# Cranial-XIX/cs231-capsule-yolo-traffic-sign-detection

Measured on AMD Instinct MI355X. Metric: train images/sec darkcapsule GTSDB 416x416 @1/2/4/8 GPU; loss-curve parity, higher is better.
Workload: dtype f32; 1 GPU; experiments/darkcapsule GTSDB-shaped 416x416, n_grid 13, 3 routing iters, batch 32 per GPU, recon off, fp32 (BASELINE configs[2]); global_batch=32, parallelism=dp1

## Files before the change

### cs231-capsule-yolo-traffic-sign-detection_amd/_lib.py

```python
import ctypes as C
import os

_HERE = os.path.dirname(os.path.abspath(__file__))
LIB_PATH = os.environ.get('CAPSYOLO_LIB') or os.path.join(_HERE, 'libcapsyolo_hip.so')

_c_float_p = C.c_void_p
_ll = C.c_longlong


class ConvGemm(C.Structure):
    _fields_ = [('X', C.c_void_p), ('Wp', C.c_void_p), ('Y', C.c_void_p), ('bias', C.c_void_p), ('stats', C.c_void_p),
                ('xs_b', _ll), ('xs_y', _ll), ('xs_x', _ll), ('xs_c', _ll),
                ('B', C.c_int), ('Hi', C.c_int), ('Wi', C.c_int), ('Cin', C.c_int),
                ('Ho', C.c_int), ('Wo', C.c_int), ('N', C.c_int),
                ('TH', C.c_int), ('TW', C.c_int), ('in_stride', C.c_int), ('dy0', C.c_int), ('dx0', C.c_int),
                ('dstep', C.c_int),
                ('Hy', C.c_int), ('Wy', C.c_int), ('out_stride', C.c_int), ('out_oy', C.c_int), ('out_ox', C.c_int),
                ('act', C.c_int),
                ('bn_z', C.c_void_p), ('bn_scale', C.c_void_p), ('bn_shift', C.c_void_p), ('bn_mean', C.c_void_p),
                ('bn_invstd', C.c_void_p), ('bn_red', C.c_void_p), ('bn_slope', C.c_float), ('act_slope', C.c_float),
                ('ws', C.c_void_p), ('ws_floats', _ll)]


class ConvWgrad(C.Structure):
    _fields_ = [('X', C.c_void_p), ('dZ', C.c_void_p), ('dW', C.c_void_p), ('slabs', C.c_void_p),
                ('xs_b', _ll), ('xs_y', _ll), ('xs_x', _ll), ('xs_c', _ll),
                ('B', C.c_int), ('Hi', C.c_int), ('Wi', C.c_int), ('Cin', C.c_int),
                ('Ho', C.c_int), ('Wo', C.c_int), ('N', C.c_int),
                ('KH', C.c_int), ('KW', C.c_int), ('stride', C.c_int), ('pad', C.c_int)]


class RoutingFwd(C.Structure):
    _fields_ = [('u', C.c_void_p), ('W', C.c_void_p), ('v_out', C.c_void_p), ('s_hist', C.c_void_p),
                ('R', C.c_int), ('N', C.c_int), ('C', C.c_int), ('Din', C.c_int), ('Dout', C.c_int),
                ('n_iter', C.c_int), ('gather_g', C.c_int), ('gather_B', C.c_int), ('ws', C.c_void_p)]


class RoutingBwd(C.Structure):
    _fields_ = [('u', C.c_void_p), ('W', C.c_void_p), ('s_hist', C.c_void_p), ('dv', C.c_void_p),
                ('du', C.c_void_p), ('dW', C.c_void_p), ('ws', C.c_void_p),
                ('R', C.c_int), ('N', C.c_int), ('C', C.c_int), ('Din', C.c_int), ('Dout', C.c_int),
                ('n_iter', C.c_int), ('gather_g', C.c_int), ('gather_B', C.c_int)]


class Decoder(C.Structure):
    _fields_ = [(k, C.c_void_p) for k in ('caps', 'labels', 'deltas', 'x', 'lin_w', 'lin_b', 'w4', 'b4', 'w7', 'b7', 'w10', 'b10',
                                          'w12', 'b12', 'out_f32', 'out_u8', 'sqerr', 'err')] + \
               [(k, C.c_int) for k in ('n', 'C', 'D', 'n_delta')]


_P, _I, _F, _L = C.c_void_p, C.c_int, C.c_float, C.c_longlong

_SIGS = {
    'cy_conv_pack_weights': [_P, _P, _I, _I, _I, _I, _I, _I, _I, _I, _I, _I, _P],
    'cy_conv_gemm': [C.POINTER(ConvGemm), _P],
    'cy_conv_wgrad': [C.POINTER(ConvWgrad), _P],
    'cy_channel_sum': [_P, _P, _L, _I, _P],
    'cy_wino_pack_weights': [_P, _P, _I, _I, _I, _P],
    'cy_conv1_3x3_fwd': [_P, _P, _P, _P, _P, _P, _P, _F, _I, _I, _I, _I, _P],
    'cy_conv1_3x3_stats': [_P, _P, _P, _P, _P, _I, _I, _I, _I, _P],
    'cy_conv1_bn_bwd_onepass': [_P, _P, _P, _P, _P, _P, _P, _P, _F, _P, _P, _P, _P, _P, _P, _P, _I, _I, _I, _I, _P],
    'cy_conv1_bn_bwd_onepass_bf16': [_P, _P, _P, _P, _P, _P, _P, _P, _F, _P, _P, _P, _P, _P, _P, _P, _I, _I, _I, _I, _P],
    'cy_conv1_3x3_wgrad': [_P, _P, _P, _P, _I, _I, _I, _I, _P],
    'cy_conv1_bn_bwd_reduce': [_P, _P, _P, _P, _P, _P, _P, _P, _F, _P, _I, _I, _I, _I, _P],
    'cy_conv1_bn_bwd_reduce_bf16': [_P, _P, _P, _P, _P, _P, _P, _P, _F, _P, _I, _I, _I, _I, _P],
    'cy_conv1_bn_bwd_wgrad': [_P, _P, _P, _P, _P, _P, _P, _P, _F, _P, _L, _P, _P, _I, _I, _I, _I, _P],
    'cy_conv1_bn_bwd_wgrad_bf16': [_P, _P, _P, _P, _P, _P, _P, _P, _F, _P, _L, _P, _P, _I, _I, _I, _I, _P],
    'cy_conv1_3x3_fwd_act_bf16': [_P, _P, _P, _P, _P, _P, _F, _I, _I, _I, _I, _P],
    'cy_conv3x3_winograd': [_P, _P, _P, _P, _P, _F, _I, _I, _I, _I, _I, _P],
    'cy_conv3x3_winograd_ws': [_P, _P, _P, _P, _P, _F, _I, _I, _I, _I, _I, _P, _L, _P],
    'cy_wino4_pack_weights': [_P, _P, _I, _I, _I, _P],
    'cy_conv3x3_winograd4': [_P, _P, _P, _P, _P, _F, _I, _I, _I, _I, _I, _P],
    'cy_conv3x3_winograd4_wgrad': [_P, _P, _P, _P, _I, _I, _I, _I, _I, _P],
    'cy_conv3x3_winograd4_wgrad_bn': [_P, _P, _P, _P, _P, _P, _P, _P, _L, _P, _P, _I, _I, _I, _I, _I, _P],
    'cy_conv3x3_winograd_wgrad': [_P, _P, _P, _P, _I, _I, _I, _I, _I, _P],
    'cy_conv3x3_winograd_wgrad_bn': [_P, _P, _P, _P, _P, _P, _P, _P, _F, _I, _P, _L, _P, _P, _I, _I, _I, _I, _I, _P],
    'cy_bn_param_grad': [_P, _P, _P, _I, _P],
    'cy_wino2_pack_weights': [_P, _P, _I, _I, _P],
    'cy_conv4x4s2_winograd': [_P, _P, _P, _P, _P, _P, _P, _F, _F, _I, _I, _I, _I, _I, _P],
    'cy_conv4x4s2_winograd4': [_P, _P, _P, _P, _P, _P, _P, _F, _F, _I, _I, _I, _I, _I, _P],
    'cy_wino4s2_pack_weights': [_P, _P, _I, _I, _P],
    'cy_wino4s2_pack_dgrad_weights': [_P, _P, _I, _I, _P],
    'cy_conv4x4s2_winograd4_dgrad': [_P, _P, _P, _P, _P, _P, _P, _P, _F, _P, _I, _I, _I, _I, _I, _P],
    'cy_conv4x4s2_winograd_wgrad': [_P, _P, _P, _P, _P, _P, _F, _I, _I, _I, _I, _I, _P],
    'cy_wino2_pack_dgrad_weights': [_P, _P, _I, _I, _P],
    'cy_conv4x4s2_winograd_dgrad': [_P, _P, _P, _P, _P, _P, _P, _P, _F, _P, _I, _I, _I, _I, _I, _P],
    'cy_bn_finalize': [_P, _L, _P, _P, _P, _P, _F, _F, _P, _P, _P, _P, _I, _P, _P],
    'cy_bn_red_fold': [_P, _I, C.c_double, _P, _P, _P, _I, _P],
    'cy_bn_eval_scale_shift': [_P, _P, _P, _P, _F, _P, _P, _I, _P],
    'cy_bn_fold_eval': [_P, _P, _P, _P, _P, _P, _F, _P, _P, _I, _I, _P],
    'cy_affine_act': [_P, _P, _P, _P, _F, _L, _I, _P],
    'cy_bn_bwd_reduce': [_P, _P, _P, _P, _P, _P, _F, _P, _L, _I, _P],
    'cy_bn_bwd_apply': [_P, _P, _P, _P, _P, _P, _P, _P, _F, _P, _P, _P, _L, _I, _P],
    'cy_act_bwd': [_P, _P, _P, _F, _L, _P],
    'cy_routing_fwd': [C.POINTER(RoutingFwd), _P],
    'cy_routing_bwd': [C.POINTER(RoutingBwd), _P],
    'cy_routing_general_fwd': [C.POINTER(RoutingFwd), _P],
    'cy_routing_general_bwd': [C.POINTER(RoutingBwd), _P],
    'cy_squash_fwd': [_P, _P, _L, _I, _P],
    'cy_squash_bwd': [_P, _P, _P, _L, _I, _P],
    'cy_length_fwd': [_P, _P, _L, _I, _P],
    'cy_length_bwd': [_P, _P, _P, _P, _L, _I, _P],
    'cy_darkcapsule_loss': [_P, _P, _I, _P, _P, _I, _I, _P],
    'cy_darkcapsule2_loss': [_P, _P, _P, _P, _I, _I, _I, _P],
    'cy_darkcapsule3_loss': [_P, _P, _P, _P, _I, _I, _I, _I, _P],
    'cy_margin_loss': [_P, _P, _P, _P, _I, _I, _P],
    'cy_recon_loss_add': [_P, _P, _F, _P, _P, _L, _P],
    'cy_dark_loss': [_P, _P, _P, _P, _P, _I, _I, _I, _I, _F, _F, _F, _P],
    'cy_scale_by_device_scalar': [_P, _P, _P, _L, _P],
    'cy_center_u8': [_P, _P, _I, _I, _I, _I, _I, _P],
    'cy_permute4': [_P, _P, _L, _I, _I, _I, _L, _L, _L, _L, _I, _P],
    'cy_maxpool2_fwd': [_P, _P, _P, _I, _I, _I, _I, _P],
    'cy_affine_act_maxpool2': [_P, _P, _P, _F, _P, _P, _I, _I, _I, _I, _P],
    'cy_maxpool2_bwd_bn': [_P, _P, _P, _P, _P, _P, _P, _F, _P, _P, _I, _I, _I, _I, _P],
    'cy_maxpool2_bwd': [_P, _P, _P, _I, _I, _I, _I, _P],
    'cy_upsample_fwd': [_P, _P, _I, _I, _I, _I, _I, _P],
    'cy_upsample_bwd': [_P, _P, _I, _I, _I, _I, _I, _P],
    'cy_tanh_fwd': [_P, _P, _L, _P],
    'cy_tanh_bwd': [_P, _P, _P, _L, _P],
    'cy_yolo_head_fwd': [_P, _P, _L, _I, _I, _P],
    'cy_yolo_head_bwd': [_P, _P, _P, _L, _I, _I, _P],
    'cy_yolo_decode_boxes': [_P, _P, C.c_double, C.c_double, _I, _I, _I, _I, _F, _P, _P, _P, _P, _I, _P],
    'cy_detect_confusion': [_P, _P, _I, _P, _P, _I, _I, C.c_double, _I, _P, _P],
    'cy_crop_resize_u8': [_P, _P, _P, _I, _L, _P, _P, _I, _I, _I, _F, _F, _I, _P, _P, _P],
    'cy_combine_scores': [_P, _P, _P, _P, _I, _P, C.c_double, _I, _I, _I, _I, _P, _P, _P, _P],
    'cy_yolo_decode_boxes_conf': [_P, _P, C.c_double, C.c_double, _I, _I, _I, _I, _F, _P, _P, _P, _P, _P, _I, _P],
    'cy_confusion_sweep': [_P, _P, _P, _I, _P, _P, _P, _I, _I, _I, _P, _I, _P, _I, _I, _P, _P, _P],
    'cy_draw_boxes_u8': [_P, _P, _P, _I, _L, _P, _P, _P, _P, _I, _I, _P, _P, _P],
    'cy_paste_resize_u8': [_P, _P, _P, _I, _L, _P, _P, _P, _I, _L, _P, _P, _P, _I, _P, _I, _I, _I, _I, _P, _P, _P],
    'cy_gather_jitter_u8': [_P, _P, _I, _I, _I, _P, _P, _P, _I, _P, _P, _P, _P],
    'cy_rank_counts': [_P, _P, _P, _I, _I, _P, _P, _P, _P, _P],
    'cy_pick_capsule': [_P, _P, _P, _I, _I, _I, _I, _P],
    'cy_decoder_fwd': [C.POINTER(Decoder), _P],
    'cy_zero_bytes': [_P, _L, _P],
    'cy_conv_bf16_pack_weights': [_P, _P, _I, _I, _I, _I, _I, _I, _I, _I, _I, _I, _P],
    'cy_conv_gemm_bf16': [C.POINTER(ConvGemm), _I, _P],
    'cy_conv_gemm_bf16_classes': [C.POINTER(ConvGemm), _I, _I, _P],
    'cy_conv_wgrad_bf16': [_P, _P, _P, _P, _I, _I, _I, _I, _I, _I, _I, _I, _I, _P],
    'cy_conv_wgrad_bf16_bn': [_P, _P, _P, _P, _P, _P, _P, _P, _P, _P, _P, _P, _I, _I, _I, _I, _I, _I, _I, _I, _I, _P],
    'cy_affine_act_bf16': [_P, _P, _P, _P, _F, _L, _I, _I, _P],
    'cy_bn_bwd_reduce_bf16': [_P, _P, _I, _P, _P, _P, _P, _F, _P, _L, _I, _P],
    'cy_bn_bwd_apply_bf16': [_P, _P, _I, _P, _P, _P, _P, _P, _F, _P, _P, _P, _L, _I, _P],
    'cy_cast_f32_bf16': [_P, _P, _L, _P],
    'cy_cast_bf16_f32': [_P, _P, _L, _P],
    'cy_multi_copy': [_P, _P, _I, _I, _P, _I, _F, _P],
    'cy_adam_multi': [_P, _P, _I, _I, _F, _F, _F, _F, _F, _F, _P],
    'cy_adam_multi_dev': [_P, _P, _I, _I, _P, _P],
}
_RET = {
    'capsyolo_last_error': (C.c_char_p, []),
    'capsyolo_abi_version': (C.c_int, []),
    'cy_conv_packed_floats': (_L, [_I, _I]),
    'cy_conv_bf16_packed_elems': (_L, [_I, _I]),
    'cy_conv_wgrad_bf16_ws_floats': (_L, [_I, _I, _I, _I, _I, _I, _I]),
    'cy_conv_wgrad_bf16_bn_ws_floats': (_L, [_I, _I, _I, _I, _I, _I, _I]),
    'cy_wino_packed_floats': (_L, [_I, _I]),
    'cy_wino_split_ws_floats': (_L, [_I, _I, _I, _I, _I, _I]),
    'cy_wino4_packed_floats': (_L, [_I, _I]),
    'cy_wino4_wgrad_ws_floats': (_L, [_I, _I, _I, _I, _I]),
    'cy_wino4_wgrad_ok': (_I, [_I, _I, _I, _I, _I]),
    'cy_conv1_3x3_wgrad_ws_floats': (_L, [_I, _I, _I, _I]),
    'cy_conv1_3x3_stats_ws_floats': (_L, [_I, _I]),
    'cy_conv1_3x3_stats_m2_offset': (_L, [_I, _I]),
    'cy_conv1_bn_bwd_wgrad_ws_floats': (_L, [_I, _I, _I, _I]),
    'cy_wino2_packed_floats': (_L, [_I, _I]),
    'cy_wino4s2_packed_floats': (_L, [_I, _I]),
    'cy_wino4s2_ok': (_I, [_I, _I, _I, _I, _I]),
    'cy_wino4s2_dgrad_ok': (_I, [_I, _I, _I, _I, _I]),
    'cy_wino4s2_dgrad_packed_floats': (_L, [_I, _I]),
    'cy_wino2_dgrad_packed_floats': (_L, [_I, _I]),
    'cy_wino2_wgrad_ws_floats': (_L, [_I, _I, _I]),
    'cy_wino_wgrad_ws_floats': (_L, [_I, _I, _I]),
    'cy_conv_wgrad_ws_floats': (_L, [C.POINTER(ConvWgrad)]),
    'cy_conv_gemm_ws_floats': (_L, [C.POINTER(ConvGemm)]),
    'cy_routing_bwd_ws_floats': (_L, [C.POINTER(RoutingBwd)]),
    'cy_routing_fwd_ws_floats': (_L, [C.POINTER(RoutingFwd)]),
    'cy_routing_general_bwd_ws_floats': (_L, [C.POINTER(RoutingBwd)]),
    'cy_routing_general_fwd_ws_floats': (_L, [C.POINTER(RoutingFwd)]),
    'cy_routing_specialised': (_I, [C.POINTER(RoutingFwd)]),
    'cy_rank_ws_ints': (_L, [_I, _I]),
    'cy_paste_resize_max_pastes': (_I, []),
    'cy_conv_gemm_bf16_plan': (_I, [C.POINTER(ConvGemm), _I, _I, C.POINTER(C.c_int)]),
    'cy_routing_plan': (_I, [C.POINTER(RoutingFwd), _I, _I, C.POINTER(_L), _I]),
}
EXPORTS = sorted(list(_SIGS) + list(_RET))
ABI_VERSION = 5

_lib = None


class HipExtensionError(RuntimeError):
    pass


def load():
    global _lib
    if _lib is not None:
        return _lib
    if not os.path.exists(LIB_PATH):
        raise HipExtensionError(
            'libcapsyolo_hip.so is not built (%s). Run `python -c "import __graft_entry__ as g; g.build()"` '
            'or `make -C cs231-capsule-yolo-traffic-sign-detection_amd/csrc`. There is no CPU fallback.' % LIB_PATH)
    lib = C.CDLL(LIB_PATH)
    lib.capsyolo_abi_version.restype = C.c_int
    have = lib.capsyolo_abi_version()
    if have != ABI_VERSION:
        raise HipExtensionError('%s has ABI version %d, these bindings were written for %d: rebuild it '
                                '(make -C cs231-capsule-yolo-traffic-sign-detection_amd/csrc)' % (LIB_PATH, have, ABI_VERSION))
    for name, argtypes in _SIGS.items():
        fn = getattr(lib, name)
        fn.argtypes, fn.restype = argtypes, C.c_int
    for name, (restype, argtypes) in _RET.items():
        fn = getattr(lib, name)
        fn.argtypes, fn.restype = argtypes, restype
    _lib = lib
    return lib


TRACE = None


def call(name, *args):
    lib = load()
    if TRACE is not None:
        TRACE.append(name)
    rc = getattr(lib, name)(*args)
    if rc != 0:
        msg = lib.capsyolo_last_error()
        raise HipExtensionError('%s failed (code %d): %s' % (name, rc, msg.decode() if msg else '?'))


def query(name, *args):
    return getattr(load(), name)(*args)
```

### cs231-capsule-yolo-traffic-sign-detection_amd/csrc/conv1.hip

```cpp
#include "common.h"
#ifndef CY_C1_NT
#define CY_C1_NT 1
#endif
#if CY_C1_NT
#define CY_C1_ST(v, p) __builtin_nontemporal_store((v), (p))
#define CY_C1_LD(p) __builtin_nontemporal_load((p))
#else
#define CY_C1_ST(v, p) (*(p) = (v))
#define CY_C1_LD(p) (*(p))
#endif


namespace {

struct Conv1Args {
  const float* X; const float* W; const float* bias; float* Y; double* stats;
  const float* scale; const float* shift; float slope;
  int B, H, Wd, Cout;
  long long ntiles;
};

template <int NT, bool AFF, bool STORE, bool OBF = false>
__global__ __launch_bounds__(256, 1) void conv1_fwd_kernel(Conv1Args a) {
  const int t = threadIdx.x, lane = t & 63, wave = t >> 6;
  const int li = lane & 31, lh = lane >> 5;
  const long long gw = (long long)blockIdx.x * 4 + wave, nw = (long long)gridDim.x * 4;
  const int segs = a.Wd / 32;
  const size_t plane = (size_t)a.H * a.Wd;

  int toff[14];
  int tky[14], tkx[14];
  float wreg[NT][14];
#pragma unroll
  for (int s = 0; s < 14; ++s) {
    const int k = 2 * s + lh;
    const int kk = k < 27 ? k : 0;
    const int c = kk / 9, kh = (kk % 9) / 3, kw = kk % 3;
    tky[s] = k < 27 ? kh - 1 : (1 << 20);
    tkx[s] = kw - 1;
    toff[s] = (int)(c * plane) + (kh - 1) * a.Wd + (kw - 1);
#pragma unroll
    for (int nt = 0; nt < NT; ++nt)
      wreg[nt][s] = k < 27 ? a.W[((size_t)(NT * li + nt) * 3 + c) * 9 + kh * 3 + kw] : 0.f;
  }
  float bv[NT];
#pragma unroll
  for (int nt = 0; nt < NT; ++nt) bv[nt] = a.bias != nullptr ? a.bias[NT * li + nt] : 0.f;
  float ssum[NT], ssq[NT];
#pragma unroll
  for (int nt = 0; nt < NT; ++nt) { ssum[nt] = 0.f; ssq[nt] = 0.f; }
  constexpr bool aff = AFF;
  float asc[NT];
#pragma unroll
  for (int nt = 0; nt < NT; ++nt) {
    asc[nt] = aff ? a.scale[NT * li + nt] : 1.f;
    if (aff) bv[nt] = bv[nt] * asc[nt] + a.shift[NT * li + nt];
  }

  auto load_a = [&](long long tile, float (&av)[14]) {
    const int seg = (int)(tile % segs);
    const long long row = tile / segs;
    const int y = (int)(row % a.H), b = (int)(row / a.H);
    const int x = seg * 32 + li;
    const float* px = a.X + (size_t)b * 3 * plane + (size_t)y * a.Wd + x;
    const bool inner = y >= 1 && y + 1 < a.H && seg >= 1 && seg + 1 < segs;
    if (inner) {
#pragma unroll
      for (int s = 0; s < 14; ++s) av[s] = (s < 13 || lh == 0) ? px[toff[s]] : 0.f;
    } else {
#pragma unroll
      for (int s = 0; s < 14; ++s) {
        const bool ok = (unsigned)(y + tky[s]) < (unsigned)a.H && (unsigned)(x + tkx[s]) < (unsigned)a.Wd;
        const float v = px[ok ? toff[s] : 0];
        av[s] = ok ? v : 0.f;
      }
    }
  };

  float acur[14], anext[14];
  long long tile = gw;
  if (tile < a.ntiles) load_a(tile, acur);
  for (; tile < a.ntiles; tile += nw) {
    const long long tn = tile + nw;
    if (tn < a.ntiles) load_a(tn, anext);
    f32x16 acc[NT];
#pragma unroll
    for (int nt = 0; nt < NT; ++nt)
#pragma unroll
      for (int r = 0; r < 16; ++r) acc[nt][r] = 0.f;
#pragma unroll
    for (int s = 0; s < 14; ++s)
#pragma unroll
      for (int nt = 0; nt < NT; ++nt) acc[nt] = __builtin_amdgcn_mfma_f32_32x32x2f32(acur[s], wreg[nt][s], acc[nt], 0, 0, 0);
    float* yp = a.Y + (size_t)tile * 32 * a.Cout + NT * li;
#pragma unroll
    for (int r = 0; r < 16; ++r) {
      typedef float vecn __attribute__((ext_vector_type(NT)));
      const int p = (r & 3) + 8 * (r >> 2) + 4 * lh;
      float v[NT];
#pragma unroll
      for (int nt = 0; nt < NT; ++nt) {
        if (aff) {
          const float y = __builtin_fmaf(acc[nt][r], asc[nt], bv[nt]);
          const float ys = y * a.slope;
          asm("v_max_f32 %0, %1, %2" : "=v"(v[nt]) : "v"(y), "v"(ys));
        } else {
          v[nt] = acc[nt][r] + bv[nt];
          ssum[nt] += v[nt];
          ssq[nt] = __builtin_fmaf(v[nt], v[nt], ssq[nt]);
        }
      }
      if constexpr (!STORE) {
        (void)p;
      } else if constexpr (OBF) {
        unsigned short* yb = (unsigned short*)a.Y + (size_t)tile * 32 * a.Cout + NT * li + (size_t)p * a.Cout;
        unsigned short h[NT];
#pragma unroll
        for (int nt = 0; nt < NT; ++nt) { const __bf16 b = (__bf16)v[nt]; h[nt] = *(const unsigned short*)&b; }
        if constexpr (NT == 4) {
          typedef unsigned u32x2_t __attribute__((ext_vector_type(2)));
          CY_C1_ST((u32x2_t{(unsigned)h[0] | ((unsigned)h[1] << 16), (unsigned)h[2] | ((unsigned)h[3] << 16)}), (u32x2_t*)yb);
        } else if constexpr (NT == 2) {
          *(unsigned*)yb = (unsigned)h[0] | ((unsigned)h[1] << 16);
        } else {
          yb[0] = h[0];
        }
      } else if constexpr (NT == 1) {
        yp[(size_t)p * a.Cout] = v[0];
      } else {
        vecn o;
#pragma unroll
        for (int nt = 0; nt < NT; ++nt) o[nt] = v[nt];
        CY_C1_ST(o, (vecn*)(yp + (size_t)p * a.Cout));
      }
    }
#pragma unroll
    for (int s = 0; s < 14; ++s) acur[s] = anext[s];
  }
  if (a.stats != nullptr) {
    double* st = a.stats + (size_t)((blockIdx.x * 4 + wave) % CY_STATS_COPIES) * a.Cout * 2;
#pragma unroll
    for (int nt = 0; nt < NT; ++nt) {
      const float s1 = ssum[nt] + __shfl_xor(ssum[nt], 32, 64), s2 = ssq[nt] + __shfl_xor(ssq[nt], 32, 64);
      if (lh == 0) {
        atomicAdd(st + 2 * (NT * li + nt), (double)s1);
        atomicAdd(st + 2 * (NT * li + nt) + 1, (double)s2);
      }
    }
  }
}

typedef __bf16 c1_bf16x8 __attribute__((ext_vector_type(8)));
template <int NT>
__global__ __launch_bounds__(256, 1) void conv1_fwd_bf16_kernel(Conv1Args a) {
  const int t = threadIdx.x, lane = t & 63, wave = t >> 6;
  const int li = lane & 31, lh = lane >> 5;
  const long long gw = (long long)blockIdx.x * 4 + wave, nw = (long long)gridDim.x * 4;
  const int segs = a.Wd / 32;
  const size_t plane = (size_t)a.H * a.Wd;
  int toff[16], tky[16], tkx[16];
  c1_bf16x8 wreg[NT][2];
#pragma unroll
  for (int i = 0; i < 16; ++i) {
    const int k = 16 * (i >> 3) + 8 * lh + (i & 7);
    const int kk = k < 27 ? k : 0;
    const int c = kk / 9, kh = (kk % 9) / 3, kw = kk % 3;
    tky[i] = k < 27 ? kh - 1 : (1 << 20);
    tkx[i] = kw - 1;
    toff[i] = (int)(c * plane) + (kh - 1) * a.Wd + (kw - 1);
#pragma unroll
    for (int nt = 0; nt < NT; ++nt)
      wreg[nt][i >> 3][i & 7] = (__bf16)(k < 27 ? a.W[((size_t)(NT * li + nt) * 3 + c) * 9 + kh * 3 + kw] : 0.f);
  }
  float bv[NT], asc[NT];
#pragma unroll
  for (int nt = 0; nt < NT; ++nt) {
    asc[nt] = a.scale[NT * li + nt];
    bv[nt] = (a.bias != nullptr ? a.bias[NT * li + nt] : 0.f) * asc[nt] + a.shift[NT * li + nt];
  }
  auto load_a = [&](long long tile, float (&av)[16]) {
    const int seg = (int)(tile % segs);
    const long long row = tile / segs;
    const int y = (int)(row % a.H), b = (int)(row / a.H);
    const int x = seg * 32 + li;
    const float* px = a.X + (size_t)b * 3 * plane + (size_t)y * a.Wd + x;
    const bool inner = y >= 1 && y + 1 < a.H && seg >= 1 && seg + 1 < segs;
    if (inner) {
#pragma unroll
      for (int i = 0; i < 16; ++i) av[i] = (i < 8 || lh == 0 || (i & 7) < 3) ? px[toff[i]] : 0.f;
    } else {
#pragma unroll
      for (int i = 0; i < 16; ++i) {
        const bool ok = (unsigned)(y + tky[i]) < (unsigned)a.H && (unsigned)(x + tkx[i]) < (unsigned)a.Wd;
        const float v = px[ok ? toff[i] : 0];
        av[i] = ok ? v : 0.f;
      }
    }
  };
  float acur[16], anext[16];
  long long tile = gw;
  if (tile < a.ntiles) load_a(tile, acur);
  for (; tile < a.ntiles; tile += nw) {
    const long long tn = tile + nw;
    if (tn < a.ntiles) load_a(tn, anext);
    c1_bf16x8 a8[2];
#pragma unroll
    for (int i = 0; i < 16; ++i) a8[i >> 3][i & 7] = (__bf16)acur[i];
    f32x16 acc[NT];
#pragma unroll
    for (int nt = 0; nt < NT; ++nt)
#pragma unroll
      for (int r = 0; r < 16; ++r) acc[nt][r] = 0.f;
#pragma unroll
    for (int s = 0; s < 2; ++s)
#pragma unroll
      for (int nt = 0; nt < NT; ++nt) acc[nt] = __builtin_amdgcn_mfma_f32_32x32x16_bf16(a8[s], wreg[nt][s], acc[nt], 0, 0, 0);
#pragma unroll
    for (int r = 0; r < 16; ++r) {
      const int p = (r & 3) + 8 * (r >> 2) + 4 * lh;
      unsigned short h[NT];
#pragma unroll
      for (int nt = 0; nt < NT; ++nt) {
        const float y = __builtin_fmaf(acc[nt][r], asc[nt], bv[nt]);
        const float ys = y * a.slope;
        float v;
        asm("v_max_f32 %0, %1, %2" : "=v"(v) : "v"(y), "v"(ys));
        const __bf16 b = (__bf16)v;
        h[nt] = *(const unsigned short*)&b;
      }
      unsigned short* yb = (unsigned short*)a.Y + (size_t)tile * 32 * a.Cout + NT * li + (size_t)p * a.Cout;
      if constexpr (NT == 4) {
        typedef unsigned u32x2_t __attribute__((ext_vector_type(2)));
        CY_C1_ST((u32x2_t{(unsigned)h[0] | ((unsigned)h[1] << 16), (unsigned)h[2] | ((unsigned)h[3] << 16)}), (u32x2_t*)yb);
      } else if constexpr (NT == 2) {
        *(unsigned*)yb = (unsigned)h[0] | ((unsigned)h[1] << 16);
      } else {
        yb[0] = h[0];
      }
    }
#pragma unroll
    for (int i = 0; i < 16; ++i) acur[i] = anext[i];
  }
}

template <int NT>
__global__ __launch_bounds__(256, 1) void conv1_wgrad_kernel(Conv1Args a, float* __restrict__ slabs) {
  const int t = threadIdx.x, lane = t & 63, wave = t >> 6;
  const int li = lane & 31, lh = lane >> 5;
  const long long gw = (long long)blockIdx.x * 4 + wave, nw = (long long)gridDim.x * 4;
  const int segs = a.Wd / 32;
  const size_t plane = (size_t)a.H * a.Wd;
  const int kk = li < 27 ? li : 0;
  const int tc = kk / 9, tkh = (kk % 9) / 3, tkw = kk % 3;
  const int toff = (int)(tc * plane) + (tkh - 1) * a.Wd + (tkw - 1) + lh;

  auto load_tile = [&](long long tile, float (&av)[NT][16], float (&bv)[16]) {
    const int seg = (int)(tile % segs);
    const long long row = tile / segs;
    const int y = (int)(row % a.H), b = (int)(row / a.H);
    const float* pz = a.Y + (size_t)tile * 32 * a.Cout + (size_t)lh * a.Cout + NT * li;
#pragma unroll
    for (int s = 0; s < 16; ++s) {
      typedef float vecn __attribute__((ext_vector_type(NT)));
      if constexpr (NT == 1) {
        av[0][s] = pz[(size_t)(2 * s) * a.Cout];
      } else {
        const vecn v = *(const vecn*)(pz + (size_t)(2 * s) * a.Cout);
#pragma unroll
        for (int nt = 0; nt < NT; ++nt) av[nt][s] = v[nt];
      }
    }
    const float* px = a.X + (size_t)b * 3 * plane + (size_t)y * a.Wd + seg * 32;
    const bool inner = y >= 1 && y + 1 < a.H && seg >= 1 && seg + 1 < segs;
    if (inner) {
#pragma unroll
      for (int s = 0; s < 16; ++s) bv[s] = px[toff + 2 * s];
    } else {
      const bool rowok = (unsigned)(y + tkh - 1) < (unsigned)a.H;
#pragma unroll
      for (int s = 0; s < 16; ++s) {
        const bool ok = rowok && (unsigned)(seg * 32 + 2 * s + lh + tkw - 1) < (unsigned)a.Wd;
        const float v = px[ok ? toff + 2 * s : 0];
        bv[s] = ok ? v : 0.f;
      }
    }
  };

  f32x16 acc[NT];
#pragma unroll
  for (int nt = 0; nt < NT; ++nt)
#pragma unroll
    for (int r = 0; r < 16; ++r) acc[nt][r] = 0.f;
  float acur[NT][16], bcur[16], anext[NT][16], bnext[16];
  long long tile = gw;
  if (tile < a.ntiles) load_tile(tile, acur, bcur);
  for (; tile < a.ntiles; tile += nw) {
    const long long tn = tile + nw;
    if (tn < a.ntiles) load_tile(tn, anext, bnext);
#pragma unroll
    for (int s = 0; s < 16; ++s)
#pragma unroll
      for (int nt = 0; nt < NT; ++nt) acc[nt] = __builtin_amdgcn_mfma_f32_32x32x2f32(acur[nt][s], bcur[s], acc[nt], 0, 0, 0);
#pragma unroll
    for (int s = 0; s < 16; ++s) {
      bcur[s] = bnext[s];
#pragma unroll
      for (int nt = 0; nt < NT; ++nt) acur[nt][s] = anext[nt][s];
    }
  }
  float* out = slabs + (size_t)gw * a.Cout * 32;
#pragma unroll
  for (int nt = 0; nt < NT; ++nt)
#pragma unroll
    for (int r = 0; r < 16; ++r) {
      const int co = NT * ((r & 3) + 8 * (r >> 2) + 4 * lh) + nt;
      out[(size_t)co * 32 + li] = acc[nt][r];
    }
}

struct Conv1BnArgs {
  const float* X; const float* W; const float* bias; const float* dA;
  const float* scale; const float* shift; const float* mean; const float* invstd; float slope;
  double* red_out;
  const double* red_in; double inv_count;
  float* slabs;
  int B, H, Wd, Cout;
  long long ntiles;
};

template <int NT, int PASS, bool GBF = false>
__global__ __launch_bounds__(256, 1) void conv1_bn_bwd_kernel(Conv1BnArgs a) {
  typedef float vecn __attribute__((ext_vector_type(NT)));
  const int t = threadIdx.x, lane = t & 63, wave = t >> 6;
  const int li = lane & 31, lh = lane >> 5;
  const long long gw = (long long)blockIdx.x * 4 + wave, nw = (long long)gridDim.x * 4;
  const int segs = a.Wd / 32;
  const size_t plane = (size_t)a.H * a.Wd;
  int toff[14], tky[14], tkx[14];
  float wreg[NT][14];
#pragma unroll
  for (int s = 0; s < 14; ++s) {
    const int k = 2 * s + lh;
    const int kk = k < 27 ? k : 0;
    const int c = kk / 9, kh = (kk % 9) / 3, kw = kk % 3;
    tky[s] = k < 27 ? kh - 1 : (1 << 20);
    tkx[s] = kw - 1;
    toff[s] = (int)(c * plane) + (kh - 1) * a.Wd + (kw - 1);
#pragma unroll
    for (int nt = 0; nt < NT; ++nt)
      wreg[nt][s] = k < 27 ? a.W[((size_t)(NT * li + nt) * 3 + c) * 9 + kh * 3 + kw] : 0.f;
  }
  const int kt = li < 27 ? li : 0;
  const int wc = kt / 9, wkh = (kt % 9) / 3, wkw = kt % 3;
  const int woff = (int)(wc * plane) + (wkh - 1) * a.Wd + (wkw - 1) + 4 * lh;
  float bv[NT], sc[NT], sh[NT], is[NT], nm[NT], m1[NT], m2[NT];
#pragma unroll
  for (int nt = 0; nt < NT; ++nt) {
    const int c = NT * li + nt;
    bv[nt] = a.bias != nullptr ? a.bias[c] : 0.f;
    sc[nt] = a.scale[c]; sh[nt] = a.shift[c]; is[nt] = a.invstd[c]; nm[nt] = -a.mean[c] * is[nt];
    m1[nt] = PASS == 1 ? (float)(a.red_in[2 * c] * a.inv_count) : 0.f;
    m2[nt] = PASS == 1 ? (float)(a.red_in[2 * c + 1] * a.inv_count) : 0.f;
  }
  float b1[NT], b2[NT];
#pragma unroll
  for (int nt = 0; nt < NT; ++nt) { b1[nt] = 0.f; b2[nt] = 0.f; }

  auto load_img = [&](long long tile, float (&av)[14], float (&bw)[16]) {
    const int seg = (int)(tile % segs);
    const long long row = tile / segs;
    const int y = (int)(row % a.H), b = (int)(row / a.H);
    const float* p0 = a.X + (size_t)b * 3 * plane + (size_t)y * a.Wd + seg * 32;
    const float* px = p0 + li;
    const bool inner = y >= 1 && y + 1 < a.H && seg >= 1 && seg + 1 < segs;
    if (inner) {
#pragma unroll
      for (int s = 0; s < 14; ++s) av[s] = (s < 13 || lh == 0) ? px[toff[s]] : 0.f;
      if (PASS >= 1) {
#pragma unroll
        for (int s = 0; s < 16; ++s) bw[s] = p0[woff + (s & 3) + 8 * (s >> 2)];
      }
    } else {
#pragma unroll
      for (int s = 0; s < 14; ++s) {
        const bool ok = (unsigned)(y + tky[s]) < (unsigned)a.H && (unsigned)(seg * 32 + li + tkx[s]) < (unsigned)a.Wd;
        const float v = px[ok ? toff[s] : 0];
        av[s] = ok ? v : 0.f;
      }
      if (PASS >= 1) {
        const bool rowok = (unsigned)(y + wkh - 1) < (unsigned)a.H;
#pragma unroll
        for (int s = 0; s < 16; ++s) {
          const int pcol = (s & 3) + 8 * (s >> 2) + 4 * lh;
          const bool ok = rowok && (unsigned)(seg * 32 + pcol + wkw - 1) < (unsigned)a.Wd;
          const float v = p0[ok ? woff + (s & 3) + 8 * (s >> 2) : 0];
          bw[s] = ok ? v : 0.f;
        }
      }
    }
  };

  f32x16 accw[NT];
#pragma unroll
  for (int nt = 0; nt < NT; ++nt)
#pragma unroll
    for (int r = 0; r < 16; ++r) accw[nt][r] = 0.f;
  float acur[14], anext[14], bwcur[16], bwnext[16];
  long long tile = gw;
  if (tile < a.ntiles) load_img(tile, acur, bwcur);
  for (; tile < a.ntiles; tile += nw) {
    vecn g[16];
    if constexpr (GBF) {
      const unsigned short* pg = (const unsigned short*)a.dA + (size_t)tile * 32 * a.Cout + NT * li;
#pragma unroll
      for (int r = 0; r < 16; ++r) {
        const unsigned short* q = pg + (size_t)((r & 3) + 8 * (r >> 2) + 4 * lh) * a.Cout;
        if constexpr (NT == 4) {
          typedef unsigned u32x2_t __attribute__((ext_vector_type(2)));
          const u32x2_t w = CY_C1_LD((const u32x2_t*)q);
          g[r][0] = __uint_as_float(w[0] << 16); g[r][1] = __uint_as_float(w[0] & 0xffff0000u);
          g[r][2] = __uint_as_float(w[1] << 16); g[r][3] = __uint_as_float(w[1] & 0xffff0000u);
        } else if constexpr (NT == 2) {
          const unsigned w = *(const unsigned*)q;
          g[r][0] = __uint_as_float(w << 16); g[r][1] = __uint_as_float(w & 0xffff0000u);
        } else {
          g[r] = vecn(__uint_as_float((unsigned)q[0] << 16));
        }
      }
    } else {
      const float* pg = a.dA + (size_t)tile * 32 * a.Cout + NT * li;
#pragma unroll
      for (int r = 0; r < 16; ++r) g[r] = CY_C1_LD((const vecn*)(pg + (size_t)((r & 3) + 8 * (r >> 2) + 4 * lh) * a.Cout));
    }
    const long long tn = tile + nw;
    if (tn < a.ntiles) load_img(tn, anext, bwnext);
    f32x16 acc[NT];
#pragma unroll
    for (int nt = 0; nt < NT; ++nt)
#pragma unroll
      for (int r = 0; r < 16; ++r) acc[nt][r] = 0.f;
#pragma unroll
    for (int s = 0; s < 14; ++s)
#pragma unroll
      for (int nt = 0; nt < NT; ++nt) acc[nt] = __builtin_amdgcn_mfma_f32_32x32x2f32(acur[s], wreg[nt][s], acc[nt], 0, 0, 0);
#pragma unroll
    for (int r = 0; r < 16; ++r) {
      float dzr[NT];
#pragma unroll
      for (int nt = 0; nt < NT; ++nt) {
        const float z = acc[nt][r] + bv[nt];
        const float y = __builtin_fmaf(z, sc[nt], sh[nt]);
        const float gv = ((const float*)&g[r])[nt];
        const float d = y > 0.f ? gv : gv * a.slope;
        const float xh = __builtin_fmaf(z, is[nt], nm[nt]);
        if (PASS == 0) {
          b1[nt] += d;
          b2[nt] = __builtin_fmaf(d, xh, b2[nt]);
        } else if (PASS == 1) {
          dzr[nt] = sc[nt] * (d - m1[nt] - xh * m2[nt]);
        } else {
          b1[nt] += d;
          dzr[nt] = d;
        }
      }
      if (PASS >= 1) {
#pragma unroll
        for (int nt = 0; nt < NT; ++nt) accw[nt] = __builtin_amdgcn_mfma_f32_32x32x2f32(dzr[nt], bwcur[r], accw[nt], 0, 0, 0);
      }
    }
#pragma unroll
    for (int s = 0; s < 14; ++s) acur[s] = anext[s];
    if (PASS >= 1) {
#pragma unroll
      for (int s = 0; s < 16; ++s) bwcur[s] = bwnext[s];
    }
  }
  if (PASS == 0 || PASS == 2) {
    double* rd = a.red_out + (size_t)((blockIdx.x * 4 + wave) % CY_STATS_COPIES) * a.Cout * 2;
#pragma unroll
    for (int nt = 0; nt < NT; ++nt) {
      const float s1 = b1[nt] + __shfl_xor(b1[nt], 32, 64), s2 = b2[nt] + __shfl_xor(b2[nt], 32, 64);
      if (lh == 0) {
        atomicAdd(rd + 2 * (NT * li + nt), (double)s1);
        if (PASS == 0) atomicAdd(rd + 2 * (NT * li + nt) + 1, (double)s2);
      }
    }
  }
  if (PASS >= 1) {
    float* out = a.slabs + (size_t)gw * a.Cout * 32;
#pragma unroll
    for (int nt = 0; nt < NT; ++nt)
#pragma unroll
      for (int r = 0; r < 16; ++r) {
        const int co = NT * ((r & 3) + 8 * (r >> 2) + 4 * lh) + nt;
        out[(size_t)co * 32 + li] = accw[nt][r];
      }
  }
}

template <int NT, int PASS>
__global__ __launch_bounds__(256, 1) void conv1_bn_bwd_bf16mm_kernel(Conv1BnArgs a) {
  const int t = threadIdx.x, lane = t & 63, wave = t >> 6;
  const int li = lane & 31, lh = lane >> 5;
  const long long gw = (long long)blockIdx.x * 4 + wave, nw = (long long)gridDim.x * 4;
  const int segs = a.Wd / 32;
  const size_t plane = (size_t)a.H * a.Wd;
  int toff[16], tky[16], tkx[16];
  c1_bf16x8 wreg[NT][2];
#pragma unroll
  for (int i = 0; i < 16; ++i) {
    const int k = 16 * (i >> 3) + 8 * lh + (i & 7);
    const int kk = k < 27 ? k : 0;
    const int c = kk / 9, kh = (kk % 9) / 3, kw = kk % 3;
    tky[i] = k < 27 ? kh - 1 : (1 << 20);
    tkx[i] = kw - 1;
    toff[i] = (int)(c * plane) + (kh - 1) * a.Wd + (kw - 1);
#pragma unroll
    for (int nt = 0; nt < NT; ++nt)
      wreg[nt][i >> 3][i & 7] = (__bf16)(k < 27 ? a.W[((size_t)(NT * li + nt) * 3 + c) * 9 + kh * 3 + kw] : 0.f);
  }
  const int kt = li < 27 ? li : 0;
  const int wc = kt / 9, wkh = (kt % 9) / 3, wkw = kt % 3;
  const int woff = (int)(wc * plane) + (wkh - 1) * a.Wd + (wkw - 1) + 4 * lh;
  float bv[NT], sc[NT], sh[NT], is[NT], nm[NT], m1[NT], m2[NT], b1[NT], b2[NT];
#pragma unroll
  for (int nt = 0; nt < NT; ++nt) {
    const int c = NT * li + nt;
    bv[nt] = a.bias != nullptr ? a.bias[c] : 0.f;
    sc[nt] = a.scale[c]; sh[nt] = a.shift[c];
    sh[nt] = __builtin_fmaf(bv[nt], sc[nt], sh[nt]);
    is[nt] = PASS < 2 ? a.invstd[c] : 0.f;
    nm[nt] = PASS < 2 ? (bv[nt] - a.mean[c]) * is[nt] : 0.f;
    m1[nt] = PASS == 1 ? (float)(a.red_in[2 * c] * a.inv_count) : 0.f;
    m2[nt] = PASS == 1 ? (float)(a.red_in[2 * c + 1] * a.inv_count) : 0.f;
    b1[nt] = 0.f; b2[nt] = 0.f;
  }
  auto load_img = [&](long long tile, float (&av)[16], float (&bw)[16]) {
    const int seg = (int)(tile % segs);
    const long long row = tile / segs;
    const int y = (int)(row % a.H), b = (int)(row / a.H);
    const float* p0 = a.X + (size_t)b * 3 * plane + (size_t)y * a.Wd + seg * 32;
    const float* px = p0 + li;
    const bool inner = y >= 1 && y + 1 < a.H && seg >= 1 && seg + 1 < segs;
    if (inner) {
#pragma unroll
      for (int i = 0; i < 16; ++i) av[i] = (i < 8 || lh == 0 || (i & 7) < 3) ? px[toff[i]] : 0.f;
      if (PASS >= 1) {
#pragma unroll
        for (int r = 0; r < 16; ++r) bw[r] = p0[woff + (r & 3) + 8 * (r >> 2)];
      }
    } else {
#pragma unroll
      for (int i = 0; i < 16; ++i) {
        const bool ok = (unsigned)(y + tky[i]) < (unsigned)a.H && (unsigned)(seg * 32 + li + tkx[i]) < (unsigned)a.Wd;
        const float v = px[ok ? toff[i] : 0];
        av[i] = ok ? v : 0.f;
      }
      if (PASS >= 1) {
        const bool rowok = (unsigned)(y + wkh - 1) < (unsigned)a.H;
#pragma unroll
        for (int r = 0; r < 16; ++r) {
          const int pcol = (r & 3) + 8 * (r >> 2) + 4 * lh;
          const bool ok = rowok && (unsigned)(seg * 32 + pcol + wkw - 1) < (unsigned)a.Wd;
          const float v = p0[ok ? woff + (r & 3) + 8 * (r >> 2) : 0];
          bw[r] = ok ? v : 0.f;
        }
      }
    }
  };
  f32x16 accw[NT];
#pragma unroll
  for (int nt = 0; nt < NT; ++nt)
#pragma unroll
    for (int r = 0; r < 16; ++r) accw[nt][r] = 0.f;
  float acur[16], anext[16], bwcur[16], bwnext[16];
  long long tile = gw;
  if (tile < a.ntiles) load_img(tile, acur, bwcur);
  for (; tile < a.ntiles; tile += nw) {
    float g[16][NT];
    {
      const unsigned short* pg = (const unsigned short*)a.dA + (size_t)tile * 32 * a.Cout + NT * li;
#pragma unroll
      for (int r = 0; r < 16; ++r) {
        const unsigned short* q = pg + (size_t)((r & 3) + 8 * (r >> 2) + 4 * lh) * a.Cout;
        if constexpr (NT == 4) {
          typedef unsigned u32x2_t __attribute__((ext_vector_type(2)));
          const u32x2_t w = CY_C1_LD((const u32x2_t*)q);
          g[r][0] = __uint_as_float(w[0] << 16); g[r][1] = __uint_as_float(w[0] & 0xffff0000u);
          g[r][2] = __uint_as_float(w[1] << 16); g[r][3] = __uint_as_float(w[1] & 0xffff0000u);
        } else if constexpr (NT == 2) {
          const unsigned w = *(const unsigned*)q;
          g[r][0] = __uint_as_float(w << 16); g[r][1] = __uint_as_float(w & 0xffff0000u);
        } else {
          g[r][0] = __uint_as_float((unsigned)q[0] << 16);
        }
      }
    }
    const long long tn = tile + nw;
    if (tn < a.ntiles) load_img(tn, anext, bwnext);
    c1_bf16x8 a8[2], b8[2];
#pragma unroll
    for (int i = 0; i < 16; ++i) { a8[i >> 3][i & 7] = (__bf16)acur[i]; if (PASS >= 1) b8[i >> 3][i & 7] = (__bf16)bwcur[i]; }
    f32x16 acc[NT];
#pragma unroll
    for (int nt = 0; nt < NT; ++nt)
#pragma unroll
      for (int r = 0; r < 16; ++r) acc[nt][r] = 0.f;
#pragma unroll
    for (int s = 0; s < 2; ++s)
#pragma unroll
      for (int nt = 0; nt < NT; ++nt) acc[nt] = __builtin_amdgcn_mfma_f32_32x32x16_bf16(a8[s], wreg[nt][s], acc[nt], 0, 0, 0);
#pragma unroll
    for (int nt = 0; nt < NT; ++nt) {
      c1_bf16x8 d8[2];
#pragma unroll
      for (int r = 0; r < 16; ++r) {
        const float y = __builtin_fmaf(acc[nt][r], sc[nt], sh[nt]);
        const float gv = g[r][nt];
        const float d = y > 0.f ? gv : gv * a.slope;
        if (PASS == 0) {
          const float xh = __builtin_fmaf(acc[nt][r], is[nt], nm[nt]);
          b1[nt] += d;
          b2[nt] = __builtin_fmaf(d, xh, b2[nt]);
        } else if (PASS == 1) {
          const float xh = __builtin_fmaf(acc[nt][r], is[nt], nm[nt]);
          d8[r >> 3][r & 7] = (__bf16)(sc[nt] * (d - m1[nt] - xh * m2[nt]));
        } else {
          b1[nt] += d;
          d8[r >> 3][r & 7] = (__bf16)d;
        }
      }
      if (PASS >= 1) {
#pragma unroll
        for (int s = 0; s < 2; ++s) accw[nt] = __builtin_amdgcn_mfma_f32_32x32x16_bf16(d8[s], b8[s], accw[nt], 0, 0, 0);
      }
    }
#pragma unroll
    for (int i = 0; i < 16; ++i) { acur[i] = anext[i]; if (PASS >= 1) bwcur[i] = bwnext[i]; }
  }
  if (PASS == 0 || PASS == 2) {
    double* rd = a.red_out + (size_t)((blockIdx.x * 4 + wave) % CY_STATS_COPIES) * a.Cout * 2;
#pragma unroll
    for (int nt = 0; nt < NT; ++nt) {
      const float s1 = b1[nt] + __shfl_xor(b1[nt], 32, 64), s2 = b2[nt] + __shfl_xor(b2[nt], 32, 64);
      if (lh == 0) {
        atomicAdd(rd + 2 * (NT * li + nt), (double)s1);
        if (PASS == 0) atomicAdd(rd + 2 * (NT * li + nt) + 1, (double)s2);
      }
    }
  }
  if (PASS >= 1) {
    float* out = a.slabs + (size_t)gw * a.Cout * 32;
#pragma unroll
    for (int nt = 0; nt < NT; ++nt)
#pragma unroll
      for (int r = 0; r < 16; ++r) {
        const int co = NT * ((r & 3) + 8 * (r >> 2) + 4 * lh) + nt;
        out[(size_t)co * 32 + li] = accw[nt][r];
      }
  }
}

__global__ __launch_bounds__(256) void conv1_wgrad_finish_kernel(const float* __restrict__ slabs, float* __restrict__ dW,
                                                                 int nslab, int Cout) {
  __shared__ float part[8][32];
  const int co = blockIdx.x, tap = threadIdx.x & 31, grp = threadIdx.x >> 5;
  float s = 0.f;
  for (int w = grp; w < nslab; w += 8) s += slabs[((size_t)w * Cout + co) * 32 + tap];
  part[grp][tap] = s;
  __syncthreads();
  if (threadIdx.x < 27) {
    float v = 0.f;
#pragma unroll
    for (int g = 0; g < 8; ++g) v += part[g][threadIdx.x];
    dW[co * 27 + threadIdx.x] = v;
  }
}

__global__ __launch_bounds__(256) void conv1_bn_bwd_finish_kernel(const float* __restrict__ slabs, int nslab, const double* __restrict__ redc,
                                                                  const double* __restrict__ M2, const float* __restrict__ W,
                                                                  const float* __restrict__ bias, const float* __restrict__ scale,
                                                                  const float* __restrict__ mean, const float* __restrict__ invstd,
                                                                  float* __restrict__ dW, float* __restrict__ dgamma,
                                                                  float* __restrict__ dbeta, double* __restrict__ red_out, int Cout) {
  __shared__ float part[8][32];
  __shared__ double G[27], wv[27], sdz;
  const int co = blockIdx.x, tap = threadIdx.x & 31, grp = threadIdx.x >> 5;
  float s = 0.f;
  for (int w = grp; w < nslab; w += 8) s += slabs[((size_t)w * Cout + co) * 32 + tap];
  part[grp][tap] = s;
  __syncthreads();
  if (threadIdx.x < 27) {
    float v = 0.f;
#pragma unroll
    for (int g = 0; g < 8; ++g) v += part[g][threadIdx.x];
    G[threadIdx.x] = (double)v;
    wv[threadIdx.x] = (double)W[co * 27 + threadIdx.x];
  }
  __syncthreads();
  double Sd = 0.0;
  for (int c = 0; c < CY_STATS_COPIES; ++c) Sd += redc[((size_t)c * Cout + co) * 2];
  const double b = bias != nullptr ? (double)bias[co] : 0.0, mu = (double)mean[co], is = (double)invstd[co];
  if (threadIdx.x == 0) {
    double wg = 0.0;
    for (int t = 0; t < 27; ++t) wg += wv[t] * G[t];
    sdz = wg + b * Sd;
  }
  __syncthreads();
  const double P = M2[27 * 32 + 27];
  const double sdx = is * (sdz - mu * Sd);
  if (threadIdx.x == 0) {
    dbeta[co] = (float)Sd;
    dgamma[co] = (float)sdx;
    if (red_out != nullptr) { red_out[2 * co] = Sd; red_out[2 * co + 1] = sdx; }
  }
  if (threadIdx.x < 27) {
    const int t = threadIdx.x;
    double m2w = 0.0;
    for (int u = 0; u < 27; ++u) m2w += M2[t * 32 + u] * wv[u];
    const double mvt = M2[27 * 32 + t];
    const double sxp = is * (m2w + (b - mu) * mvt);
    dW[co * 27 + t] = (float)((double)scale[co] * (G[t] - (Sd / P) * mvt - (sdx / P) * sxp));
  }
}

static int conv1_blocks(long long ntiles, long long* blocks, const char* who) {
  return cyi_persistent_blocks(who, (ntiles + 3) / 4, blocks);
}

}

extern "C" long long cy_conv1_3x3_wgrad_ws_floats(int B, int H, int Wd, int Cout) {
  long long blocks = 0;
  if (B <= 0 || H <= 0 || Wd <= 0 || Wd % 32 || conv1_blocks((long long)B * H * (Wd / 32), &blocks, "cy_conv1_3x3_wgrad_ws_floats")) return -1;
  return blocks * 4 * Cout * 32;
}

extern "C" int cy_conv1_3x3_wgrad(const float* X, const float* dZ, float* dW, float* ws, int B, int H, int Wd, int Cout,
                                  void* stream) {
  CY_REQUIRE(X && dZ && dW && ws && B > 0 && H > 0 && Wd > 0, "cy_conv1_3x3_wgrad: bad arguments");
  CY_REQUIRE(Wd % 32 == 0, "cy_conv1_3x3_wgrad: W=%d must be a multiple of 32", Wd);
  CY_REQUIRE(Cout == 32 || Cout == 64 || Cout == 128, "cy_conv1_3x3_wgrad: Cout=%d must be 32, 64 or 128", Cout);
  CY_REQUIRE((long long)3 * H * Wd < (1ll << 30), "cy_conv1_3x3_wgrad: image too large for 32-bit offsets");
  Conv1Args a;
  a.X = X; a.W = nullptr; a.bias = nullptr; a.Y = const_cast<float*>(dZ); a.stats = nullptr;
  a.scale = a.shift = nullptr; a.slope = 1.f;
  a.B = B; a.H = H; a.Wd = Wd; a.Cout = Cout;
  a.ntiles = (long long)B * H * (Wd / 32);
  long long blocks = 0;
  int rc = conv1_blocks(a.ntiles, &blocks, "cy_conv1_3x3_wgrad");
  if (rc) return rc;
  hipStream_t s = (hipStream_t)stream;
  if (Cout == 128) conv1_wgrad_kernel<4><<<(unsigned)blocks, 256, 0, s>>>(a, ws);
  else if (Cout == 64) conv1_wgrad_kernel<2><<<(unsigned)blocks, 256, 0, s>>>(a, ws);
  else conv1_wgrad_kernel<1><<<(unsigned)blocks, 256, 0, s>>>(a, ws);
  CY_LAUNCH_CHECK("cy_conv1_3x3_wgrad");
  conv1_wgrad_finish_kernel<<<Cout, 256, 0, s>>>(ws, dW, (int)(blocks * 4), Cout);
  CY_LAUNCH_CHECK("cy_conv1_3x3_wgrad (finish)");
  return 0;
}

static int conv1_bn_check(const char* who, const float* X, const float* W, const float* dA, const float* scale,
                          const float* shift, const float* mean, const float* invstd, float slope, int B, int H, int Wd,
                          int Cout) {
  CY_REQUIRE(X && W && dA && scale && shift && mean && invstd && B > 0 && H > 0 && Wd > 0, "%s: bad arguments", who);
  CY_REQUIRE(Wd % 32 == 0, "%s: W=%d must be a multiple of 32", who, Wd);
  CY_REQUIRE(Cout == 32 || Cout == 64 || Cout == 128, "%s: Cout=%d must be 32, 64 or 128", who, Cout);
  CY_REQUIRE((long long)3 * H * Wd < (1ll << 30), "%s: image too large for 32-bit offsets", who);
  CY_REQUIRE(slope >= 0.f && slope <= 1.f, "%s: slope must be in [0, 1]", who);
  return 0;
}

static int conv1_bn_bwd_reduce_impl(const char* who, const float* X, const float* W, const float* bias, const void* dA,
                                    bool da_bf16, const float* scale, const float* shift, const float* mean, const float* invstd,
                                    float slope, double* red, int B, int H, int Wd, int Cout, void* stream) {
  int rc = conv1_bn_check(who, X, W, (const float*)dA, scale, shift, mean, invstd, slope, B, H, Wd, Cout);
  if (rc) return rc;
  CY_REQUIRE(red != nullptr, "%s: red is NULL", who);
  Conv1BnArgs a;
  a.X = X; a.W = W; a.bias = bias; a.dA = (const float*)dA; a.scale = scale; a.shift = shift; a.mean = mean; a.invstd = invstd;
  a.slope = slope; a.red_out = red; a.red_in = nullptr; a.inv_count = 0.0; a.slabs = nullptr;
  a.B = B; a.H = H; a.Wd = Wd; a.Cout = Cout; a.ntiles = (long long)B * H * (Wd / 32);
  long long blocks = 0;
  rc = conv1_blocks(a.ntiles, &blocks, who);
  if (rc) return rc;
  hipStream_t s = (hipStream_t)stream;
  if (da_bf16) {
#ifdef CY_C1_F32MM
    if (Cout == 128) conv1_bn_bwd_kernel<4, 0, true><<<(unsigned)blocks, 256, 0, s>>>(a);
    else if (Cout == 64) conv1_bn_bwd_kernel<2, 0, true><<<(unsigned)blocks, 256, 0, s>>>(a);
    else conv1_bn_bwd_kernel<1, 0, true><<<(unsigned)blocks, 256, 0, s>>>(a);
#else
    if (Cout == 128) conv1_bn_bwd_bf16mm_kernel<4, 0><<<(unsigned)blocks, 256, 0, s>>>(a);
    else if (Cout == 64) conv1_bn_bwd_bf16mm_kernel<2, 0><<<(unsigned)blocks, 256, 0, s>>>(a);
    else conv1_bn_bwd_bf16mm_kernel<1, 0><<<(unsigned)blocks, 256, 0, s>>>(a);
#endif
  } else {
    if (Cout == 128) conv1_bn_bwd_kernel<4, 0><<<(unsigned)blocks, 256, 0, s>>>(a);
    else if (Cout == 64) conv1_bn_bwd_kernel<2, 0><<<(unsigned)blocks, 256, 0, s>>>(a);
    else conv1_bn_bwd_kernel<1, 0><<<(unsigned)blocks, 256, 0, s>>>(a);
  }
  CY_LAUNCH_CHECK(who);
  return 0;
}
extern "C" int cy_conv1_bn_bwd_reduce(const float* X, const float* W, const float* bias, const float* dA, const float* scale,
                                      const float* shift, const float* mean, const float* invstd, float slope, double* red,
                                      int B, int H, int Wd, int Cout, void* stream) {
  return conv1_bn_bwd_reduce_impl("cy_conv1_bn_bwd_reduce", X, W, bias, dA, false, scale, shift, mean, invstd, slope, red, B, H, Wd,
                                  Cout, stream);
}
extern "C" int cy_conv1_bn_bwd_reduce_bf16(const float* X, const float* W, const float* bias, const void* dA, const float* scale,
                                           const float* shift, const float* mean, const float* invstd, float slope, double* red,
                                           int B, int H, int Wd, int Cout, void* stream) {
  return conv1_bn_bwd_reduce_impl("cy_conv1_bn_bwd_reduce_bf16", X, W, bias, dA, true, scale, shift, mean, invstd, slope, red, B, H,
                                  Wd, Cout, stream);
}

static int conv1_bn_bwd_onepass_impl(const char* who, const float* X, const float* W, const float* bias, const void* dA, bool da_bf16,
                                     const float* scale, const float* shift, const float* mean, const float* invstd, float slope,
                                     const double* M2, double* redc, float* dW, float* dgamma, float* dbeta, double* red_out,
                                     float* ws, int B, int H, int Wd, int Cout, void* stream) {
  int rc = conv1_bn_check(who, X, W, (const float*)dA, scale, shift, mean, invstd, slope, B, H, Wd, Cout);
  if (rc) return rc;
  CY_REQUIRE(M2 && redc && dW && dgamma && dbeta && ws, "%s: NULL argument", who);
  Conv1BnArgs a;
  a.X = X; a.W = W; a.bias = bias; a.dA = (const float*)dA; a.scale = scale; a.shift = shift; a.mean = mean; a.invstd = invstd;
  a.slope = slope; a.red_out = redc; a.red_in = nullptr; a.inv_count = 0.0; a.slabs = ws;
  a.B = B; a.H = H; a.Wd = Wd; a.Cout = Cout; a.ntiles = (long long)B * H * (Wd / 32);
  long long blocks = 0;
  rc = conv1_blocks(a.ntiles, &blocks, who);
  if (rc) return rc;
  hipStream_t s = (hipStream_t)stream;
  if (da_bf16) {
#ifdef CY_C1_F32MM
    if (Cout == 128) conv1_bn_bwd_kernel<4, 2, true><<<(unsigned)blocks, 256, 0, s>>>(a);
    else if (Cout == 64) conv1_bn_bwd_kernel<2, 2, true><<<(unsigned)blocks, 256, 0, s>>>(a);
    else conv1_bn_bwd_kernel<1, 2, true><<<(unsigned)blocks, 256, 0, s>>>(a);
#else
    if (Cout == 128) conv1_bn_bwd_bf16mm_kernel<4, 2><<<(unsigned)blocks, 256, 0, s>>>(a);
    else if (Cout == 64) conv1_bn_bwd_bf16mm_kernel<2, 2><<<(unsigned)blocks, 256, 0, s>>>(a);
    else conv1_bn_bwd_bf16mm_kernel<1, 2><<<(unsigned)blocks, 256, 0, s>>>(a);
#endif
  } else {
    if (Cout == 128) conv1_bn_bwd_kernel<4, 2><<<(unsigned)blocks, 256, 0, s>>>(a);
    else if (Cout == 64) conv1_bn_bwd_kernel<2, 2><<<(unsigned)blocks, 256, 0, s>>>(a);
    else conv1_bn_bwd_kernel<1, 2><<<(unsigned)blocks, 256, 0, s>>>(a);
  }
  CY_LAUNCH_CHECK(who);
  conv1_bn_bwd_finish_kernel<<<Cout, 256, 0, s>>>(ws, (int)(blocks * 4), redc, M2, W, bias, scale, mean, invstd, dW, dgamma, dbeta,
                                                  red_out, Cout);
  CY_LAUNCH_CHECK(who);
  return 0;
}
extern "C" int cy_conv1_bn_bwd_onepass(const float* X, const float* W, const float* bias, const float* dA, const float* scale,
                                       const float* shift, const float* mean, const float* invstd, float slope, const double* M2,
                                       double* redc, float* dW, float* dgamma, float* dbeta, double* red_out, float* ws, int B,
                                       int H, int Wd, int Cout, void* stream) {
  return conv1_bn_bwd_onepass_impl("cy_conv1_bn_bwd_onepass", X, W, bias, dA, false, scale, shift, mean, invstd, slope, M2, redc, dW,
                                   dgamma, dbeta, red_out, ws, B, H, Wd, Cout, stream);
}
extern "C" int cy_conv1_bn_bwd_onepass_bf16(const float* X, const float* W, const float* bias, const void* dA, const float* scale,
                                            const float* shift, const float* mean, const float* invstd, float slope,
                                            const double* M2, double* redc, float* dW, float* dgamma, float* dbeta, double* red_out,
                                            float* ws, int B, int H, int Wd, int Cout, void* stream) {
  return conv1_bn_bwd_onepass_impl("cy_conv1_bn_bwd_onepass_bf16", X, W, bias, dA, true, scale, shift, mean, invstd, slope, M2, redc,
                                   dW, dgamma, dbeta, red_out, ws, B, H, Wd, Cout, stream);
}

extern "C" long long cy_conv1_bn_bwd_wgrad_ws_floats(int B, int H, int Wd, int Cout) {
  return cy_conv1_3x3_wgrad_ws_floats(B, H, Wd, Cout);
}

static int conv1_bn_bwd_wgrad_impl(const char* who, bool da_bf16, const float* X, const float* W, const float* bias, const void* dA, const float* scale,
                                     const float* shift, const float* mean, const float* invstd, float slope,
                                     const double* red, long long count, float* dW, float* ws, int B, int H, int Wd,
                                     int Cout, void* stream) {
  int rc = conv1_bn_check(who, X, W, (const float*)dA, scale, shift, mean, invstd, slope, B, H, Wd, Cout);
  if (rc) return rc;
  CY_REQUIRE(red && dW && ws && count > 0, "cy_conv1_bn_bwd_wgrad: bad arguments");
  Conv1BnArgs a;
  a.X = X; a.W = W; a.bias = bias; a.dA = (const float*)dA; a.scale = scale; a.shift = shift; a.mean = mean; a.invstd = invstd;
  a.slope = slope; a.red_out = nullptr; a.red_in = red; a.inv_count = 1.0 / (double)count; a.slabs = ws;
  a.B = B; a.H = H; a.Wd = Wd; a.Cout = Cout; a.ntiles = (long long)B * H * (Wd / 32);
  long long blocks = 0;
  rc = conv1_blocks(a.ntiles, &blocks, who);
  if (rc) return rc;
  hipStream_t s = (hipStream_t)stream;
  if (da_bf16) {
#ifdef CY_C1_F32MM
    if (Cout == 128) conv1_bn_bwd_kernel<4, 1, true><<<(unsigned)blocks, 256, 0, s>>>(a);
    else if (Cout == 64) conv1_bn_bwd_kernel<2, 1, true><<<(unsigned)blocks, 256, 0, s>>>(a);
    else conv1_bn_bwd_kernel<1, 1, true><<<(unsigned)blocks, 256, 0, s>>>(a);
#else
    if (Cout == 128) conv1_bn_bwd_bf16mm_kernel<4, 1><<<(unsigned)blocks, 256, 0, s>>>(a);
    else if (Cout == 64) conv1_bn_bwd_bf16mm_kernel<2, 1><<<(unsigned)blocks, 256, 0, s>>>(a);
    else conv1_bn_bwd_bf16mm_kernel<1, 1><<<(unsigned)blocks, 256, 0, s>>>(a);
#endif
  } else {
    if (Cout == 128) conv1_bn_bwd_kernel<4, 1><<<(unsigned)blocks, 256, 0, s>>>(a);
    else if (Cout == 64) conv1_bn_bwd_kernel<2, 1><<<(unsigned)blocks, 256, 0, s>>>(a);
    else conv1_bn_bwd_kernel<1, 1><<<(unsigned)blocks, 256, 0, s>>>(a);
  }
  CY_LAUNCH_CHECK(who);
  conv1_wgrad_finish_kernel<<<Cout, 256, 0, s>>>(ws, dW, (int)(blocks * 4), Cout);
  CY_LAUNCH_CHECK(who);
  return 0;
}

extern "C" int cy_conv1_bn_bwd_wgrad(const float* X, const float* W, const float* bias, const float* dA, const float* scale,
                                     const float* shift, const float* mean, const float* invstd, float slope,
                                     const double* red, long long count, float* dW, float* ws, int B, int H, int Wd,
                                     int Cout, void* stream) {
  return conv1_bn_bwd_wgrad_impl("cy_conv1_bn_bwd_wgrad", false, X, W, bias, dA, scale, shift, mean, invstd, slope, red, count, dW, ws, B,
                                 H, Wd, Cout, stream);
}
extern "C" int cy_conv1_bn_bwd_wgrad_bf16(const float* X, const float* W, const float* bias, const void* dA, const float* scale,
                                          const float* shift, const float* mean, const float* invstd, float slope,
                                          const double* red, long long count, float* dW, float* ws, int B, int H, int Wd,
                                          int Cout, void* stream) {
  return conv1_bn_bwd_wgrad_impl("cy_conv1_bn_bwd_wgrad_bf16", true, X, W, bias, dA, scale, shift, mean, invstd, slope, red, count, dW,
                                 ws, B, H, Wd, Cout, stream);
}

extern "C" int cy_conv1_3x3_fwd(const float* X, const float* W, const float* bias, float* Y, double* stats,
                                const float* scale, const float* shift, float slope, int B, int H, int Wd, int Cout,
                                void* stream) {
  CY_REQUIRE(X && W && (Y || (stats && !scale)) && B > 0 && H > 0 && Wd > 0, "cy_conv1_3x3_fwd: bad arguments");
  CY_REQUIRE((scale == nullptr) == (shift == nullptr), "cy_conv1_3x3_fwd: scale and shift go together");
  CY_REQUIRE(scale == nullptr || (stats == nullptr && slope >= 0.f && slope <= 1.f),
             "cy_conv1_3x3_fwd: the affine pass takes no statistics and a slope in [0, 1]");
  CY_REQUIRE(Wd % 32 == 0, "cy_conv1_3x3_fwd: W=%d must be a multiple of 32", Wd);
  CY_REQUIRE(Cout == 32 || Cout == 64 || Cout == 128, "cy_conv1_3x3_fwd: Cout=%d must be 32, 64 or 128", Cout);
  CY_REQUIRE((long long)3 * H * Wd < (1ll << 30), "cy_conv1_3x3_fwd: image too large for 32-bit offsets");
  Conv1Args a;
  a.X = X; a.W = W; a.bias = bias; a.Y = Y; a.stats = stats;
  a.scale = scale; a.shift = shift; a.slope = slope;
  a.B = B; a.H = H; a.Wd = Wd; a.Cout = Cout;
  a.ntiles = (long long)B * H * (Wd / 32);
  long long blocks = 0;
  int rc = conv1_blocks(a.ntiles, &blocks, "cy_conv1_3x3_fwd");
  if (rc) return rc;
  hipStream_t s = (hipStream_t)stream;
#define CY_CONV1_LAUNCH(NT_)                                                                  \
  do {                                                                                         \
    if (scale) conv1_fwd_kernel<NT_, true, true><<<(unsigned)blocks, 256, 0, s>>>(a);          \
    else if (Y) conv1_fwd_kernel<NT_, false, true><<<(unsigned)blocks, 256, 0, s>>>(a);        \
    else conv1_fwd_kernel<NT_, false, false><<<(unsigned)blocks, 256, 0, s>>>(a);              \
  } while (0)
  if (Cout == 128) CY_CONV1_LAUNCH(4);
  else if (Cout == 64) CY_CONV1_LAUNCH(2);
  else CY_CONV1_LAUNCH(1);
#undef CY_CONV1_LAUNCH
  CY_LAUNCH_CHECK("cy_conv1_3x3_fwd");
  return 0;
}

extern "C" int cy_conv1_3x3_fwd_act_bf16(const float* X, const float* W, const float* bias, void* Y, const float* scale,
                                         const float* shift, float slope, int B, int H, int Wd, int Cout, void* stream) {
  CY_REQUIRE(X && W && Y && scale && shift && B > 0 && H > 0 && Wd > 0, "cy_conv1_3x3_fwd_act_bf16: bad arguments");
  CY_REQUIRE(slope >= 0.f && slope <= 1.f, "cy_conv1_3x3_fwd_act_bf16: slope must be in [0, 1]");
  CY_REQUIRE(Wd % 32 == 0, "cy_conv1_3x3_fwd_act_bf16: W=%d must be a multiple of 32", Wd);
  CY_REQUIRE(Cout == 32 || Cout == 64 || Cout == 128, "cy_conv1_3x3_fwd_act_bf16: Cout=%d must be 32, 64 or 128", Cout);
  CY_REQUIRE((long long)3 * H * Wd < (1ll << 30), "cy_conv1_3x3_fwd_act_bf16: image too large for 32-bit offsets");
  Conv1Args a;
  a.X = X; a.W = W; a.bias = bias; a.Y = (float*)Y; a.stats = nullptr;
  a.scale = scale; a.shift = shift; a.slope = slope;
  a.B = B; a.H = H; a.Wd = Wd; a.Cout = Cout;
  a.ntiles = (long long)B * H * (Wd / 32);
  long long blocks = 0;
  int rc = conv1_blocks(a.ntiles, &blocks, "cy_conv1_3x3_fwd_act_bf16");
  if (rc) return rc;
  hipStream_t s = (hipStream_t)stream;
#ifdef CY_C1_F32MM
  if (Cout == 128) conv1_fwd_kernel<4, true, true, true><<<(unsigned)blocks, 256, 0, s>>>(a);
  else if (Cout == 64) conv1_fwd_kernel<2, true, true, true><<<(unsigned)blocks, 256, 0, s>>>(a);
  else conv1_fwd_kernel<1, true, true, true><<<(unsigned)blocks, 256, 0, s>>>(a);
#else
  if (Cout == 128) conv1_fwd_bf16_kernel<4><<<(unsigned)blocks, 256, 0, s>>>(a);
  else if (Cout == 64) conv1_fwd_bf16_kernel<2><<<(unsigned)blocks, 256, 0, s>>>(a);
  else conv1_fwd_bf16_kernel<1><<<(unsigned)blocks, 256, 0, s>>>(a);
#endif
  CY_LAUNCH_CHECK("cy_conv1_3x3_fwd_act_bf16");
  return 0;
}
```

### cs231-capsule-yolo-traffic-sign-detection_amd/ops.py

```python
import collections
import ctypes as C
import functools

import torch

from . import _lib
from ._lib import ConvGemm, ConvWgrad, RoutingBwd, RoutingFwd, call, query


def _stream():
    return C.c_void_p(torch.cuda.current_stream().cuda_stream)


class KernelTimer(object):

    def __init__(self):
        self.enabled = False
        self.events = {}

    class _Range(object):
        def __init__(self, timer, name):
            self.timer, self.name = timer, name

        def __enter__(self):
            if self.timer.enabled:
                self.start = torch.cuda.Event(enable_timing=True)
                self.start.record(torch.cuda.current_stream())

        def __exit__(self, *exc):
            if self.timer.enabled:
                end = torch.cuda.Event(enable_timing=True)
                end.record(torch.cuda.current_stream())
                self.timer.events.setdefault(self.name, []).append((self.start, end))
            return False

    def range(self, name):
        return KernelTimer._Range(self, name)

    def reset(self):
        self.events = {}

    def summary(self):
        return dict((k, (len(v), sum(a.elapsed_time(b) for a, b in v) / len(v))) for k, v in self.events.items())


timer = KernelTimer()


def _ptr(t):
    return None if t is None else C.c_void_p(t.data_ptr())


def _f32(t, name='tensor'):
    if not (t.is_cuda and t.dtype == torch.float32):
        raise _lib.HipExtensionError('%s must be a float32 tensor on the GPU (got %s on %s); there is no CPU fallback'
                                     % (name, t.dtype, t.device))
    return t if t.is_contiguous() else t.contiguous()


def _empty(shape, like, dtype=torch.float32):
    return torch.empty(shape, dtype=dtype, device=like.device)


class _ZeroPool(object):

    def __init__(self):
        self.pools = {}

    def reset(self, device):
        st = self.pools.get(device)
        if st is None:
            return
        if st['need'] > st['buf'].numel():
            st['buf'] = torch.zeros(2 * st['need'], dtype=torch.uint8, device=device)
        elif st['off']:
            call('cy_zero_bytes', C.c_void_p(st['buf'].data_ptr()), st['off'], _stream())
        st['off'], st['need'] = 0, 0

    def take(self, shape, dtype, device):
        n = 1
        for d in shape:
            n *= int(d)
        nbytes = (n * torch.empty((), dtype=dtype).element_size() + 255) & ~255
        st = self.pools.get(device)
        if st is None:
            st = self.pools[device] = {'buf': torch.zeros(1 << 20, dtype=torch.uint8, device=device), 'off': 0, 'need': 0}
        st['need'] += nbytes
        if st['off'] + nbytes > st['buf'].numel():
            return torch.zeros(shape, dtype=dtype, device=device)
        out = st['buf'][st['off']:st['off'] + nbytes].view(dtype)[:n].view(shape)
        st['off'] += nbytes
        return out


zero_pool = _ZeroPool()
_zero_consts = {}


def _const_zeros(n, like):
    key = (int(n), like.device)
    t = _zero_consts.get(key)
    if t is None:
        t = _zero_consts[key] = torch.zeros(n, dtype=torch.float32, device=like.device)
    return t


def _x_geometry(x, nchw):
    if nchw:
        B, Cin, Hi, Wi = x.shape
        return B, Hi, Wi, Cin, (Cin * Hi * Wi, Wi, 1, Hi * Wi)
    B, Hi, Wi, Cin = x.shape
    return B, Hi, Wi, Cin, (Hi * Wi * Cin, Wi * Cin, Cin, 1)


STATS_COPIES = 16
USE_CONV1_MOMENTS = True
FUSE_BN_BWD_APPLY_BF16 = True
USE_CONV1_ONEPASS = True
CONV1_MOMENTS_MIN_PIXELS = 1 << 18
USE_CONV1_BWD = True
USE_CONV1 = True
USE_WINOGRAD_S2_DGRAD = True
USE_WINOGRAD_S2 = True
USE_WINOGRAD = True
USE_WINOGRAD4_S2 = True
USE_WINOGRAD4_S2_DGRAD = True
WINOGRAD4_S2_MIN_PIXELS = 1 << 16
USE_WINOGRAD4 = True
WINOGRAD4_MIN_PIXELS = 1 << 17


FUSE_BN_BWD_REDUCE = True
FUSE_BN_BWD_APPLY = True
FUSE_INPUT_AFFINE = True
USE_WINOGRAD4_WGRAD = True

ConvPlan = collections.namedtuple('ConvPlan', [
    'fwd', 'dgrad', 'wgrad',
    'in_affine',
    'dgrad_bn_fuse',
    'dgrad_premasks',
    'wgrad_bn',
    'wgrad_bn4',
    'conv1',
    'conv1_bwd',
    'conv1_moments',
    'conv1_onepass'])
_WINO3_DGRAD = ('conv_wino_dgrad', 'conv_wino4_dgrad')


@functools.lru_cache(maxsize=None)
def _shape_ok(name, *shape):
    return bool(query(name, *shape))


def conv_plan(in_shape, cout, k, stride, pad, nchw=False, relu=False, lrelu=False):
    if nchw:
        B, Cin, Hi, Wi = in_shape
    else:
        B, Hi, Wi, Cin = in_shape
    fwd, dgrad, wgrad = 'conv_gemm_fwd', None if nchw else 'conv_gemm_dgrad', 'conv_wgrad'
    in_affine = wgrad_bn = wgrad_bn4 = conv1 = False
    if k == 3 and stride == 1 and pad == 1:
        px = B * Hi * Wi
        if nchw:
            conv1 = bool(USE_CONV1 and Cin == 3 and cout in (32, 64, 128) and Wi % 32 == 0)
            if conv1:
                fwd, wgrad = fwd if relu or lrelu else 'conv1_fwd', 'conv1_wgrad'
        elif USE_WINOGRAD:
            f4 = USE_WINOGRAD4 and px >= WINOGRAD4_MIN_PIXELS
            if not relu and Cin % 8 == 0 and Cin >= 8:
                fwd = 'conv_wino4_fwd' if f4 else 'conv_wino_fwd'
            if cout % 8 == 0 and cout >= 8:
                dgrad = 'conv_wino4_dgrad' if f4 else 'conv_wino_dgrad'
            w3 = Cin % 64 == 0 and cout % 64 == 0
            w4 = bool(USE_WINOGRAD4_WGRAD and px >= WINOGRAD4_MIN_PIXELS and _shape_ok('cy_wino4_wgrad_ok', B, Hi, Wi, Cin, cout))
            wgrad = 'conv_wino4_wgrad' if w4 else 'conv_wino_wgrad' if w3 else wgrad
            wgrad_bn = bool(FUSE_BN_BWD_APPLY and w3)
            wgrad_bn4 = wgrad_bn and w4
    elif (k == 4 and stride == 2 and pad == 1 and not nchw and USE_WINOGRAD and USE_WINOGRAD_S2 and Hi % 2 == 0 and Wi % 2 == 0):
        f4 = USE_WINOGRAD4_S2 and B * (Hi // 2) * (Wi // 2) >= WINOGRAD4_S2_MIN_PIXELS
        if not relu and Cin % 8 == 0:
            fwd = 'conv_wino42_fwd' if f4 and _shape_ok('cy_wino4s2_ok', B, Hi, Wi, Cin, cout) else 'conv_wino2_fwd'
        if USE_WINOGRAD_S2_DGRAD and Cin % 64 == 0 and cout % 8 == 0:
            dgrad = ('conv_wino42_dgrad' if f4 and USE_WINOGRAD4_S2_DGRAD and _shape_ok('cy_wino4s2_dgrad_ok', B, Hi, Wi, Cin, cout)
                     else 'conv_wino2_dgrad')
        if Cin % 32 == 0 and cout % 64 == 0:
            wgrad, in_affine = 'conv_wino2_wgrad', not relu
    dgrad_bn_fuse = bool(FUSE_BN_BWD_REDUCE and dgrad is not None and dgrad not in _WINO3_DGRAD and Cin % 4 == 0)
    conv1_bwd = bool(conv1 and USE_CONV1_BWD)
    return ConvPlan(fwd, dgrad, wgrad, in_affine, dgrad_bn_fuse, dgrad_bn_fuse and dgrad in ('conv_wino2_dgrad', 'conv_wino42_dgrad'),
                    wgrad_bn, wgrad_bn4, conv1, conv1_bwd,
                    bool(conv1_bwd and USE_CONV1_MOMENTS and B * Hi * Wi >= CONV1_MOMENTS_MIN_PIXELS), bool(conv1 and USE_CONV1_ONEPASS))


def _winograd(x, weight, bias, stats, transpose, f4, tag, out_slope=1.0):
    B, H, W_, Cg = x.shape
    Cout_l, Cin_l = weight.shape[0], weight.shape[1]
    n = Cin_l if transpose else Cout_l
    st = _stream()
    u = _empty((query('cy_wino4_packed_floats' if f4 else 'cy_wino_packed_floats', Cg, n),), x)
    call('cy_wino4_pack_weights' if f4 else 'cy_wino_pack_weights', _ptr(weight), _ptr(u), Cout_l, Cin_l, 1 if transpose else 0, st)
    y = _empty((B, H, W_, n), x)
    nws = 0 if f4 else query('cy_wino_split_ws_floats', B, H, W_, Cg, n, int(bias is None and stats is None and out_slope == 1.0))
    ws = _empty((nws,), x) if nws > 0 else None
    with timer.range(('conv_wino4_' if f4 else 'conv_wino_') + ('dgrad/' if transpose else 'fwd/') + tag):
        if f4:
            call('cy_conv3x3_winograd4', _ptr(x), _ptr(u), _ptr(y), _ptr(bias), _ptr(stats), float(out_slope), B, H, W_, Cg, n, st)
        else:
            call('cy_conv3x3_winograd_ws', _ptr(x), _ptr(u), _ptr(y), _ptr(bias), _ptr(stats), float(out_slope), B, H, W_, Cg, n,
                 _ptr(ws), nws, st)
    return y


def conv1_affine_act(x, weight, bias, scale, shift, slope, tag='conv', out_bf16=False):
    B, _, Hi, Wi = x.shape
    Cout = weight.shape[0]
    with timer.range('conv1_fwd_act/' + tag):
        if out_bf16:
            out = torch.empty((B, Hi, Wi, Cout), dtype=torch.bfloat16, device=x.device)
            call('cy_conv1_3x3_fwd_act_bf16', _ptr(x), _ptr(weight.contiguous()), _ptr(bias), _ptr(out), _ptr(scale), _ptr(shift),
                 float(slope), B, Hi, Wi, Cout, _stream())
        else:
            out = _empty((B, Hi, Wi, Cout), x)
            call('cy_conv1_3x3_fwd', _ptr(x), _ptr(weight.contiguous()), _ptr(bias), _ptr(out), None, _ptr(scale), _ptr(shift),
                 float(slope), B, Hi, Wi, Cout, _stream())
    return out


def conv_forward(x, weight, bias, k, stride, pad, nchw=False, stats=None, relu=False, tag='conv', in_affine=None, lrelu=None):
    if lrelu is not None and (relu or stats is not None or in_affine is not None or not 0.0 <= lrelu <= 1.0):
        raise _lib.HipExtensionError('conv_forward: the LeakyReLU epilogue (slope %r) is the eval-mode forward: no statistics, no '
                                     'fused input affine, slope in [0, 1]' % (lrelu,))
    osl = 1.0 if lrelu is None else float(lrelu)
    x, weight = _f32(x, 'conv input'), _f32(weight, 'conv weight')
    B, Hi, Wi, Cin, xs = _x_geometry(x, nchw)
    Cout = weight.shape[0]
    Ho, Wo = (Hi + 2 * pad - k) // stride + 1, (Wi + 2 * pad - k) // stride + 1
    plan = conv_plan(x.shape, Cout, k, stride, pad, nchw, relu, lrelu is not None)
    if in_affine is not None and not plan.in_affine:
        raise _lib.HipExtensionError('a fused input affine needs the 4x4/stride-2 Winograd kernels (got k=%d s=%d Cin=%d Cout=%d)' % (k, stride, Cin, Cout))
    if plan.fwd in ('conv_wino_fwd', 'conv_wino4_fwd'):
        return _winograd(x, weight, bias, stats, False, plan.fwd == 'conv_wino4_fwd', tag, osl)
    st = _stream()
    if plan.fwd in ('conv_wino2_fwd', 'conv_wino42_fwd'):
        pk, f4 = ('cy_wino4s2', '4') if plan.fwd == 'conv_wino42_fwd' else ('cy_wino2', '')
        y = _empty((B, Ho, Wo, Cout), x)
        isc, ish, isl = in_affine if in_affine is not None else (None, None, 1.0)
        u = _empty((query(pk + '_packed_floats', Cin, Cout),), x)
        call(pk + '_pack_weights', _ptr(weight), _ptr(u), Cout, Cin, st)
        with timer.range(plan.fwd + '/' + tag):
            call('cy_conv4x4s2_winograd' + f4, _ptr(x), _ptr(u), _ptr(y), _ptr(bias), _ptr(stats), _ptr(isc), _ptr(ish),
                 float(isl), osl, B, Hi, Wi, Cin, Cout, st)
        return y
    if plan.fwd == 'conv1_fwd':
        z = _empty((B, Ho, Wo, Cout), x)
        with timer.range('conv1_fwd/' + tag):
            call('cy_conv1_3x3_fwd', _ptr(x), _ptr(weight.contiguous()), _ptr(bias), _ptr(z), _ptr(stats), None, None, 1.0,
                 B, Hi, Wi, Cout, st)
        return z
    wp = _empty((query('cy_conv_packed_floats', k * k * Cin, Cout),), x)
    call('cy_conv_pack_weights', _ptr(weight), _ptr(wp), Cout, Cin, k, k, k, k, 0, 0, 1, 0, st)
    z = _empty((B, Ho, Wo, Cout), x)
    a = ConvGemm(X=x.data_ptr(), Wp=wp.data_ptr(), Y=z.data_ptr(),
                 bias=bias.data_ptr() if bias is not None else None,
                 stats=stats.data_ptr() if stats is not None else None,
                 xs_b=xs[0], xs_y=xs[1], xs_x=xs[2], xs_c=xs[3], B=B, Hi=Hi, Wi=Wi, Cin=Cin, Ho=Ho, Wo=Wo, N=Cout,
                 TH=k, TW=k, in_stride=stride, dy0=-pad, dx0=-pad, dstep=1,
                 Hy=Ho, Wy=Wo, out_stride=1, out_oy=0, out_ox=0, act=1 if relu else 2 if lrelu is not None else 0, act_slope=osl)
    ws = _gemm_workspace(a, x)
    with timer.range('conv_gemm_fwd/' + tag):
        call('cy_conv_gemm', C.byref(a), st)
    del ws
    return z


def _gemm_workspace(a, like):
    n = query('cy_conv_gemm_ws_floats', C.byref(a))
    if n <= 0:
        return None
    ws = _empty((n,), like)
    a.ws, a.ws_floats = ws.data_ptr(), n
    return ws


def dgrad_classes(Hi, Wi, k, stride, pad):
    out = []
    for py in range(stride):
        kh0 = (py + pad) % stride
        TH = len(range(kh0, k, stride))
        for px in range(stride):
            kw0 = (px + pad) % stride
            TW = len(range(kw0, k, stride))
            Hv, Wv = (Hi - py + stride - 1) // stride, (Wi - px + stride - 1) // stride
            if Hv <= 0 or Wv <= 0:
                continue
            if TH == 0 or TW == 0:
                raise _lib.HipExtensionError('conv_dgrad: kernel %d / stride %d leaves input pixels without taps'
                                             % (k, stride))
            out.append(dict(TH=TH, TW=TW, kh0=kh0, kw0=kw0, kstep=stride, Ho=Hv, Wo=Wv,
                            dy0=(py + pad - kh0) // stride, dx0=(px + pad - kw0) // stride, dstep=-1,
                            out_stride=stride, out_oy=py, out_ox=px))
    return out


def conv_dgrad(dz, weight, in_shape, k, stride, pad, tag='conv', bn_fuse=None, plan=None):
    dz, weight = _f32(dz, 'grad'), _f32(weight, 'conv weight')
    B, Hi, Wi, Cin = in_shape
    _, Ho, Wo, Cout = dz.shape
    plan = plan or conv_plan(in_shape, Cout, k, stride, pad)
    if plan.dgrad in _WINO3_DGRAD:
        if bn_fuse is not None:
            raise _lib.HipExtensionError('bn_fuse is implemented in the direct input-gradient kernel only')
        return _winograd(dz, weight, None, None, True, plan.dgrad == 'conv_wino4_dgrad', tag)
    st = _stream()
    dx = _empty((B, Hi, Wi, Cin), dz)
    if plan.dgrad in ('conv_wino2_dgrad', 'conv_wino42_dgrad'):
        pk, f4 = ('cy_wino4s2', '4') if plan.dgrad == 'conv_wino42_dgrad' else ('cy_wino2', '')
        bz, bsc, bsh, bmu, bis, bsl, bred = bn_fuse if bn_fuse is not None else (None,) * 5 + (0.0, None)
        u = _empty((query(pk + '_dgrad_packed_floats', Cin, Cout),), dz)
        call(pk + '_pack_dgrad_weights', _ptr(weight), _ptr(u), Cout, Cin, st)
        with timer.range(plan.dgrad + '/' + tag):
            call('cy_conv4x4s2_winograd%s_dgrad' % f4, _ptr(dz), _ptr(u), _ptr(dx), _ptr(bz), _ptr(bsc), _ptr(bsh), _ptr(bmu),
                 _ptr(bis), float(bsl), _ptr(bred), B, Hi, Wi, Cin, Cout, st)
        return dx
    wp = _empty((query('cy_conv_packed_floats', ((k + stride - 1) // stride) ** 2 * Cout, Cin),), dz)
    for c in dgrad_classes(Hi, Wi, k, stride, pad):
        call('cy_conv_pack_weights', _ptr(weight), _ptr(wp), Cout, Cin, k, k, c['TH'], c['TW'], c['kh0'], c['kw0'],
             c['kstep'], 1, st)
        a = ConvGemm(X=dz.data_ptr(), Wp=wp.data_ptr(), Y=dx.data_ptr(), bias=None, stats=None,
                     xs_b=Ho * Wo * Cout, xs_y=Wo * Cout, xs_x=Cout, xs_c=1, B=B, Hi=Ho, Wi=Wo, Cin=Cout,
                     Ho=c['Ho'], Wo=c['Wo'], N=Cin, TH=c['TH'], TW=c['TW'], in_stride=1,
                     dy0=c['dy0'], dx0=c['dx0'], dstep=c['dstep'],
                     Hy=Hi, Wy=Wi, out_stride=c['out_stride'], out_oy=c['out_oy'], out_ox=c['out_ox'], act=0)
        if bn_fuse is not None:
            bz, bsc, bsh, bmu, bis, bsl, bred = bn_fuse
            a.bn_z, a.bn_scale, a.bn_shift = bz.data_ptr(), bsc.data_ptr(), bsh.data_ptr()
            a.bn_mean, a.bn_invstd, a.bn_red, a.bn_slope = bmu.data_ptr(), bis.data_ptr(), bred.data_ptr(), float(bsl)
        ws = _gemm_workspace(a, dz)
        with timer.range('conv_gemm_dgrad/' + tag):
            call('cy_conv_gemm', C.byref(a), st)
        del ws
    return dx


def conv_wgrad(x, dz, k, stride, pad, nchw=False, tag='conv', in_affine=None, plan=None):
    x, dz = _f32(x, 'conv input'), _f32(dz, 'grad')
    B, Hi, Wi, Cin, xs = _x_geometry(x, nchw)
    _, Ho, Wo, Cout = dz.shape
    st = _stream()
    dW = _empty((Cout, Cin, k, k), dz)
    plan = plan or conv_plan(x.shape, Cout, k, stride, pad, nchw)
    if in_affine is not None and not plan.in_affine:
        raise _lib.HipExtensionError('a fused input affine needs the 4x4/stride-2 Winograd weight-gradient kernel')
    if plan.wgrad == 'conv_wino4_wgrad':
        ws = _empty((query('cy_wino4_wgrad_ws_floats', B, Hi, Wi, Cin, Cout),), dz)
        with timer.range('conv_wino4_wgrad/' + tag):
            call('cy_conv3x3_winograd4_wgrad', _ptr(x), _ptr(dz), _ptr(dW), _ptr(ws), B, Hi, Wi, Cin, Cout, st)
    elif plan.wgrad == 'conv_wino_wgrad':
        ws = _empty((query('cy_wino_wgrad_ws_floats', B, Cin, Cout),), dz)
        with timer.range('conv_wino_wgrad/' + tag):
            call('cy_conv3x3_winograd_wgrad', _ptr(x), _ptr(dz), _ptr(dW), _ptr(ws), B, Hi, Wi, Cin, Cout, st)
    elif plan.wgrad == 'conv_wino2_wgrad':
        ws = _empty((query('cy_wino2_wgrad_ws_floats', B, Cin, Cout),), dz)
        isc, ish, isl = in_affine if in_affine is not None else (None, None, 1.0)
        with timer.range('conv_wino2_wgrad/' + tag):
            call('cy_conv4x4s2_winograd_wgrad', _ptr(x), _ptr(dz), _ptr(dW), _ptr(ws), _ptr(isc), _ptr(ish), float(isl),
                 B, Hi, Wi, Cin, Cout, st)
    elif plan.wgrad == 'conv1_wgrad':
        ws = _empty((query('cy_conv1_3x3_wgrad_ws_floats', B, Hi, Wi, Cout),), dz)
        with timer.range('conv1_wgrad/' + tag):
            call('cy_conv1_3x3_wgrad', _ptr(x), _ptr(dz), _ptr(dW), _ptr(ws), B, Hi, Wi, Cout, st)
    else:
        a = ConvWgrad(X=x.data_ptr(), dZ=dz.data_ptr(), dW=dW.data_ptr(), slabs=None,
                      xs_b=xs[0], xs_y=xs[1], xs_x=xs[2], xs_c=xs[3], B=B, Hi=Hi, Wi=Wi, Cin=Cin, Ho=Ho, Wo=Wo, N=Cout,
                      KH=k, KW=k, stride=stride, pad=pad)
        ws = _empty((query('cy_conv_wgrad_ws_floats', C.byref(a)),), dz)
        a.slabs = ws.data_ptr()
        with timer.range('conv_wgrad/' + tag):
            call('cy_conv_wgrad', C.byref(a), st)
    return dW


FOLD_EVAL_BN = True
PARAM_EPOCH = 0


def _bump_param_epoch():
    global PARAM_EPOCH
    PARAM_EPOCH += 1


def fold_eval_bn(weight, bias, gamma, beta, bn):
    ts = (weight, bias, gamma, beta, bn.running_mean, bn.running_var)
    key = (PARAM_EPOCH, float(bn.eps)) + tuple((t.data_ptr(), t._version) if t is not None else None for t in ts)
    hit = getattr(bn, '_cy_fold', None)
    if hit is not None and hit[0] == key:
        return hit[1], hit[2]
    weight = _f32(weight, 'conv weight')
    Wf, bf = torch.empty_like(weight), _empty((weight.shape[0],), weight)
    call('cy_bn_fold_eval', _ptr(weight), _ptr(bias), _ptr(gamma), _ptr(beta), _ptr(bn.running_mean), _ptr(bn.running_var),
         float(bn.eps), _ptr(Wf), _ptr(bf), weight.shape[0], weight.numel() // weight.shape[0], _stream())
    bn._cy_fold = (key, Wf, bf)
    return Wf, bf


class ConvBlockCfg(object):

    def __init__(self, k, stride, pad, nchw_in=False, bn=None, slope=None, name='conv', defer_act=False, in_slope=None):
        self.k, self.stride, self.pad, self.nchw_in, self.name = k, stride, pad, nchw_in, name
        self.defer_act = defer_act
        self.in_slope = in_slope
        self.in_holder = None
        self.out_holder = None
        self.out_bf16 = False
        self.in_f32 = self.out_f32 = False
        self.bn = bn
        self.slope = slope


SYNC_BN = False


def _sync_world():
    import torch.distributed as dist
    if SYNC_BN and dist.is_available() and dist.is_initialized() and dist.get_world_size() > 1:
        return dist, dist.get_world_size()
    return None, 1


def _bn_finalize(stats, P, gamma, beta, bn, scale, shift, mean, invstd, N, st):
    dist, world = _sync_world()
    if dist is not None:
        dist.all_reduce(stats)
    call('cy_bn_finalize', _ptr(stats), P * world, _ptr(gamma), _ptr(beta), _ptr(bn.running_mean),
         _ptr(bn.running_var), float(bn.momentum), float(bn.eps), _ptr(scale), _ptr(shift), _ptr(mean),
         _ptr(invstd), N, _ptr(bn.num_batches_tracked), st)
    _bump_param_epoch()


def _leave(out, cfg, st):
    if not cfg.out_bf16:
        return out
    ob = torch.empty(out.shape, dtype=torch.bfloat16, device=out.device)
    call('cy_cast_f32_bf16', _ptr(out), _ptr(ob), out.numel(), st)
    return ob


class _ConvBlock(torch.autograd.Function):

    @staticmethod
    def forward(ctx, x, weight, bias, gamma, beta, cfg, in_scale=None, in_shift=None):
        x, weight = _f32(x, 'conv input'), _f32(weight, 'conv weight')
        st = _stream()
        N = weight.shape[0]
        bn = cfg.bn
        ctx.cfg, ctx.has_bias, ctx.bn_train = cfg, bias is not None, False
        ctx.set_materialize_grads(False)
        ctx.holder = None
        ctx.in_affine = ina = (in_scale, in_shift, float(cfg.in_slope)) if cfg.in_slope is not None else None
        if bn is None:
            if cfg.defer_act:
                raise _lib.HipExtensionError('defer_act needs a BatchNorm block')
            relu = cfg.slope is not None and cfg.slope == 0.0
            z = conv_forward(x, weight, bias, cfg.k, cfg.stride, cfg.pad, cfg.nchw_in, None, relu, cfg.name, ina)
            out = z
            if cfg.slope is not None and not relu:
                out = torch.empty_like(z)
                call('cy_affine_act', _ptr(z), _ptr(out), None, None, float(cfg.slope), z.numel() // N, N, st)
            ctx.save_for_backward(x, weight, z)
            return out
        scale, shift, mean, invstd = (_empty((N,), x) for _ in range(4))
        slope = 1.0 if cfg.slope is None else float(cfg.slope)
        plan = conv_plan(x.shape, N, cfg.k, cfg.stride, cfg.pad, cfg.nchw_in)
        ctx.conv1_m2 = None
        ctx.conv1_fused = bool(plan.conv1_bwd and bn.training and not cfg.defer_act and not x.requires_grad and 0.0 <= slope <= 1.0)
        if bn.training:
            stats = zero_pool.take((STATS_COPIES, N, 2), torch.float64, x.device)
            if ctx.conv1_fused:
                Bx, _, Hx, Wx = x.shape
                if plan.conv1_moments:
                    wsm = _empty((query('cy_conv1_3x3_stats_ws_floats', Bx, Hx),), x)
                    with timer.range('conv1_fwd_stats/' + cfg.name):
                        call('cy_conv1_3x3_stats', _ptr(x), _ptr(weight.contiguous()), _ptr(bias), _ptr(stats), _ptr(wsm),
                             Bx, Hx, Wx, N, st)
                    off = query('cy_conv1_3x3_stats_m2_offset', Bx, Hx)
                    ctx.conv1_m2 = wsm[off:off + 2048]
                else:
                    with timer.range('conv1_fwd_stats/' + cfg.name):
                        call('cy_conv1_3x3_fwd', _ptr(x), _ptr(weight.contiguous()), _ptr(bias), None, _ptr(stats), None, None,
                             1.0, Bx, Hx, Wx, N, st)
                z = x.new_empty(0)
                P = Bx * Hx * Wx
            else:
                z = conv_forward(x, weight, bias, cfg.k, cfg.stride, cfg.pad, cfg.nchw_in, stats, False, cfg.name, ina)
                P = z.numel() // N
            _bn_finalize(stats, P, gamma, beta, bn, scale, shift, mean, invstd, N, st)
            ctx.bn_train = True
        else:
            ctx.folded = bool(FOLD_EVAL_BN and not cfg.defer_act and ina is None and 0.0 <= slope <= 1.0)
            if ctx.folded:
                ctx.save_for_backward()
                if plan.conv1:
                    call('cy_bn_eval_scale_shift', _ptr(gamma), _ptr(beta), _ptr(bn.running_mean), _ptr(bn.running_var),
                         float(bn.eps), _ptr(scale), _ptr(shift), N, st)
                    return conv1_affine_act(x, weight, bias, scale, shift, slope, cfg.name, cfg.out_bf16)
                Wf, bf = fold_eval_bn(weight, bias, gamma, beta, bn)
                return _leave(conv_forward(x, Wf, bf, cfg.k, cfg.stride, cfg.pad, cfg.nchw_in, None, False, cfg.name, None, lrelu=slope), cfg, st)
            z = conv_forward(x, weight, bias, cfg.k, cfg.stride, cfg.pad, cfg.nchw_in, None, False, cfg.name, ina)
            P = z.numel() // N
            call('cy_bn_eval_scale_shift', _ptr(gamma), _ptr(beta), _ptr(bn.running_mean), _ptr(bn.running_var),
                 float(bn.eps), _ptr(scale), _ptr(shift), N, st)
        ctx.P = P
        ctx.save_for_backward(x, weight, z, scale, shift, mean, invstd, gamma, *([bias] if bias is not None else []))
        if cfg.defer_act:
            ctx.mark_non_differentiable(scale, shift)
            ctx.holder = cfg.out_holder = {'mean': mean, 'invstd': invstd, 'red': None} if ctx.bn_train else None
            return z, scale, shift
        if plan.conv1 and 0.0 <= slope <= 1.0:
            return conv1_affine_act(x, weight, bias, scale, shift, slope, cfg.name, cfg.out_bf16)
        out = torch.empty_like(z)
        call('cy_affine_act', _ptr(z), _ptr(out), _ptr(scale), _ptr(shift), slope, P, N, st)
        return _leave(out, cfg, st)

    @staticmethod
    def backward(ctx, da, *unused):
        cfg = ctx.cfg
        if da is None:
            raise _lib.HipExtensionError('conv block %s: no gradient reached its output' % cfg.name)
        if getattr(ctx, 'folded', False):
            raise _lib.HipExtensionError('backward through an eval-mode BatchNorm block is not implemented')
        da_bf16 = da.dtype == torch.bfloat16 and cfg.out_bf16
        if da_bf16 and not (cfg.bn is not None and ctx.bn_train and ctx.conv1_fused):
            daf = torch.empty(da.shape, dtype=torch.float32, device=da.device)
            call('cy_cast_bf16_f32', _ptr(da.contiguous()), _ptr(daf), da.numel(), _stream())
            da, da_bf16 = daf, False
        if not da_bf16:
            da = _f32(da, 'grad')
        st = _stream()
        saved = ctx.saved_tensors
        x, weight, z = saved[0], saved[1], saved[2]
        N = weight.shape[0]
        P = ctx.P if cfg.bn is not None else z.numel() // N
        plan = conv_plan(x.shape, N, cfg.k, cfg.stride, cfg.pad, cfg.nchw_in)
        dgamma = dbeta = dbias = dW = None
        if cfg.bn is None:
            if cfg.slope is not None:
                dz = torch.empty_like(z)
                call('cy_act_bwd', _ptr(z), _ptr(da), _ptr(dz), float(cfg.slope), z.numel(), st)
            else:
                dz = da
            if ctx.has_bias:
                dbias = _empty((N,), z)
                call('cy_channel_sum', _ptr(dz), _ptr(dbias), P, N, st)
        else:
            if not ctx.bn_train:
                raise _lib.HipExtensionError('backward through an eval-mode BatchNorm block is not implemented')
            scale, shift, mean, invstd, gamma = saved[3:8]
            slope = 1.0 if cfg.slope is None else float(cfg.slope)
            if ctx.conv1_fused:
                da = da.contiguous()
                bias_t = saved[8] if ctx.has_bias else None
                B, _, Hi, Wi = x.shape
                redc = zero_pool.take((STATS_COPIES, N, 2), torch.float64, z.device)
                dW, dbeta, dgamma = _empty(tuple(weight.shape), z), _empty((N,), z), _empty((N,), z)
                ws = _empty((query('cy_conv1_bn_bwd_wgrad_ws_floats', B, Hi, Wi, N),), z)
                dbias = _const_zeros(N, z) if ctx.has_bias else None
                if plan.conv1_onepass and ctx.conv1_m2 is not None and _sync_world()[0] is None:
                    with timer.range('conv1_bn_bwd_onepass/' + cfg.name):
                        call('cy_conv1_bn_bwd_onepass_bf16' if da_bf16 else 'cy_conv1_bn_bwd_onepass', _ptr(x), _ptr(weight),
                             _ptr(bias_t), _ptr(da), _ptr(scale), _ptr(shift), _ptr(mean), _ptr(invstd), slope,
                             _ptr(ctx.conv1_m2), _ptr(redc), _ptr(dW), _ptr(dgamma), _ptr(dbeta), None, _ptr(ws), B, Hi, Wi, N, st)
                    return None, dW, dbias, dgamma, dbeta, None, None, None
                with timer.range('conv1_bn_bwd_reduce/' + cfg.name):
                    call('cy_conv1_bn_bwd_reduce_bf16' if da_bf16 else 'cy_conv1_bn_bwd_reduce', _ptr(x), _ptr(weight), _ptr(bias_t), _ptr(da), _ptr(scale), _ptr(shift),
                         _ptr(mean), _ptr(invstd), slope, _ptr(redc), B, Hi, Wi, N, st)
                red = _empty((N, 2), z, torch.float64)
                dist, world = _sync_world()
                call('cy_bn_red_fold', _ptr(redc), STATS_COPIES, 1.0 / world, _ptr(red), _ptr(dgamma), _ptr(dbeta), N, st)
                if dist is not None:
                    dist.all_reduce(red)
                    call('cy_bn_red_fold', _ptr(red), 1, 1.0, None, _ptr(dgamma), _ptr(dbeta), N, st)
                with timer.range('conv1_bn_bwd_wgrad/' + cfg.name):
                    call('cy_conv1_bn_bwd_wgrad_bf16' if da_bf16 else 'cy_conv1_bn_bwd_wgrad', _ptr(x), _ptr(weight), _ptr(bias_t), _ptr(da), _ptr(scale), _ptr(shift),
                         _ptr(mean), _ptr(invstd), slope, _ptr(red), P, _ptr(dW), _ptr(ws), B, Hi, Wi, N, st)
                return None, dW, dbias, dgamma, dbeta, None, None, None
            premasked = False
            if ctx.holder is not None and ctx.holder.get('red') is not None:
                red = ctx.holder['red']
                ctx.holder['red'] = None
                premasked = bool(ctx.holder.pop('premasked', False))
                if premasked:
                    slope = 1.0
            else:
                red = _empty((N, 2), z, torch.float64)
                call('cy_bn_bwd_reduce', _ptr(z), _ptr(da), _ptr(scale), _ptr(shift), _ptr(mean), _ptr(invstd), slope,
                     _ptr(red), P, N, st)
            dist, world = _sync_world()
            if dist is not None:
                red = red.contiguous()
                call('cy_bn_red_fold', _ptr(red), 1, 1.0 / world, _ptr(red), None, None, N, st)
                dist.all_reduce(red)
            dz = torch.empty_like(z)
            dgamma, dbeta = _empty((N,), z), _empty((N,), z)
            if ctx.has_bias:
                dbias = _const_zeros(N, z)
            if plan.wgrad_bn and ctx.in_affine is None:
                red = red.contiguous()
                call('cy_bn_param_grad', _ptr(red), _ptr(dgamma), _ptr(dbeta), N, st)
                B_, Hi, Wi, Cin = x.shape
                dW = _empty(tuple(weight.shape), z)
                if premasked and plan.wgrad_bn4:
                    ws = _empty((query('cy_wino4_wgrad_ws_floats', B_, Hi, Wi, Cin, N),), z)
                    with timer.range('conv_wino4_wgrad_bn/' + cfg.name):
                        call('cy_conv3x3_winograd4_wgrad_bn', _ptr(_f32(x, 'conv input')), _ptr(z), _ptr(da), _ptr(dz), _ptr(scale),
                             _ptr(mean), _ptr(invstd), _ptr(red), P, _ptr(dW), _ptr(ws), B_, Hi, Wi, Cin, N, st)
                else:
                    ws = _empty((query('cy_wino_wgrad_ws_floats', B_, Cin, N),), z)
                    with timer.range('conv_wino_wgrad_bn/' + cfg.name):
                        call('cy_conv3x3_winograd_wgrad_bn', _ptr(_f32(x, 'conv input')), _ptr(z), _ptr(da), _ptr(dz), _ptr(scale),
                             _ptr(shift), _ptr(mean), _ptr(invstd), slope, 1 if premasked else 0, _ptr(red), P, _ptr(dW), _ptr(ws),
                             B_, Hi, Wi, Cin, N, st)
            else:
                call('cy_bn_bwd_apply', _ptr(z), _ptr(da), _ptr(dz), _ptr(scale), _ptr(shift), _ptr(mean), _ptr(invstd),
                     _ptr(gamma), slope, _ptr(red), _ptr(dgamma), _ptr(dbeta), P, N, st)
        if dW is None:
            dW = conv_wgrad(x, dz, cfg.k, cfg.stride, cfg.pad, cfg.nchw_in, cfg.name, ctx.in_affine, plan)
        dx = None
        if ctx.needs_input_grad[0]:
            if plan.dgrad is None:
                raise _lib.HipExtensionError('input gradient of an NCHW-input convolution is not implemented')
            fuse, h = None, cfg.in_holder
            if plan.dgrad_bn_fuse and ctx.in_affine is not None and h is not None:
                bred = zero_pool.take((STATS_COPIES, x.shape[3], 2), torch.float64, x.device)
                fuse = (x, ctx.in_affine[0], ctx.in_affine[1], h['mean'], h['invstd'], ctx.in_affine[2], bred)
            dx = conv_dgrad(dz, weight, tuple(x.shape), cfg.k, cfg.stride, cfg.pad, cfg.name, fuse, plan)
            if fuse is not None:
                h['premasked'] = plan.dgrad_premasks
                h['red'] = _empty((x.shape[3], 2), x, torch.float64)
                call('cy_bn_red_fold', _ptr(bred), STATS_COPIES, 1.0, _ptr(h['red']), None, None, x.shape[3], st)
        return dx, dW, dbias, dgamma, dbeta, None, None, None


def _bf(t, name='tensor'):
    if not (t.is_cuda and t.dtype == torch.bfloat16):
        raise _lib.HipExtensionError('%s must be a bfloat16 tensor on the GPU (got %s on %s)' % (name, t.dtype, t.device))
    return t if t.is_contiguous() else t.contiguous()


def bf16_layer_ok(k, stride, pad, cin, cout):
    return pad == 1 and ((k == 3 and stride == 1 and cout % 128 == 0) or (k == 4 and stride == 2)) and cin % 64 == 0 and cout % 64 == 0


def cast_bf16(x):
    return _CastBF16.apply(x)


class _CastBF16(torch.autograd.Function):
    @staticmethod
    def forward(ctx, x):
        x = _f32(x)
        y = torch.empty(x.shape, dtype=torch.bfloat16, device=x.device)
        call('cy_cast_f32_bf16', _ptr(x), _ptr(y), x.numel(), _stream())
        return y

    @staticmethod
    def backward(ctx, dy):
        if dy.dtype == torch.bfloat16:
            out = torch.empty(dy.shape, dtype=torch.float32, device=dy.device)
            call('cy_cast_bf16_f32', _ptr(_bf(dy)), _ptr(out), dy.numel(), _stream())
            return out
        return dy


def conv_forward_bf16(x, weight, bias, k, stride, pad, stats=None, tag='conv', lrelu=None, out_f32=False):
    x, weight = _bf(x, 'conv input'), _f32(weight, 'conv weight')
    B, Hi, Wi, Cin = x.shape
    Cout = weight.shape[0]
    Ho, Wo = (Hi + 2 * pad - k) // stride + 1, (Wi + 2 * pad - k) // stride + 1
    st = _stream()
    wp = torch.empty((query('cy_conv_bf16_packed_elems', k * k * Cin, Cout),), dtype=torch.bfloat16, device=x.device)
    call('cy_conv_bf16_pack_weights', _ptr(weight), _ptr(wp), Cout, Cin, k, k, k, k, 0, 0, 1, 0, st)
    z = torch.empty((B, Ho, Wo, Cout), dtype=torch.float32 if out_f32 else torch.bfloat16, device=x.device)
    a = _fwd_desc_bf16(x.shape, Cout, k, stride, pad, lrelu)
    a.X, a.Wp, a.Y = x.data_ptr(), wp.data_ptr(), z.data_ptr()
    a.bias, a.stats = bias.data_ptr() if bias is not None else None, stats.data_ptr() if stats is not None else None
    with timer.range('conv_bf16_fwd/' + tag):
        call('cy_conv_gemm_bf16', C.byref(a), 1 if out_f32 else 0, st)
    return z


BF16_DGRAD_ONE_LAUNCH = True
FUSE_BN_BWD_REDUCE_BF16 = True


def conv_dgrad_bf16(dz, weight, in_shape, k, stride, pad, out_f32=False, tag='conv', bn_fuse=None):
    dz, weight = _bf(dz, 'grad'), _f32(weight, 'conv weight')
    if bn_fuse is not None and out_f32:
        raise _lib.HipExtensionError('conv_dgrad_bf16: the fused BatchNorm-backward sums are built for the bf16 output')
    B, Hi, Wi, Cin = in_shape
    _, Ho, Wo, Cout = dz.shape
    st = _stream()
    dx = torch.empty((B, Hi, Wi, Cin), dtype=torch.float32 if out_f32 else torch.bfloat16, device=dz.device)
    classes, descs, one_launch = _dgrad_descs_bf16(in_shape, dz.shape, k, stride, pad)
    nel = query('cy_conv_bf16_packed_elems', ((k + stride - 1) // stride) ** 2 * Cout, Cin)
    wp = torch.empty((len(classes), nel), dtype=torch.bfloat16, device=dz.device)
    for i, c in enumerate(classes):
        call('cy_conv_bf16_pack_weights', _ptr(weight), _ptr(wp[i]), Cout, Cin, k, k, c['TH'], c['TW'], c['kh0'], c['kw0'],
             c['kstep'], 1, st)
        a = descs[i]
        a.X, a.Wp, a.Y = dz.data_ptr(), wp[i].data_ptr(), dx.data_ptr()
        if bn_fuse is not None:
            bz, bsc, bsh, bmu, bis, bsl, bred = bn_fuse
            a.bn_z, a.bn_scale, a.bn_shift = _bf(bz, 'producer z').data_ptr(), bsc.data_ptr(), bsh.data_ptr()
            a.bn_mean, a.bn_invstd, a.bn_red, a.bn_slope = bmu.data_ptr(), bis.data_ptr(), bred.data_ptr(), float(bsl)
    if one_launch:
        with timer.range('conv_bf16_dgrad/' + tag):
            call('cy_conv_gemm_bf16_classes', descs, len(classes), 1 if out_f32 else 0, st)
    else:
        for i in range(len(classes)):
            with timer.range('conv_bf16_dgrad/' + tag):
                call('cy_conv_gemm_bf16', C.byref(descs[i]), 1 if out_f32 else 0, st)
    return dx


def _fwd_desc_bf16(x_shape, Cout, k, stride, pad, lrelu=None):
    B, Hi, Wi, Cin = x_shape
    Ho, Wo = (Hi + 2 * pad - k) // stride + 1, (Wi + 2 * pad - k) // stride + 1
    return ConvGemm(xs_b=Hi * Wi * Cin, xs_y=Wi * Cin, xs_x=Cin, xs_c=1, B=B, Hi=Hi, Wi=Wi, Cin=Cin, Ho=Ho, Wo=Wo, N=Cout,
                    TH=k, TW=k, in_stride=stride, dy0=-pad, dx0=-pad, dstep=1, Hy=Ho, Wy=Wo, out_stride=1, out_oy=0, out_ox=0,
                    act=0 if lrelu is None else 2, act_slope=1.0 if lrelu is None else float(lrelu))


def _dgrad_descs_bf16(in_shape, dz_shape, k, stride, pad):
    B, Hi, Wi, Cin = in_shape
    _, Ho, Wo, Cout = dz_shape
    classes = dgrad_classes(Hi, Wi, k, stride, pad)
    descs = (ConvGemm * len(classes))()
    for i, c in enumerate(classes):
        descs[i] = ConvGemm(xs_b=Ho * Wo * Cout, xs_y=Wo * Cout, xs_x=Cout, xs_c=1, B=B, Hi=Ho, Wi=Wo, Cin=Cout,
                            Ho=c['Ho'], Wo=c['Wo'], N=Cin, TH=c['TH'], TW=c['TW'], in_stride=1, dy0=c['dy0'], dx0=c['dx0'],
                            dstep=c['dstep'], Hy=Hi, Wy=Wi, out_stride=c['out_stride'], out_oy=c['out_oy'], out_ox=c['out_ox'], act=0)
    same = all((c['TH'], c['TW'], c['Ho'], c['Wo'], c['dstep'], c['out_stride']) ==
               (classes[0]['TH'], classes[0]['TW'], classes[0]['Ho'], classes[0]['Wo'], classes[0]['dstep'], classes[0]['out_stride'])
               for c in classes)
    return classes, descs, BF16_DGRAD_ONE_LAUNCH and 1 < len(classes) <= 4 and same


def _plan_bf16(descs, ncls, out_f32, bnf):
    plan = (C.c_int * 5)()
    if bnf:
        for i in range(ncls):
            descs[i].bn_red = 1
    rc = query('cy_conv_gemm_bf16_plan', descs, ncls, 1 if out_f32 else 0, plan)
    if rc != 0:
        raise _lib.HipExtensionError('cy_conv_gemm_bf16_plan failed (code %d): %s' % (rc, query('capsyolo_last_error').decode()))
    return dict(BM=plan[0], BN=plan[1], TAPIN=plan[2], ntiles=plan[3], blocks=plan[4])


def conv_bf16_plans(op, in_shape, Cout, k, stride, pad, out_f32=False, bnf=False):
    B, Hi, Wi, Cin = in_shape
    if op == 'fwd':
        if bnf:
            raise ValueError('the fused BatchNorm-backward sums belong to the input gradient')
        return [_plan_bf16((ConvGemm * 1)(_fwd_desc_bf16(in_shape, Cout, k, stride, pad)), 1, out_f32, False)]
    Ho, Wo = (Hi + 2 * pad - k) // stride + 1, (Wi + 2 * pad - k) // stride + 1
    classes, descs, one_launch = _dgrad_descs_bf16(in_shape, (B, Ho, Wo, Cout), k, stride, pad)
    if one_launch:
        return [_plan_bf16(descs, len(classes), out_f32, bnf)]
    return [_plan_bf16((ConvGemm * 1)(descs[i]), 1, out_f32, bnf) for i in range(len(classes))]


def conv_wgrad_bf16(x, dz, k, stride, pad, tag='conv'):
    x, dz = _bf(x, 'conv input'), _bf(dz, 'grad')
    B, Hi, Wi, Cin = x.shape
    _, Ho, Wo, Cout = dz.shape
    nws = query('cy_conv_wgrad_bf16_ws_floats', B, Ho, Wo, Cin, Cout, k, stride)
    if nws < 0 or pad != 1:
        raise _lib.HipExtensionError('bf16 weight gradient: unsupported layer k=%d s=%d p=%d Cin=%d Cout=%d' % (k, stride, pad, Cin, Cout))
    ws = _empty((nws,), dz)
    dW = _empty((Cout, Cin, k, k), dz)
    with timer.range('conv_bf16_wgrad/' + tag):
        call('cy_conv_wgrad_bf16', _ptr(x), _ptr(dz), _ptr(dW), _ptr(ws), B, Hi, Wi, Cin, Ho, Wo, Cout, k, stride, _stream())
    return dW


class _ConvBlockBF16(torch.autograd.Function):

    @staticmethod
    def forward(ctx, x, weight, bias, gamma, beta, cfg):
        st = _stream()
        if cfg.in_f32:
            xf = _f32(x, 'conv input')
            x = torch.empty(xf.shape, dtype=torch.bfloat16, device=xf.device)
            call('cy_cast_f32_bf16', _ptr(xf), _ptr(x), xf.numel(), st)
        x, weight = _bf(x, 'conv input'), _f32(weight, 'conv weight')
        N = weight.shape[0]
        bn = cfg.bn
        if bn is None or cfg.slope is None:
            raise _lib.HipExtensionError('the bf16 path is built for conv -> BatchNorm -> LeakyReLU blocks')
        ctx.cfg, ctx.has_bias = cfg, bias is not None
        scale, shift, mean, invstd = (_empty((N,), weight) for _ in range(4))
        if bn.training:
            stats = zero_pool.take((STATS_COPIES, N, 2), torch.float64, x.device)
            z = conv_forward_bf16(x, weight, bias, cfg.k, cfg.stride, cfg.pad, stats, cfg.name)
            P = z.numel() // N
            _bn_finalize(stats, P, gamma, beta, bn, scale, shift, mean, invstd, N, st)
        else:
            if FOLD_EVAL_BN and 0.0 <= float(cfg.slope) <= 1.0:
                Wf, bf = fold_eval_bn(weight, bias, gamma, beta, bn)
                ctx.bn_train = False
                ctx.save_for_backward()
                return conv_forward_bf16(x, Wf, bf, cfg.k, cfg.stride, cfg.pad, None, cfg.name, lrelu=float(cfg.slope), out_f32=cfg.out_f32)
            z = conv_forward_bf16(x, weight, bias, cfg.k, cfg.stride, cfg.pad, None, cfg.name)
            P = z.numel() // N
            call('cy_bn_eval_scale_shift', _ptr(gamma), _ptr(beta), _ptr(bn.running_mean), _ptr(bn.running_var), float(bn.eps),
                 _ptr(scale), _ptr(shift), N, st)
        ctx.bn_train, ctx.P = bool(bn.training), P
        out_f32 = cfg.out_f32
        out = torch.empty(z.shape, dtype=torch.float32 if out_f32 else torch.bfloat16, device=z.device)
        call('cy_affine_act_bf16', _ptr(z), _ptr(out), _ptr(scale), _ptr(shift), float(cfg.slope), P, N, 1 if out_f32 else 0, st)
        ctx.save_for_backward(x, weight, z, scale, shift, mean, invstd)
        h = cfg.out_holder
        if h is not None:
            h.clear()
            if bn.training and not out_f32:
                h.update(z=z, scale=scale, shift=shift, mean=mean, invstd=invstd, slope=float(cfg.slope), red=None)
        return out

    @staticmethod
    def backward(ctx, da):
        cfg = ctx.cfg
        if not ctx.bn_train:
            raise _lib.HipExtensionError('backward through an eval-mode BatchNorm block is not implemented')
        x, weight, z, scale, shift, mean, invstd = ctx.saved_tensors
        st = _stream()
        N, P = weight.shape[0], ctx.P
        da_f32 = da.dtype == torch.float32
        da = _f32(da, 'grad') if da_f32 else _bf(da, 'grad')
        slope = float(cfg.slope)
        ho = cfg.out_holder
        if ho is not None and ho.get('red') is not None and not da_f32:
            red = ho['red']
            ho['red'] = None
            slope = 1.0
        else:
            red = _empty((N, 2), weight, torch.float64)
            call('cy_bn_bwd_reduce_bf16', _ptr(z), _ptr(da), 1 if da_f32 else 0, _ptr(scale), _ptr(shift), _ptr(mean), _ptr(invstd),
                 slope, _ptr(red), P, N, st)
        dist, world = _sync_world()
        if dist is not None:
            call('cy_bn_red_fold', _ptr(red), 1, 1.0 / world, _ptr(red), None, None, N, st)
            dist.all_reduce(red)
        dz = torch.empty_like(z)
        dgamma, dbeta = _empty((N,), weight), _empty((N,), weight)
        Bx, Hx, Wx, Cx = x.shape
        nws = -1
        if FUSE_BN_BWD_APPLY_BF16 and slope == 1.0 and not da_f32 and cfg.pad == 1:
            nws = query('cy_conv_wgrad_bf16_bn_ws_floats', Bx, z.shape[1], z.shape[2], Cx, N, cfg.k, cfg.stride)
        if nws >= 0:
            ws = _empty((nws,), weight)
            dW = _empty((N, Cx, cfg.k, cfg.k), weight)
            with timer.range('conv_bf16_wgrad_bn/' + cfg.name):
                call('cy_conv_wgrad_bf16_bn', _ptr(x), _ptr(da.contiguous()), _ptr(z), _ptr(dz), _ptr(dW), _ptr(ws), _ptr(scale), _ptr(mean),
                     _ptr(invstd), _ptr(red), _ptr(dgamma), _ptr(dbeta), Bx, Hx, Wx, Cx, z.shape[1], z.shape[2], N, cfg.k, cfg.stride, st)
        else:
            call('cy_bn_bwd_apply_bf16', _ptr(z), _ptr(da), 1 if da_f32 else 0, _ptr(dz), _ptr(scale), _ptr(shift), _ptr(mean),
                 _ptr(invstd), slope, _ptr(red), _ptr(dgamma), _ptr(dbeta), P, N, st)
            dW = conv_wgrad_bf16(x, dz, cfg.k, cfg.stride, cfg.pad, cfg.name)
        dx = None
        if ctx.needs_input_grad[0]:
            in_f32, hi = cfg.in_f32, cfg.in_holder
            fuse = None
            if (FUSE_BN_BWD_REDUCE_BF16 and hi is not None and hi.get('z') is not None and not in_f32
                    and tuple(hi['z'].shape) == tuple(x.shape)):
                Cin = x.shape[3]
                bred = zero_pool.take((STATS_COPIES, Cin, 2), torch.float64, x.device)
                fuse = (hi['z'], hi['scale'], hi['shift'], hi['mean'], hi['invstd'], hi['slope'], bred)
            dx = conv_dgrad_bf16(dz, weight, tuple(x.shape), cfg.k, cfg.stride, cfg.pad, in_f32, cfg.name, fuse)
            if fuse is not None:
                hi['red'] = _empty((x.shape[3], 2), weight, torch.float64)
                call('cy_bn_red_fold', _ptr(fuse[6]), STATS_COPIES, 1.0, _ptr(hi['red']), None, None, x.shape[3], st)
        dbias = _const_zeros(N, weight) if ctx.has_bias else None
        return dx, dW, dbias, dgamma, dbeta, None


def conv_block_bf16(x, weight, bias, gamma, beta, cfg):
    return _ConvBlockBF16.apply(x, weight, bias, gamma, beta, cfg)


def conv_block(x, weight, bias, gamma, beta, cfg, in_scale=None, in_shift=None):
    return _ConvBlock.apply(x, weight, bias, gamma, beta, cfg, in_scale, in_shift)


ROUTING_FORCE_GENERAL = False


ROUTING_PATHS = ('c1', 'rows_fused', 'rows_phased', 'general', 'mfma_fused', 'mfma_phased')
ROUTING_REGIONS = ('ds_all', 'V', 'SA', 'slabs', 'tail', 'W', 'cdb', 'du_hat', 'dW_splits')


def routing_plan(R, N, Cc, Din, Dout, n_iter, gather_g=0, gather_B=0, backward=False, force_general=None):
    a = RoutingFwd(R=R, N=N, C=Cc, Din=Din, Dout=Dout, n_iter=n_iter, gather_g=gather_g, gather_B=gather_B)
    out = (C.c_longlong * (7 + 3 * len(ROUTING_REGIONS)))()
    force = ROUTING_FORCE_GENERAL if force_general is None else force_general
    rc = query('cy_routing_plan', C.byref(a), int(backward), int(force), out, len(out))
    if rc:
        msg = _lib.load().capsyolo_last_error()
        raise _lib.HipExtensionError('cy_routing_plan failed (code %d): %s' % (rc, msg.decode() if msg else '?'))
    names = [n + '_all' if backward and n == 'V' else n for n in ROUTING_REGIONS]
    return {'path': ROUTING_PATHS[out[0]], 'row_blocks': out[1], 'nch': out[2], 'ic': out[3], 'cdb': bool(out[4]), 'total': out[5],
            'regions': [(names[out[7 + 3 * k]], out[8 + 3 * k], out[9 + 3 * k]) for k in range(out[6])]}


def _routing_call(kind, a, like):
    p = routing_plan(a.R, a.N, a.C, a.Din, a.Dout, a.n_iter, a.gather_g, a.gather_B, backward=kind == 'bwd')
    ws = _empty((p['total'],), like) if p['total'] else None
    a.ws = ws.data_ptr() if p['total'] else None
    with timer.range('routing_' + kind):
        call(('cy_routing_general_' if p['path'] == 'general' else 'cy_routing_') + kind, C.byref(a), _stream())


class _Routing(torch.autograd.Function):
    @staticmethod
    def forward(ctx, u, W, n_iter, gather_g, gather_B):
        u, W = _f32(u, 'capsule input'), _f32(W, 'route_weights')
        _, N, Cc, Din, Dout = W.shape
        if gather_g:
            R = gather_g * gather_g * gather_B
            out_shape = (gather_B, gather_g, gather_g, Cc, Dout)
        else:
            R = u.shape[0]
            out_shape = (R, Cc, Dout)
        v = _empty(out_shape, u)
        s_hist = _empty((n_iter, R, Cc, Dout), u)
        _routing_call('fwd', RoutingFwd(u=u.data_ptr(), W=W.data_ptr(), v_out=v.data_ptr(), s_hist=s_hist.data_ptr(), R=R, N=N, C=Cc,
                                        Din=Din, Dout=Dout, n_iter=n_iter, gather_g=gather_g, gather_B=gather_B, ws=None), u)
        ctx.save_for_backward(u, W, s_hist)
        ctx.dims = (R, N, Cc, Din, Dout, n_iter, gather_g, gather_B)
        return v

    @staticmethod
    def backward(ctx, dv):
        u, W, s_hist = ctx.saved_tensors
        R, N, Cc, Din, Dout, n_iter, g, gB = ctx.dims
        dv = _f32(dv, 'grad')
        du, dW = torch.empty_like(u), torch.empty_like(W)
        _routing_call('bwd', RoutingBwd(u=u.data_ptr(), W=W.data_ptr(), s_hist=s_hist.data_ptr(), dv=dv.data_ptr(), du=du.data_ptr(),
                                        dW=dW.data_ptr(), ws=None, R=R, N=N, C=Cc, Din=Din, Dout=Dout, n_iter=n_iter, gather_g=g,
                                        gather_B=gB), u)
        return du, dW, None, None, None


def routing(u, W, n_iter=3, gather_g=0, gather_B=0):
    return _Routing.apply(u, W, int(n_iter), int(gather_g), int(gather_B))


class _Rows(torch.autograd.Function):

    @staticmethod
    def forward(ctx, x, kind):
        x = _f32(x)
        D = x.shape[-1]
        rows = x.numel() // D
        st = _stream()
        ctx.kind = kind
        if kind == 'squash':
            y = torch.empty_like(x)
            call('cy_squash_fwd', _ptr(x), _ptr(y), rows, D, st)
            ctx.save_for_backward(x)
        else:
            y = _empty(x.shape[:-1], x)
            call('cy_length_fwd', _ptr(x), _ptr(y), rows, D, st)
            ctx.save_for_backward(x, y)
        return y

    @staticmethod
    def backward(ctx, dy):
        dy = _f32(dy)
        st = _stream()
        x = ctx.saved_tensors[0]
        D = x.shape[-1]
        rows = x.numel() // D
        dx = torch.empty_like(x)
        if ctx.kind == 'squash':
            call('cy_squash_bwd', _ptr(x), _ptr(dy), _ptr(dx), rows, D, st)
        else:
            call('cy_length_bwd', _ptr(x), _ptr(ctx.saved_tensors[1]), _ptr(dy), _ptr(dx), rows, D, st)
        return dx, None


def squash(x):
    return _Rows.apply(x, 'squash')


def length(x):
    return _Rows.apply(x, 'length')


class _Permute4(torch.autograd.Function):

    @staticmethod
    def forward(ctx, x, nb, dims, strides):
        x = _f32(x)
        out = _empty((nb,) + tuple(dims), x)
        call('cy_permute4', _ptr(x), _ptr(out), nb, dims[0], dims[1], dims[2], strides[0], strides[1], strides[2],
             strides[3], 0, _stream())
        ctx.args = (nb, dims, strides, tuple(x.shape))
        return out

    @staticmethod
    def backward(ctx, dout):
        nb, dims, strides, xshape = ctx.args
        dout = _f32(dout)
        dx = _empty(xshape, dout)
        call('cy_permute4', _ptr(dout), _ptr(dx), nb, dims[0], dims[1], dims[2], strides[0], strides[1], strides[2],
             strides[3], 1, _stream())
        return dx, None, None, None


def nchw_to_nhwc(x):
    B, Cc, H, W = x.shape
    return _Permute4.apply(x, B, (H, W, Cc), (Cc * H * W, W, 1, H * W))


def nhwc_to_nchw(x):
    B, H, W, Cc = x.shape
    return _Permute4.apply(x, B, (Cc, H, W), (H * W * Cc, 1, W * Cc, Cc))


def primary_caps_rows(z, n_caps):
    B, H, W, Cc = z.shape
    O = Cc // n_caps
    out = _Permute4.apply(z, B, (O, H * W, n_caps), (H * W * Cc, n_caps, Cc, 1))
    return out.view(B, O * H * W, n_caps)


class _MaxPool2(torch.autograd.Function):
    @staticmethod
    def forward(ctx, x):
        x = _f32(x)
        B, H, W, Cc = x.shape
        y = _empty((B, H // 2, W // 2, Cc), x)
        idx = _empty((B, H // 2, W // 2, Cc), x, torch.uint8)
        call('cy_maxpool2_fwd', _ptr(x), _ptr(y), _ptr(idx), B, H // 2, W // 2, Cc, _stream())
        ctx.save_for_backward(idx)
        ctx.shape = (B, H, W, Cc)
        return y

    @staticmethod
    def backward(ctx, dy):
        (idx,) = ctx.saved_tensors
        B, H, W, Cc = ctx.shape
        dy = _f32(dy)
        dx = _empty((B, H, W, Cc), dy) if (H % 2 == 0 and W % 2 == 0) else torch.zeros((B, H, W, Cc), device=dy.device)
        call('cy_maxpool2_bwd', _ptr(dy), _ptr(idx), _ptr(dx), B, H // 2, W // 2, Cc, _stream())
        return dx


def maxpool2(x):
    return _MaxPool2.apply(x)


FUSE_POOL = True


def pool_fusable(C, H, W, slope):
    return (FUSE_POOL and H % 2 == 0 and W % 2 == 0 and C % 4 == 0 and (C % 64 == 0 or C in (4, 8, 16, 32)) and slope is not None
            and 0.0 < slope <= 1.0)


class _AffineActMaxPool(torch.autograd.Function):

    @staticmethod
    def forward(ctx, z, scale, shift, slope, holder):
        z = _f32(z, 'conv output')
        B, H, W, Cc = z.shape
        y = _empty((B, H // 2, W // 2, Cc), z)
        idx = torch.empty((B, H // 2, W // 2, Cc), dtype=torch.uint8, device=z.device)
        with timer.range('affine_act_maxpool'):
            call('cy_affine_act_maxpool2', _ptr(z), _ptr(scale), _ptr(shift), float(slope), _ptr(y), _ptr(idx), B, H // 2, W // 2, Cc, _stream())
        ctx.save_for_backward(z, scale, shift, idx)
        ctx.slope, ctx.holder = float(slope), holder
        return y

    @staticmethod
    def backward(ctx, dy):
        z, scale, shift, idx = ctx.saved_tensors
        B, H, W, Cc = z.shape
        dy = _f32(dy, 'pooled gradient')
        h = ctx.holder
        d = torch.empty_like(z)
        red = zero_pool.take((Cc, 2), torch.float64, z.device)
        with timer.range('maxpool_bwd_bn'):
            call('cy_maxpool2_bwd_bn', _ptr(dy), _ptr(idx), _ptr(z), _ptr(scale), _ptr(shift), _ptr(h['mean']), _ptr(h['invstd']), ctx.slope,
                 _ptr(d), _ptr(red), B, H // 2, W // 2, Cc, _stream())
        h['red'], h['premasked'] = red, True
        return d, None, None, None, None


def affine_act_maxpool(z, scale, shift, slope, holder):
    return _AffineActMaxPool.apply(z, scale, shift, slope, holder)


class _Upsample(torch.autograd.Function):
    @staticmethod
    def forward(ctx, x, f):
        x = _f32(x)
        B, H, W, Cc = x.shape
        y = _empty((B, H * f, W * f, Cc), x)
        call('cy_upsample_fwd', _ptr(x), _ptr(y), B, H, W, Cc, f, _stream())
        ctx.args = (B, H, W, Cc, f)
        return y

    @staticmethod
    def backward(ctx, dy):
        B, H, W, Cc, f = ctx.args
        dy = _f32(dy)
        dx = _empty((B, H, W, Cc), dy)
        call('cy_upsample_bwd', _ptr(dy), _ptr(dx), B, H, W, Cc, f, _stream())
        return dx, None


def upsample_nearest(x, f):
    return _Upsample.apply(x, int(f))


class _Tanh(torch.autograd.Function):
    @staticmethod
    def forward(ctx, x):
        x = _f32(x)
        y = torch.empty_like(x)
        call('cy_tanh_fwd', _ptr(x), _ptr(y), x.numel(), _stream())
        ctx.save_for_backward(y)
        return y

    @staticmethod
    def backward(ctx, dy):
        (y,) = ctx.saved_tensors
        dy = _f32(dy)
        dx = torch.empty_like(y)
        call('cy_tanh_bwd', _ptr(y), _ptr(dy), _ptr(dx), y.numel(), _stream())
        return dx


def tanh(x):
    return _Tanh.apply(x)


class _YoloHead(torch.autograd.Function):
    @staticmethod
    def forward(ctx, x, split, n_classes):
        x = _f32(x)
        y = torch.empty_like(x)
        cells = x.numel() // (split + n_classes)
        call('cy_yolo_head_fwd', _ptr(x), _ptr(y), cells, split, n_classes, _stream())
        ctx.save_for_backward(y)
        ctx.args = (cells, split, n_classes)
        return y

    @staticmethod
    def backward(ctx, dy):
        (y,) = ctx.saved_tensors
        cells, split, n_classes = ctx.args
        dy = _f32(dy)
        dx = torch.empty_like(y)
        call('cy_yolo_head_bwd', _ptr(y), _ptr(dy), _ptr(dx), cells, split, n_classes, _stream())
        return dx, None, None


def yolo_head(x, split, n_classes):
    return _YoloHead.apply(x, int(split), int(n_classes))


class _PickCapsule(torch.autograd.Function):
    @staticmethod
    def forward(ctx, caps, y):
        caps = _f32(caps)
        B, Cc, D = caps.shape
        y = y.to(torch.int64).contiguous()
        out = _empty((B, D), caps)
        call('cy_pick_capsule', _ptr(caps), _ptr(y), _ptr(out), B, Cc, D, 0, _stream())
        ctx.save_for_backward(y)
        ctx.shape = (B, Cc, D)
        return out

    @staticmethod
    def backward(ctx, dout):
        (y,) = ctx.saved_tensors
        B, Cc, D = ctx.shape
        dout = _f32(dout)
        dcaps = _empty((B, Cc, D), dout)
        call('cy_pick_capsule', _ptr(dout), _ptr(y), _ptr(dcaps), B, Cc, D, 1, _stream())
        return dcaps, None


def pick_capsule(caps, y):
    return _PickCapsule.apply(caps, y)


def _scaled(grad, gout):
    out = torch.empty_like(grad)
    gout = gout.to(torch.float32).contiguous()
    call('cy_scale_by_device_scalar', _ptr(grad), _ptr(gout), _ptr(out), grad.numel(), _stream())
    return out


class _DarkCapsuleLoss(torch.autograd.Function):
    @staticmethod
    def forward(ctx, caps, y):
        caps = _f32(caps, 'caps')
        if not (y.is_cuda and y.dtype == torch.float64):
            y = y.to(device=caps.device, dtype=torch.float64)
        y = y.contiguous()
        B = caps.shape[0]
        cells = caps.numel() // (5 * B)
        loss, dcaps = _empty((), caps), torch.empty_like(caps)
        call('cy_darkcapsule_loss', _ptr(caps), _ptr(y), y.shape[-1], _ptr(loss), _ptr(dcaps), B, cells, _stream())
        ctx.save_for_backward(dcaps)
        return loss

    @staticmethod
    def backward(ctx, gout):
        return _scaled(ctx.saved_tensors[0], gout), None


class _DarkCapsule23Loss(torch.autograd.Function):

    @staticmethod
    def forward(ctx, caps, y, variant):
        caps = _f32(caps, 'caps')
        if not (y.is_cuda and y.dtype == torch.float64):
            y = y.to(device=caps.device, dtype=torch.float64)
        y = y.contiguous()
        B = caps.shape[0]
        Cc = y.shape[-1] - 5
        cells = y.numel() // (y.shape[-1] * B)
        loss, dcaps = _empty((), caps), torch.empty_like(caps)
        if variant == 2:
            if caps.shape[-1] != 5 + Cc:
                raise _lib.HipExtensionError('darkcapsule2_loss: caps last dim %d != 5 + n_classes %d' % (caps.shape[-1], Cc))
            call('cy_darkcapsule2_loss', _ptr(caps), _ptr(y), _ptr(loss), _ptr(dcaps), B, cells, Cc, _stream())
        else:
            if caps.dim() != 5 or caps.shape[3] != Cc:
                raise _lib.HipExtensionError('darkcapsule3_loss: caps must be [B,g,g,n_classes,D]; got %s' % (tuple(caps.shape),))
            call('cy_darkcapsule3_loss', _ptr(caps), _ptr(y), _ptr(loss), _ptr(dcaps), B, cells, Cc, caps.shape[4], _stream())
        ctx.save_for_backward(dcaps)
        return loss

    @staticmethod
    def backward(ctx, gout):
        return _scaled(ctx.saved_tensors[0], gout), None, None


def darkcapsule2_loss_fn(caps, y):
    return _DarkCapsule23Loss.apply(caps, y, 2)


def darkcapsule3_loss_fn(caps, y):
    return _DarkCapsule23Loss.apply(caps, y, 3)


class _CapsuleLoss(torch.autograd.Function):

    @staticmethod
    def forward(ctx, scores, y, x, recon, coef):
        scores = _f32(scores, 'scores')
        B, Cc = scores.shape
        y = y.to(torch.int64).contiguous()
        st = _stream()
        loss, dscores = _empty((), scores), torch.empty_like(scores)
        call('cy_margin_loss', _ptr(scores), _ptr(y), _ptr(loss), _ptr(dscores), B, Cc, st)
        if recon is not None:
            x, recon = _f32(x, 'x'), _f32(recon, 'recon')
            drecon = torch.empty_like(recon)
            call('cy_recon_loss_add', _ptr(x), _ptr(recon), float(coef) / B, _ptr(loss), _ptr(drecon), recon.numel(), st)
            ctx.save_for_backward(dscores, drecon)
        else:
            ctx.save_for_backward(dscores)
        return loss

    @staticmethod
    def backward(ctx, gout):
        saved = ctx.saved_tensors
        drecon = _scaled(saved[1], gout) if len(saved) > 1 else None
        return _scaled(saved[0], gout), None, None, drecon, None


class _DarkLoss(torch.autograd.Function):
    @staticmethod
    def forward(ctx, y_pred, y_true, nb, n_classes, l_coord, l_noobj, img):
        y_pred = _f32(y_pred, 'y_pred')
        if not (y_true.is_cuda and y_true.dtype == torch.float64):
            y_true = y_true.to(device=y_pred.device, dtype=torch.float64)
        y_true = y_true.contiguous()
        B, g = y_pred.shape[0], y_pred.shape[1]
        loss, avg_iou = _empty((), y_pred), _empty((), y_pred)
        dpred = torch.empty_like(y_pred)
        call('cy_dark_loss', _ptr(y_pred), _ptr(y_true), _ptr(loss), _ptr(avg_iou), _ptr(dpred), B, g, nb, n_classes,
             float(l_coord), float(l_noobj), float(img), _stream())
        ctx.save_for_backward(dpred)
        ctx.mark_non_differentiable(avg_iou)
        return loss, avg_iou

    @staticmethod
    def backward(ctx, gout, _g_iou):
        return _scaled(ctx.saved_tensors[0], gout), None, None, None, None, None, None


def darkcapsule_loss_fn(caps, y):
    return _DarkCapsuleLoss.apply(caps, y)


def capsule_loss_fn(scores, y, x=None, recon=None, coef=0.0):
    return _CapsuleLoss.apply(scores, y, x, recon, coef)


def dark_loss_fn(y_pred, y_true, nb, n_classes, l_coord, l_noobj, img):
    return _DarkLoss.apply(y_pred, y_true, nb, n_classes, l_coord, l_noobj, img)
```

### include/capsyolo_hip.h

```cpp
#ifndef CAPSYOLO_HIP_H
#define CAPSYOLO_HIP_H
#ifdef __cplusplus
extern "C" {
#endif

#define CY_EINVAL 10001

const char* capsyolo_last_error(void);
int capsyolo_abi_version(void);

typedef struct {
  const float* X; const float* Wp; float* Y; const float* bias; double* stats;
  long long xs_b, xs_y, xs_x, xs_c;
  int B, Hi, Wi, Cin;
  int Ho, Wo, N;
  int TH, TW, in_stride, dy0, dx0, dstep;
  int Hy, Wy, out_stride, out_oy, out_ox;
  int act;
  const float* bn_z; const float* bn_scale; const float* bn_shift; const float* bn_mean; const float* bn_invstd;
  double* bn_red;
  float bn_slope;
  float act_slope;
  float* ws; long long ws_floats;
} cy_conv_gemm_t;

int cy_conv1_3x3_fwd(const float* X, const float* W, const float* bias, float* Y, double* stats, const float* scale,
                     const float* shift, float slope, int B, int H, int Wd, int Cout, void* stream);
long long cy_conv1_3x3_stats_ws_floats(int B, int H);
long long cy_conv1_3x3_stats_m2_offset(int B, int H);
int cy_conv1_3x3_stats(const float* X, const float* W, const float* bias, double* stats, float* ws, int B, int H, int Wd,
                       int Cout, void* stream);
long long cy_conv1_3x3_wgrad_ws_floats(int B, int H, int Wd, int Cout);
int cy_conv1_3x3_wgrad(const float* X, const float* dZ, float* dW, float* ws, int B, int H, int Wd, int Cout, void* stream);
int cy_conv1_bn_bwd_reduce(const float* X, const float* W, const float* bias, const float* dA, const float* scale,
                           const float* shift, const float* mean, const float* invstd, float slope, double* red, int B, int H,
                           int Wd, int Cout, void* stream);
long long cy_conv1_bn_bwd_wgrad_ws_floats(int B, int H, int Wd, int Cout);
int cy_conv1_bn_bwd_wgrad(const float* X, const float* W, const float* bias, const float* dA, const float* scale,
                          const float* shift, const float* mean, const float* invstd, float slope, const double* red,
                          long long count, float* dW, float* ws, int B, int H, int Wd, int Cout, void* stream);
int cy_conv1_3x3_fwd_act_bf16(const float* X, const float* W, const float* bias, void* Y, const float* scale,
                              const float* shift, float slope, int B, int H, int Wd, int Cout, void* stream);
int cy_conv1_bn_bwd_reduce_bf16(const float* X, const float* W, const float* bias, const void* dA, const float* scale,
                                const float* shift, const float* mean, const float* invstd, float slope, double* red, int B,
                                int H, int Wd, int Cout, void* stream);
int cy_conv1_bn_bwd_wgrad_bf16(const float* X, const float* W, const float* bias, const void* dA, const float* scale,
                               const float* shift, const float* mean, const float* invstd, float slope, const double* red,
                               long long count, float* dW, float* ws, int B, int H, int Wd, int Cout, void* stream);
int cy_conv1_bn_bwd_onepass(const float* X, const float* W, const float* bias, const float* dA, const float* scale,
                            const float* shift, const float* mean, const float* invstd, float slope, const double* M2,
                            double* redc, float* dW, float* dgamma, float* dbeta, double* red_out, float* ws, int B, int H,
                            int Wd, int Cout, void* stream);
int cy_conv1_bn_bwd_onepass_bf16(const float* X, const float* W, const float* bias, const void* dA, const float* scale,
                                 const float* shift, const float* mean, const float* invstd, float slope, const double* M2,
                                 double* redc, float* dW, float* dgamma, float* dbeta, double* red_out, float* ws, int B, int H,
                                 int Wd, int Cout, void* stream);

long long cy_conv_packed_floats(int K, int N);
int cy_conv_pack_weights(const float* W, float* Wp, int Cout, int Cin, int KH, int KW,
                         int TH, int TW, int kh0, int kw0, int kstep, int transpose, void* stream);
#define CY_STATS_COPIES 16
int cy_conv_gemm(const cy_conv_gemm_t* a, void* stream);
long long cy_conv_gemm_ws_floats(const cy_conv_gemm_t* a);

typedef struct {
  const float* X; const float* dZ; float* dW; float* slabs;
  long long xs_b, xs_y, xs_x, xs_c;
  int B, Hi, Wi, Cin;
  int Ho, Wo, N;
  int KH, KW, stride, pad;
} cy_conv_wgrad_t;
long long cy_conv_wgrad_ws_floats(const cy_conv_wgrad_t* a);
int cy_conv_wgrad(const cy_conv_wgrad_t* a, void* stream);

long long cy_wino_packed_floats(int Cin, int N);
int cy_wino_pack_weights(const float* W, float* U, int Cout, int Cin, int transpose, void* stream);
int cy_conv3x3_winograd(const float* X, const float* U, float* Y, const float* bias, double* stats, float out_slope,
                        int B, int H, int W, int Cin, int Cout, void* stream);
long long cy_wino_split_ws_floats(int B, int H, int W, int Cin, int Cout, int plain);
int cy_conv3x3_winograd_ws(const float* X, const float* U, float* Y, const float* bias, double* stats, float out_slope,
                           int B, int H, int W, int Cin, int Cout, float* ws, long long ws_floats, void* stream);
long long cy_wino4_packed_floats(int Cin, int N);
int cy_wino4_pack_weights(const float* W, float* U, int Cout, int Cin, int transpose, void* stream);
int cy_conv3x3_winograd4(const float* X, const float* U, float* Y, const float* bias, double* stats, float out_slope,
                         int B, int H, int W, int Cin, int Cout, void* stream);
int cy_wino4_wgrad_ok(int B, int H, int W, int Cin, int Cout);
long long cy_wino4_wgrad_ws_floats(int B, int H, int W, int Cin, int Cout);
int cy_conv3x3_winograd4_wgrad(const float* X, const float* dZ, float* dW, float* ws,
                               int B, int H, int W, int Cin, int Cout, void* stream);
int cy_conv3x3_winograd4_wgrad_bn(const float* X, const float* Z, const float* dA, float* dZ, const float* scale,
                                  const float* mean, const float* invstd, const double* red, long long count,
                                  float* dW, float* ws, int B, int H, int W, int Cin, int Cout, void* stream);
long long cy_wino_wgrad_ws_floats(int B, int Cin, int Cout);
int cy_conv3x3_winograd_wgrad(const float* X, const float* dZ, float* dW, float* ws,
                              int B, int H, int W, int Cin, int Cout, void* stream);
int cy_conv3x3_winograd_wgrad_bn(const float* X, const float* Z, const float* dA, float* dZ, const float* scale,
                                 const float* shift, const float* mean, const float* invstd, float slope, int premasked,
                                 const double* red, long long count, float* dW, float* ws,
                                 int B, int H, int W, int Cin, int Cout, void* stream);

long long cy_wino2_packed_floats(int Cin, int N);
int cy_wino2_pack_weights(const float* W, float* U, int Cout, int Cin, void* stream);
int cy_conv4x4s2_winograd(const float* X, const float* U, float* Y, const float* bias, double* stats,
                          const float* in_scale, const float* in_shift, float in_slope, float out_slope,
                          int B, int H, int W, int Cin, int Cout, void* stream);
int cy_wino4s2_ok(int B, int H, int W, int Cin, int Cout);
long long cy_wino4s2_packed_floats(int Cin, int N);
int cy_wino4s2_pack_weights(const float* W, float* U, int Cout, int Cin, void* stream);
int cy_conv4x4s2_winograd4(const float* X, const float* U, float* Y, const float* bias, double* stats,
                           const float* in_scale, const float* in_shift, float in_slope, float out_slope,
                           int B, int H, int W, int Cin, int Cout, void* stream);
int cy_wino4s2_dgrad_ok(int B, int H, int W, int Cin, int Cout);
long long cy_wino4s2_dgrad_packed_floats(int Cin, int Cout);
int cy_wino4s2_pack_dgrad_weights(const float* W, float* U, int Cout, int Cin, void* stream);
int cy_conv4x4s2_winograd4_dgrad(const float* dZ, const float* U, float* dX, const float* bn_z, const float* bn_scale,
                                 const float* bn_shift, const float* bn_mean, const float* bn_invstd, float bn_slope,
                                 double* bn_red, int B, int H, int W, int Cin, int Cout, void* stream);
long long cy_wino2_wgrad_ws_floats(int B, int Cin, int Cout);
int cy_conv4x4s2_winograd_wgrad(const float* X, const float* dZ, float* dW, float* ws,
                                const float* in_scale, const float* in_shift, float in_slope,
                                int B, int H, int W, int Cin, int Cout, void* stream);

long long cy_wino2_dgrad_packed_floats(int Cin, int Cout);
int cy_wino2_pack_dgrad_weights(const float* W, float* U, int Cout, int Cin, void* stream);
int cy_conv4x4s2_winograd_dgrad(const float* dZ, const float* U, float* dX, const float* bn_z, const float* bn_scale,
                                const float* bn_shift, const float* bn_mean, const float* bn_invstd, float bn_slope,
                                double* bn_red, int B, int H, int W, int Cin, int Cout, void* stream);

int cy_channel_sum(const float* dZ, float* out, long long P, int N, void* stream);

long long cy_conv_bf16_packed_elems(int K, int N);
int cy_conv_bf16_pack_weights(const float* W, void* Wp, int Cout, int Cin, int KH, int KW, int TH, int TW, int kh0, int kw0,
                              int kstep, int transpose, void* stream);
int cy_conv_gemm_bf16(const cy_conv_gemm_t* a, int out_f32, void* stream);
int cy_conv_gemm_bf16_classes(const cy_conv_gemm_t* a, int ncls, int out_f32, void* stream);
int cy_conv_gemm_bf16_plan(const cy_conv_gemm_t* a, int ncls, int out_f32, int* plan5);
long long cy_conv_wgrad_bf16_ws_floats(int B, int Ho, int Wo, int Cin, int Cout, int KH, int stride);
int cy_conv_wgrad_bf16(const void* X, const void* dZ, float* dW, float* ws, int B, int Hi, int Wi, int Cin, int Ho, int Wo,
                       int Cout, int KH, int stride, void* stream);
long long cy_conv_wgrad_bf16_bn_ws_floats(int B, int Ho, int Wo, int Cin, int Cout, int KH, int stride);
int cy_conv_wgrad_bf16_bn(const void* X, const void* D, const void* Z, void* dZ, float* dW, float* ws, const float* scale,
                          const float* mean, const float* invstd, const double* red, float* dgamma, float* dbeta, int B, int Hi,
                          int Wi, int Cin, int Ho, int Wo, int Cout, int KH, int stride, void* stream);
int cy_affine_act_bf16(const void* Z, void* A, const float* scale, const float* shift, float slope, long long P, int N,
                       int out_f32, void* stream);
int cy_bn_bwd_reduce_bf16(const void* Z, const void* dA, int da_f32, const float* scale, const float* shift, const float* mean,
                          const float* invstd, float slope, double* red, long long P, int N, void* stream);
int cy_bn_bwd_apply_bf16(const void* Z, const void* dA, int da_f32, void* dZ, const float* scale, const float* shift,
                         const float* mean, const float* invstd, float slope, const double* red, float* dgamma, float* dbeta,
                         long long P, int N, void* stream);
int cy_cast_f32_bf16(const float* in, void* out, long long n, void* stream);
int cy_cast_bf16_f32(const void* in, float* out, long long n, void* stream);

int cy_bn_finalize(const double* stats, long long count, const float* gamma, const float* beta,
                   float* running_mean, float* running_var, float momentum, float eps,
                   float* scale, float* shift, float* mean, float* invstd, int N, long long* num_batches_tracked, void* stream);
int cy_bn_red_fold(const double* red_copies, int copies, double scale, double* red_out, float* dgamma, float* dbeta,
                   int N, void* stream);
int cy_bn_eval_scale_shift(const float* gamma, const float* beta, const float* running_mean,
                           const float* running_var, float eps, float* scale, float* shift, int N, void* stream);
int cy_bn_fold_eval(const float* W, const float* bias, const float* gamma, const float* beta, const float* running_mean,
                    const float* running_var, float eps, float* Wf, float* bf, int Cout, int per_out, void* stream);
int cy_affine_act(const float* Z, float* A, const float* scale, const float* shift, float slope,
                  long long P, int N, void* stream);
int cy_bn_bwd_reduce(const float* Z, const float* dA, const float* scale, const float* shift,
                     const float* mean, const float* invstd, float slope, double* red,
                     long long P, int N, void* stream);
int cy_bn_bwd_apply(const float* Z, const float* dA, float* dZ, const float* scale, const float* shift,
                    const float* mean, const float* invstd, const float* gamma, float slope,
                    const double* red, float* dgamma, float* dbeta, long long P, int N, void* stream);
int cy_bn_param_grad(const double* red, float* dgamma, float* dbeta, int N, void* stream);
int cy_act_bwd(const float* Z, const float* dA, float* dZ, float slope, long long n, void* stream);

typedef struct {
  const float* u; const float* W; float* v_out; float* s_hist;
  int R, N, C, Din, Dout, n_iter;
  int gather_g, gather_B;
  float* ws;
} cy_routing_fwd_t;
long long cy_routing_fwd_ws_floats(const cy_routing_fwd_t* a);
int cy_routing_fwd(const cy_routing_fwd_t* a, void* stream);

typedef struct {
  const float* u; const float* W; const float* s_hist; const float* dv;
  float* du;
  float* dW;
  float* ws;
  int R, N, C, Din, Dout, n_iter;
  int gather_g, gather_B;
} cy_routing_bwd_t;
long long cy_routing_bwd_ws_floats(const cy_routing_bwd_t* a);
int cy_routing_bwd(const cy_routing_bwd_t* a, void* stream);

int cy_routing_specialised(const cy_routing_fwd_t* a);
long long cy_routing_general_fwd_ws_floats(const cy_routing_fwd_t* a);
int cy_routing_general_fwd(const cy_routing_fwd_t* a, void* stream);
long long cy_routing_general_bwd_ws_floats(const cy_routing_bwd_t* a);
int cy_routing_general_bwd(const cy_routing_bwd_t* a, void* stream);
int cy_routing_plan(const cy_routing_fwd_t* a, int backward, int force_general, long long* out, int n);

int cy_squash_fwd(const float* s, float* v, long long rows, int D, void* stream);
int cy_squash_bwd(const float* s, const float* dv, float* ds, long long rows, int D, void* stream);
int cy_length_fwd(const float* v, float* len, long long rows, int D, void* stream);
int cy_length_bwd(const float* v, const float* len, const float* dlen, float* dv, long long rows, int D, void* stream);

int cy_darkcapsule_loss(const float* caps, const double* y, int ystride, float* loss_out, float* dcaps,
                        int B, int cells, void* stream);
int cy_darkcapsule2_loss(const float* caps, const double* y, float* loss_out, float* dcaps, int B, int cells, int C,
                         void* stream);
int cy_darkcapsule3_loss(const float* caps, const double* y, float* loss_out, float* dcaps, int B, int cells, int C, int D,
                         void* stream);
int cy_margin_loss(const float* scores, const long long* y, float* loss_out, float* dscores,
                   int B, int C, void* stream);
int cy_recon_loss_add(const float* x, const float* recon, float coef_over_B, float* loss_out, float* drecon,
                      long long n, void* stream);
int cy_dark_loss(const float* y_pred, const double* y_true, float* loss_out, float* avg_iou_out, float* dpred,
                 int B, int g, int nb, int C, float l_coord, float l_noobj, float img_size, void* stream);
int cy_scale_by_device_scalar(const float* in, const float* scalar, float* out, long long n, void* stream);

int cy_center_u8(const unsigned char* src, float* dst, int B, int H, int W, int C, int to_nchw, void* stream);
int cy_permute4(const float* in, float* out, long long nb, int d1, int d2, int d3, long long sb, long long s1,
                long long s2, long long s3, int scatter, void* stream);
int cy_affine_act_maxpool2(const float* Z, const float* scale, const float* shift, float slope, float* Y, unsigned char* idx,
                           int B, int Ho, int Wo, int C, void* stream);
int cy_maxpool2_bwd_bn(const float* dP, const unsigned char* idx, const float* Z, const float* scale, const float* shift,
                       const float* mean, const float* invstd, float slope, float* D, double* red, int B, int Ho, int Wo, int C,
                       void* stream);
int cy_maxpool2_fwd(const float* x, float* y, unsigned char* idx, int B, int Ho, int Wo, int C, void* stream);
int cy_maxpool2_bwd(const float* dy, const unsigned char* idx, float* dx, int B, int Ho, int Wo, int C, void* stream);
int cy_upsample_fwd(const float* x, float* y, int B, int Hi, int Wi, int C, int f, void* stream);
int cy_upsample_bwd(const float* dy, float* dx, int B, int Hi, int Wi, int C, int f, void* stream);
int cy_tanh_fwd(const float* x, float* y, long long n, void* stream);
int cy_tanh_bwd(const float* y, const float* dy, float* dx, long long n, void* stream);
int cy_yolo_head_fwd(const float* x, float* y, long long cells, int split, int C, void* stream);
int cy_yolo_head_bwd(const float* y, const float* dy, float* dx, long long cells, int split, int C, void* stream);
int cy_yolo_decode_boxes(const float* y, const long long* image_hw, double img_h, double img_w, int B, int g, int nb, int C,
                         float conf_th, int* count, int* image_idx, double* xy, int* cls, int max_boxes, void* stream);
int cy_detect_confusion(const int* gt_idx, const double* gt_xy, int n_gt, const int* pr_idx, const double* pr_xy, int n_pr,
                        int n_images, double iou_th, int max_per_image, int* out4, void* stream);
int cy_crop_resize_u8(const unsigned char* imgs, const long long* img_off, const int* img_hw, int n_images, long long imgs_bytes,
                      const int* box_img, const int* rect, int n, int OH, int OW, float shift, float scale, int to_nchw,
                      float* out, int* err, void* stream);
int cy_combine_scores(const float* dark, const float* scores, const int* box_img, const double* box_xy, int n,
                      const long long* image_hw, double side, int B, int g, int D, int C, int* winner, float* y_hat, int* err,
                      void* stream);
int cy_yolo_decode_boxes_conf(const float* y, const long long* image_hw, double img_h, double img_w, int B, int g, int nb, int C,
                              float conf_th, int* count, int* image_idx, double* xy, int* cls, float* conf, int max_boxes,
                              void* stream);
int cy_confusion_sweep(const int* gt_key, const double* gt_xy, const float* gt_conf, int n_gt, const int* pr_key,
                       const double* pr_xy, const float* pr_conf, int n_pr, int n_groups, int C, const double* conf_ths, int K,
                       const double* iou_ths, int T, int max_per_group, int* out, int* err, void* stream);
int cy_draw_boxes_u8(unsigned char* imgs, const long long* img_off, const int* img_hw, int n_images, long long imgs_bytes,
                     const int* box_img, const int* box_xy, const unsigned char* box_color, const int* box_label, int n,
                     int max_items, const unsigned char* glyphs, int* err, void* stream);
#define CY_PASTE_OUT_U8 0
#define CY_PASTE_OUT_F32_NHWC 1
#define CY_PASTE_OUT_F32_NCHW 2
int cy_paste_resize_max_pastes(void);
int cy_paste_resize_u8(const unsigned char* imgs, const long long* img_off, const int* img_hw, int n_images, long long imgs_bytes,
                       const unsigned char* signs, const long long* sign_off, const int* sign_hw, int n_signs, long long signs_bytes,
                       const int* sample_img, const int* sample_rect, const int* begin, int n, const int* pastes, int n_pastes,
                       int OH, int OW, int mode, void* out, int* err, void* stream);
int cy_gather_jitter_u8(const unsigned char* set, const long long* labels, int n_set, int H, int W, const int* shift,
                        const float* light, const int* index, int B, float* x_out, long long* y_out, int* err, void* stream);
long long cy_rank_ws_ints(int N, int C);
int cy_rank_counts(const float* scores, const long long* labels, const int* order, int N, int C, int* ws, int* counts,
                   int* correct, int* err, void* stream);
int cy_pick_capsule(const float* caps, const long long* y, float* out, int B, int C, int D, int backward, void* stream);
typedef struct {
  const float* caps; const long long* labels; const float* deltas; const float* x;
  const float* lin_w; const float* lin_b; const float* w4; const float* b4; const float* w7; const float* b7;
  const float* w10; const float* b10; const float* w12; const float* b12;
  float* out_f32; unsigned char* out_u8; float* sqerr; int* err;
  int n, C, D, n_delta;
} cy_decoder_t;
int cy_decoder_fwd(const cy_decoder_t* a, void* stream);

int cy_zero_bytes(void* p, long long nbytes, void* stream);
int cy_multi_copy(const void* table, const void* blockmap, int n_blocks, int chunk, float* flat, int unpack, float scale,
                  void* stream);
int cy_adam_multi(const void* table, const void* blockmap, int n_blocks, int chunk,
                  float lr, float beta1, float beta2, float eps, float bias_corr1, float bias_corr2,
                  void* stream);
int cy_adam_multi_dev(const void* table, const void* blockmap, int n_blocks, int chunk, const float* hyper, void* stream);

#ifdef __cplusplus
}
#endif
#endif
```

Baseline: 707.5 images/s.

## Store leaky-ReLU sign bitmask in conv1 forward to skip recompute in backward

The first-layer fused conv+BN+activation forward kernel now writes a packed bitmask of pre-activation signs. The one-pass backward reads this mask to apply the leaky-ReLU derivative, so it no longer reloads input patches and reruns the forward convolution MFMAs. This trades a small extra write and read of the mask for removing recomputation in backward. The path is enabled only for the fp32 gradient, single-process, moments/onepass case.

New measurement: 715.1 images/s (median of 6 runs). 1.1% higher.

```diff
diff --git a/cs231-capsule-yolo-traffic-sign-detection_amd/_lib.py b/cs231-capsule-yolo-traffic-sign-detection_amd/_lib.py
--- a/cs231-capsule-yolo-traffic-sign-detection_amd/_lib.py
+++ b/cs231-capsule-yolo-traffic-sign-detection_amd/_lib.py
@@ -61,6 +61,8 @@
     'cy_conv1_3x3_stats': [_P, _P, _P, _P, _P, _I, _I, _I, _I, _P],
     'cy_conv1_bn_bwd_onepass': [_P, _P, _P, _P, _P, _P, _P, _P, _F, _P, _P, _P, _P, _P, _P, _P, _I, _I, _I, _I, _P],
     'cy_conv1_bn_bwd_onepass_bf16': [_P, _P, _P, _P, _P, _P, _P, _P, _F, _P, _P, _P, _P, _P, _P, _P, _I, _I, _I, _I, _P],
+    'cy_conv1_3x3_fwd_act_mask': [_P, _P, _P, _P, _P, _P, _F, _P, _I, _I, _I, _I, _P],
+    'cy_conv1_bn_bwd_onepass_mask': [_P, _P, _P, _P, _P, _P, _P, _P, _P, _F, _P, _P, _P, _P, _P, _P, _P, _I, _I, _I, _I, _P],
     'cy_conv1_3x3_wgrad': [_P, _P, _P, _P, _I, _I, _I, _I, _P],
     'cy_conv1_bn_bwd_reduce': [_P, _P, _P, _P, _P, _P, _P, _P, _F, _P, _I, _I, _I, _I, _P],
     'cy_conv1_bn_bwd_reduce_bf16': [_P, _P, _P, _P, _P, _P, _P, _P, _F, _P, _I, _I, _I, _I, _P],
@@ -163,6 +165,7 @@
     'cy_conv1_3x3_stats_ws_floats': (_L, [_I, _I]),
     'cy_conv1_3x3_stats_m2_offset': (_L, [_I, _I]),
     'cy_conv1_bn_bwd_wgrad_ws_floats': (_L, [_I, _I, _I, _I]),
+    'cy_conv1_signmask_bytes': (_L, [_I, _I, _I, _I]),
     'cy_wino2_packed_floats': (_L, [_I, _I]),
     'cy_wino4s2_packed_floats': (_L, [_I, _I]),
     'cy_wino4s2_ok': (_I, [_I, _I, _I, _I, _I]),
diff --git a/cs231-capsule-yolo-traffic-sign-detection_amd/csrc/conv1.hip b/cs231-capsule-yolo-traffic-sign-detection_amd/csrc/conv1.hip
--- a/cs231-capsule-yolo-traffic-sign-detection_amd/csrc/conv1.hip
+++ b/cs231-capsule-yolo-traffic-sign-detection_amd/csrc/conv1.hip
@@ -18,10 +18,17 @@
   const float* scale; const float* shift; float slope;
   int B, H, Wd, Cout;
   long long ntiles;
+  void* mask;
 };
 
-template <int NT, bool AFF, bool STORE, bool OBF = false>
+template <int NT> struct Conv1MaskWord;
+template <> struct Conv1MaskWord<4> { typedef unsigned type __attribute__((ext_vector_type(2))); };
+template <> struct Conv1MaskWord<2> { typedef unsigned type; };
+template <> struct Conv1MaskWord<1> { typedef unsigned short type; };
+
+template <int NT, bool AFF, bool STORE, bool OBF = false, bool MASK = false>
 __global__ __launch_bounds__(256, 1) void conv1_fwd_kernel(Conv1Args a) {
+  static_assert(!MASK || (AFF && STORE && !OBF), "the sign mask belongs to the fp32 activation pass");
   const int t = threadIdx.x, lane = t & 63, wave = t >> 6;
   const int li = lane & 31, lh = lane >> 5;
   const long long gw = (long long)blockIdx.x * 4 + wave, nw = (long long)gridDim.x * 4;
@@ -51,9 +58,11 @@
   for (int nt = 0; nt < NT; ++nt) { ssum[nt] = 0.f; ssq[nt] = 0.f; }
   constexpr bool aff = AFF;
   float asc[NT];
+  float mb[NT], msh[NT];
 #pragma unroll
   for (int nt = 0; nt < NT; ++nt) {
     asc[nt] = aff ? a.scale[NT * li + nt] : 1.f;
+    if constexpr (MASK) { mb[nt] = bv[nt]; msh[nt] = a.shift[NT * li + nt]; }
     if (aff) bv[nt] = bv[nt] * asc[nt] + a.shift[NT * li + nt];
   }
 
@@ -93,6 +102,7 @@
 #pragma unroll
       for (int nt = 0; nt < NT; ++nt) acc[nt] = __builtin_amdgcn_mfma_f32_32x32x2f32(acur[s], wreg[nt][s], acc[nt], 0, 0, 0);
     float* yp = a.Y + (size_t)tile * 32 * a.Cout + NT * li;
+    unsigned mw[2] = {0u, 0u};
 #pragma unroll
     for (int r = 0; r < 16; ++r) {
       typedef float vecn __attribute__((ext_vector_type(NT)));
@@ -104,6 +114,11 @@
           const float y = __builtin_fmaf(acc[nt][r], asc[nt], bv[nt]);
           const float ys = y * a.slope;
           asm("v_max_f32 %0, %1, %2" : "=v"(v[nt]) : "v"(y), "v"(ys));
+          if constexpr (MASK) {
+            const float yb = __builtin_fmaf(acc[nt][r] + mb[nt], asc[nt], msh[nt]);
+            asm("v_cmp_lt_f32_e32 vcc, 0, %1\n\tv_addc_co_u32_e32 %0, vcc, %0, %0, vcc"
+                : "+v"(mw[NT == 4 ? r >> 3 : 0]) : "v"(yb) : "vcc");
+          }
         } else {
           v[nt] = acc[nt][r] + bv[nt];
           ssum[nt] += v[nt];
@@ -134,6 +149,12 @@
         CY_C1_ST(o, (vecn*)(yp + (size_t)p * a.Cout));
       }
     }
+    if constexpr (MASK) {
+      typedef typename Conv1MaskWord<NT>::type mword;
+      mword* mp = (mword*)a.mask + (size_t)tile * 64 + lane;
+      if constexpr (NT == 4) CY_C1_ST((mword{mw[0], mw[1]}), mp);
+      else CY_C1_ST((mword)mw[0], mp);
+    }
 #pragma unroll
     for (int s = 0; s < 14; ++s) acur[s] = anext[s];
   }
@@ -326,10 +347,13 @@
   float* slabs;
   int B, H, Wd, Cout;
   long long ntiles;
+  const void* mask;
 };
 
 template <int NT, int PASS, bool GBF = false>
 __global__ __launch_bounds__(256, 1) void conv1_bn_bwd_kernel(Conv1BnArgs a) {
+  static_assert(PASS != 3 || !GBF, "the sign-mask pass reads an fp32 gradient");
+  constexpr bool RECOMP = PASS != 3;
   typedef float vecn __attribute__((ext_vector_type(NT)));
   const int t = threadIdx.x, lane = t & 63, wave = t >> 6;
   const int li = lane & 31, lh = lane >> 5;
@@ -338,17 +362,19 @@
   const size_t plane = (size_t)a.H * a.Wd;
   int toff[14], tky[14], tkx[14];
   float wreg[NT][14];
-#pragma unroll
-  for (int s = 0; s < 14; ++s) {
-    const int k = 2 * s + lh;
-    const int kk = k < 27 ? k : 0;
-    const int c = kk / 9, kh = (kk % 9) / 3, kw = kk % 3;
-    tky[s] = k < 27 ? kh - 1 : (1 << 20);
-    tkx[s] = kw - 1;
-    toff[s] = (int)(c * plane) + (kh - 1) * a.Wd + (kw - 1);
-#pragma unroll
-    for (int nt = 0; nt < NT; ++nt)
-      wreg[nt][s] = k < 27 ? a.W[((size_t)(NT * li + nt) * 3 + c) * 9 + kh * 3 + kw] : 0.f;
+  if constexpr (RECOMP) {
+#pragma unroll
+    for (int s = 0; s < 14; ++s) {
+      const int k = 2 * s + lh;
+      const int kk = k < 27 ? k : 0;
+      const int c = kk / 9, kh = (kk % 9) / 3, kw = kk % 3;
+      tky[s] = k < 27 ? kh - 1 : (1 << 20);
+      tkx[s] = kw - 1;
+      toff[s] = (int)(c * plane) + (kh - 1) * a.Wd + (kw - 1);
+#pragma unroll
+      for (int nt = 0; nt < NT; ++nt)
+        wreg[nt][s] = k < 27 ? a.W[((size_t)(NT * li + nt) * 3 + c) * 9 + kh * 3 + kw] : 0.f;
+    }
   }
   const int kt = li < 27 ? li : 0;
   const int wc = kt / 9, wkh = (kt % 9) / 3, wkw = kt % 3;
@@ -357,8 +383,10 @@
 #pragma unroll
   for (int nt = 0; nt < NT; ++nt) {
     const int c = NT * li + nt;
-    bv[nt] = a.bias != nullptr ? a.bias[c] : 0.f;
-    sc[nt] = a.scale[c]; sh[nt] = a.shift[c]; is[nt] = a.invstd[c]; nm[nt] = -a.mean[c] * is[nt];
+    if constexpr (RECOMP) {
+      bv[nt] = a.bias != nullptr ? a.bias[c] : 0.f;
+      sc[nt] = a.scale[c]; sh[nt] = a.shift[c]; is[nt] = a.invstd[c]; nm[nt] = -a.mean[c] * is[nt];
+    }
     m1[nt] = PASS == 1 ? (float)(a.red_in[2 * c] * a.inv_count) : 0.f;
     m2[nt] = PASS == 1 ? (float)(a.red_in[2 * c + 1] * a.inv_count) : 0.f;
   }
@@ -374,18 +402,22 @@
     const float* px = p0 + li;
     const bool inner = y >= 1 && y + 1 < a.H && seg >= 1 && seg + 1 < segs;
     if (inner) {
-#pragma unroll
-      for (int s = 0; s < 14; ++s) av[s] = (s < 13 || lh == 0) ? px[toff[s]] : 0.f;
+      if constexpr (RECOMP) {
+#pragma unroll
+        for (int s = 0; s < 14; ++s) av[s] = (s < 13 || lh == 0) ? px[toff[s]] : 0.f;
+      }
       if (PASS >= 1) {
 #pragma unroll
         for (int s = 0; s < 16; ++s) bw[s] = p0[woff + (s & 3) + 8 * (s >> 2)];
       }
     } else {
-#pragma unroll
-      for (int s = 0; s < 14; ++s) {
-        const bool ok = (unsigned)(y + tky[s]) < (unsigned)a.H && (unsigned)(seg * 32 + li + tkx[s]) < (unsigned)a.Wd;
-        const float v = px[ok ? toff[s] : 0];
-        av[s] = ok ? v : 0.f;
+      if constexpr (RECOMP) {
+#pragma unroll
+        for (int s = 0; s < 14; ++s) {
+          const bool ok = (unsigned)(y + tky[s]) < (unsigned)a.H && (unsigned)(seg * 32 + li + tkx[s]) < (unsigned)a.Wd;
+          const float v = px[ok ? toff[s] : 0];
+          av[s] = ok ? v : 0.f;
+        }
       }
       if (PASS >= 1) {
         const bool rowok = (unsigned)(y + wkh - 1) < (unsigned)a.H;
@@ -432,22 +464,41 @@
 #pragma unroll
       for (int r = 0; r < 16; ++r) g[r] = CY_C1_LD((const vecn*)(pg + (size_t)((r & 3) + 8 * (r >> 2) + 4 * lh) * a.Cout));
     }
+    unsigned mw[2] = {0u, 0u};
+    if constexpr (!RECOMP) {
+      typedef typename Conv1MaskWord<NT>::type mword;
+      const mword m = CY_C1_LD((const mword*)a.mask + (size_t)tile * 64 + lane);
+      if constexpr (NT == 4) { mw[0] = m[0]; mw[1] = m[1]; }
+      else if constexpr (NT == 2) mw[0] = m;
+      else mw[0] = (unsigned)m << 16;
+    }
     const long long tn = tile + nw;
     if (tn < a.ntiles) load_img(tn, anext, bwnext);
     f32x16 acc[NT];
-#pragma unroll
-    for (int nt = 0; nt < NT; ++nt)
-#pragma unroll
-      for (int r = 0; r < 16; ++r) acc[nt][r] = 0.f;
-#pragma unroll
-    for (int s = 0; s < 14; ++s)
-#pragma unroll
-      for (int nt = 0; nt < NT; ++nt) acc[nt] = __builtin_amdgcn_mfma_f32_32x32x2f32(acur[s], wreg[nt][s], acc[nt], 0, 0, 0);
+    if constexpr (RECOMP) {
+#pragma unroll
+      for (int nt = 0; nt < NT; ++nt)
+#pragma unroll
+        for (int r = 0; r < 16; ++r) acc[nt][r] = 0.f;
+#pragma unroll
+      for (int s = 0; s < 14; ++s)
+#pragma unroll
+        for (int nt = 0; nt < NT; ++nt) acc[nt] = __builtin_amdgcn_mfma_f32_32x32x2f32(acur[s], wreg[nt][s], acc[nt], 0, 0, 0);
+    }
 #pragma unroll
     for (int r = 0; r < 16; ++r) {
       float dzr[NT];
 #pragma unroll
       for (int nt = 0; nt < NT; ++nt) {
+        if constexpr (!RECOMP) {
+          unsigned& m = mw[NT == 4 ? r >> 3 : 0];
+          const float gv = ((const float*)&g[r])[nt];
+          const float d = (int)m < 0 ? gv : gv * a.slope;
+          m <<= 1;
+          b1[nt] += d;
+          dzr[nt] = d;
+          continue;
+        }
         const float z = acc[nt][r] + bv[nt];
         const float y = __builtin_fmaf(z, sc[nt], sh[nt]);
         const float gv = ((const float*)&g[r])[nt];
@@ -468,14 +519,16 @@
         for (int nt = 0; nt < NT; ++nt) accw[nt] = __builtin_amdgcn_mfma_f32_32x32x2f32(dzr[nt], bwcur[r], accw[nt], 0, 0, 0);
       }
     }
-#pragma unroll
-    for (int s = 0; s < 14; ++s) acur[s] = anext[s];
+    if constexpr (RECOMP) {
+#pragma unroll
+      for (int s = 0; s < 14; ++s) acur[s] = anext[s];
+    }
     if (PASS >= 1) {
 #pragma unroll
       for (int s = 0; s < 16; ++s) bwcur[s] = bwnext[s];
     }
   }
-  if (PASS == 0 || PASS == 2) {
+  if (PASS == 0 || PASS >= 2) {
     double* rd = a.red_out + (size_t)((blockIdx.x * 4 + wave) % CY_STATS_COPIES) * a.Cout * 2;
 #pragma unroll
     for (int nt = 0; nt < NT; ++nt) {
@@ -743,7 +796,7 @@
   CY_REQUIRE(Cout == 32 || Cout == 64 || Cout == 128, "cy_conv1_3x3_wgrad: Cout=%d must be 32, 64 or 128", Cout);
   CY_REQUIRE((long long)3 * H * Wd < (1ll << 30), "cy_conv1_3x3_wgrad: image too large for 32-bit offsets");
   Conv1Args a;
-  a.X = X; a.W = nullptr; a.bias = nullptr; a.Y = const_cast<float*>(dZ); a.stats = nullptr;
+  a.X = X; a.W = nullptr; a.bias = nullptr; a.Y = const_cast<float*>(dZ); a.stats = nullptr; a.mask = nullptr;
   a.scale = a.shift = nullptr; a.slope = 1.f;
   a.B = B; a.H = H; a.Wd = Wd; a.Cout = Cout;
   a.ntiles = (long long)B * H * (Wd / 32);
@@ -779,7 +832,7 @@
   CY_REQUIRE(red != nullptr, "%s: red is NULL", who);
   Conv1BnArgs a;
   a.X = X; a.W = W; a.bias = bias; a.dA = (const float*)dA; a.scale = scale; a.shift = shift; a.mean = mean; a.invstd = invstd;
-  a.slope = slope; a.red_out = red; a.red_in = nullptr; a.inv_count = 0.0; a.slabs = nullptr;
+  a.slope = slope; a.red_out = red; a.red_in = nullptr; a.inv_count = 0.0; a.slabs = nullptr; a.mask = nullptr;
   a.B = B; a.H = H; a.Wd = Wd; a.Cout = Cout; a.ntiles = (long long)B * H * (Wd / 32);
   long long blocks = 0;
   rc = conv1_blocks(a.ntiles, &blocks, who);
@@ -819,11 +872,12 @@
 static int conv1_bn_bwd_onepass_impl(const char* who, const float* X, const float* W, const float* bias, const void* dA, bool da_bf16,
                                      const float* scale, const float* shift, const float* mean, const float* invstd, float slope,
                                      const double* M2, double* redc, float* dW, float* dgamma, float* dbeta, double* red_out,
-                                     float* ws, int B, int H, int Wd, int Cout, void* stream) {
+                                     float* ws, int B, int H, int Wd, int Cout, void* stream, const void* mask = nullptr) {
   int rc = conv1_bn_check(who, X, W, (const float*)dA, scale, shift, mean, invstd, slope, B, H, Wd, Cout);
   if (rc) return rc;
   CY_REQUIRE(M2 && redc && dW && dgamma && dbeta && ws, "%s: NULL argument", who);
   Conv1BnArgs a;
+  a.mask = mask;
   a.X = X; a.W = W; a.bias = bias; a.dA = (const float*)dA; a.scale = scale; a.shift = shift; a.mean = mean; a.invstd = invstd;
   a.slope = slope; a.red_out = redc; a.red_in = nullptr; a.inv_count = 0.0; a.slabs = ws;
   a.B = B; a.H = H; a.Wd = Wd; a.Cout = Cout; a.ntiles = (long long)B * H * (Wd / 32);
@@ -831,7 +885,11 @@
   rc = conv1_blocks(a.ntiles, &blocks, who);
   if (rc) return rc;
   hipStream_t s = (hipStream_t)stream;
-  if (da_bf16) {
+  if (mask != nullptr) {
+    if (Cout == 128) conv1_bn_bwd_kernel<4, 3><<<(unsigned)blocks, 256, 0, s>>>(a);
+    else if (Cout == 64) conv1_bn_bwd_kernel<2, 3><<<(unsigned)blocks, 256, 0, s>>>(a);
+    else conv1_bn_bwd_kernel<1, 3><<<(unsigned)blocks, 256, 0, s>>>(a);
+  } else if (da_bf16) {
 #ifdef CY_C1_F32MM
     if (Cout == 128) conv1_bn_bwd_kernel<4, 2, true><<<(unsigned)blocks, 256, 0, s>>>(a);
     else if (Cout == 64) conv1_bn_bwd_kernel<2, 2, true><<<(unsigned)blocks, 256, 0, s>>>(a);
@@ -867,6 +925,16 @@
                                    dW, dgamma, dbeta, red_out, ws, B, H, Wd, Cout, stream);
 }
 
+extern "C" int cy_conv1_bn_bwd_onepass_mask(const float* X, const float* W, const float* bias, const float* dA, const void* mask,
+                                            const float* scale, const float* shift, const float* mean, const float* invstd, float slope,
+                                            const double* M2, double* redc, float* dW, float* dgamma, float* dbeta, double* red_out,
+                                            float* ws, int B, int H, int Wd, int Cout, void* stream) {
+  CY_REQUIRE(mask != nullptr, "cy_conv1_bn_bwd_onepass_mask: mask is NULL");
+  CY_REQUIRE((((uintptr_t)dA | (uintptr_t)mask) & 15) == 0, "cy_conv1_bn_bwd_onepass_mask: operands must be 16-byte aligned");
+  return conv1_bn_bwd_onepass_impl("cy_conv1_bn_bwd_onepass_mask", X, W, bias, dA, false, scale, shift, mean, invstd, slope, M2, redc, dW,
+                                   dgamma, dbeta, red_out, ws, B, H, Wd, Cout, stream, mask);
+}
+
 extern "C" long long cy_conv1_bn_bwd_wgrad_ws_floats(int B, int H, int Wd, int Cout) {
   return cy_conv1_3x3_wgrad_ws_floats(B, H, Wd, Cout);
 }
@@ -880,7 +948,7 @@
   CY_REQUIRE(red && dW && ws && count > 0, "cy_conv1_bn_bwd_wgrad: bad arguments");
   Conv1BnArgs a;
   a.X = X; a.W = W; a.bias = bias; a.dA = (const float*)dA; a.scale = scale; a.shift = shift; a.mean = mean; a.invstd = invstd;
-  a.slope = slope; a.red_out = nullptr; a.red_in = red; a.inv_count = 1.0 / (double)count; a.slabs = ws;
+  a.slope = slope; a.red_out = nullptr; a.red_in = red; a.inv_count = 1.0 / (double)count; a.slabs = ws; a.mask = nullptr;
   a.B = B; a.H = H; a.Wd = Wd; a.Cout = Cout; a.ntiles = (long long)B * H * (Wd / 32);
   long long blocks = 0;
   rc = conv1_blocks(a.ntiles, &blocks, who);
@@ -922,37 +990,57 @@
                                  ws, B, H, Wd, Cout, stream);
 }
 
-extern "C" int cy_conv1_3x3_fwd(const float* X, const float* W, const float* bias, float* Y, double* stats,
-                                const float* scale, const float* shift, float slope, int B, int H, int Wd, int Cout,
-                                void* stream) {
-  CY_REQUIRE(X && W && (Y || (stats && !scale)) && B > 0 && H > 0 && Wd > 0, "cy_conv1_3x3_fwd: bad arguments");
-  CY_REQUIRE((scale == nullptr) == (shift == nullptr), "cy_conv1_3x3_fwd: scale and shift go together");
+static int conv1_fwd_impl(const char* who, const float* X, const float* W, const float* bias, float* Y, double* stats,
+                         const float* scale, const float* shift, float slope, void* mask, int B, int H, int Wd, int Cout,
+                         void* stream) {
+  CY_REQUIRE(X && W && (Y || (stats && !scale)) && B > 0 && H > 0 && Wd > 0, "%s: bad arguments", who);
+  CY_REQUIRE((scale == nullptr) == (shift == nullptr), "%s: scale and shift go together", who);
   CY_REQUIRE(scale == nullptr || (stats == nullptr && slope >= 0.f && slope <= 1.f),
-             "cy_conv1_3x3_fwd: the affine pass takes no statistics and a slope in [0, 1]");
-  CY_REQUIRE(Wd % 32 == 0, "cy_conv1_3x3_fwd: W=%d must be a multiple of 32", Wd);
-  CY_REQUIRE(Cout == 32 || Cout == 64 || Cout == 128, "cy_conv1_3x3_fwd: Cout=%d must be 32, 64 or 128", Cout);
-  CY_REQUIRE((long long)3 * H * Wd < (1ll << 30), "cy_conv1_3x3_fwd: image too large for 32-bit offsets");
+             "%s: the affine pass takes no statistics and a slope in [0, 1]", who);
+  CY_REQUIRE(Wd % 32 == 0, "%s: W=%d must be a multiple of 32", who, Wd);
+  CY_REQUIRE(Cout == 32 || Cout == 64 || Cout == 128, "%s: Cout=%d must be 32, 64 or 128", who, Cout);
+  CY_REQUIRE((long long)3 * H * Wd < (1ll << 30), "%s: image too large for 32-bit offsets", who);
   Conv1Args a;
   a.X = X; a.W = W; a.bias = bias; a.Y = Y; a.stats = stats;
   a.scale = scale; a.shift = shift; a.slope = slope;
   a.B = B; a.H = H; a.Wd = Wd; a.Cout = Cout;
   a.ntiles = (long long)B * H * (Wd / 32);
+  a.mask = mask;
   long long blocks = 0;
-  int rc = conv1_blocks(a.ntiles, &blocks, "cy_conv1_3x3_fwd");
+  int rc = conv1_blocks(a.ntiles, &blocks, who);
   if (rc) return rc;
   hipStream_t s = (hipStream_t)stream;
-#define CY_CONV1_LAUNCH(NT_)                                                                  \
-  do {                                                                                         \
-    if (scale) conv1_fwd_kernel<NT_, true, true><<<(unsigned)blocks, 256, 0, s>>>(a);          \
-    else if (Y) conv1_fwd_kernel<NT_, false, true><<<(unsigned)blocks, 256, 0, s>>>(a);        \
-    else conv1_fwd_kernel<NT_, false, false><<<(unsigned)blocks, 256, 0, s>>>(a);              \
+#define CY_CONV1_LAUNCH(NT_)                                                                             \
+  do {                                                                                                    \
+    if (mask) conv1_fwd_kernel<NT_, true, true, false, true><<<(unsigned)blocks, 256, 0, s>>>(a);         \
+    else if (scale) conv1_fwd_kernel<NT_, true, true><<<(unsigned)blocks, 256, 0, s>>>(a);                \
+    else if (Y) conv1_fwd_kernel<NT_, false, true><<<(unsigned)blocks, 256, 0, s>>>(a);                   \
+    else conv1_fwd_kernel<NT_, false, false><<<(unsigned)blocks, 256, 0, s>>>(a);                         \
   } while (0)
   if (Cout == 128) CY_CONV1_LAUNCH(4);
   else if (Cout == 64) CY_CONV1_LAUNCH(2);
   else CY_CONV1_LAUNCH(1);
 #undef CY_CONV1_LAUNCH
-  CY_LAUNCH_CHECK("cy_conv1_3x3_fwd");
+  CY_LAUNCH_CHECK(who);
   return 0;
+}
+
+extern "C" int cy_conv1_3x3_fwd(const float* X, const float* W, const float* bias, float* Y, double* stats,
+                                const float* scale, const float* shift, float slope, int B, int H, int Wd, int Cout,
+                                void* stream) {
+  return conv1_fwd_impl("cy_conv1_3x3_fwd", X, W, bias, Y, stats, scale, shift, slope, nullptr, B, H, Wd, Cout, stream);
+}
+
+extern "C" long long cy_conv1_signmask_bytes(int B, int H, int Wd, int Cout) {
+  if (B <= 0 || H <= 0 || Wd <= 0 || Wd % 32 || !(Cout == 32 || Cout == 64 || Cout == 128)) return -1;
+  return (long long)B * H * Wd * (Cout / 8);
+}
+
+extern "C" int cy_conv1_3x3_fwd_act_mask(const float* X, const float* W, const float* bias, float* Y, const float* scale,
+                                         const float* shift, float slope, void* mask, int B, int H, int Wd, int Cout, void* stream) {
+  CY_REQUIRE(Y && scale && shift, "cy_conv1_3x3_fwd_act_mask: bad arguments");
+  CY_REQUIRE((((uintptr_t)Y | (uintptr_t)mask) & 15) == 0, "cy_conv1_3x3_fwd_act_mask: operands must be 16-byte aligned");
+  return conv1_fwd_impl("cy_conv1_3x3_fwd_act_mask", X, W, bias, Y, nullptr, scale, shift, slope, mask, B, H, Wd, Cout, stream);
 }
 
 extern "C" int cy_conv1_3x3_fwd_act_bf16(const float* X, const float* W, const float* bias, void* Y, const float* scale,
@@ -963,7 +1051,7 @@
   CY_REQUIRE(Cout == 32 || Cout == 64 || Cout == 128, "cy_conv1_3x3_fwd_act_bf16: Cout=%d must be 32, 64 or 128", Cout);
   CY_REQUIRE((long long)3 * H * Wd < (1ll << 30), "cy_conv1_3x3_fwd_act_bf16: image too large for 32-bit offsets");
   Conv1Args a;
-  a.X = X; a.W = W; a.bias = bias; a.Y = (float*)Y; a.stats = nullptr;
+  a.X = X; a.W = W; a.bias = bias; a.Y = (float*)Y; a.stats = nullptr; a.mask = nullptr;
   a.scale = scale; a.shift = shift; a.slope = slope;
   a.B = B; a.H = H; a.Wd = Wd; a.Cout = Cout;
   a.ntiles = (long long)B * H * (Wd / 32);
diff --git a/cs231-capsule-yolo-traffic-sign-detection_amd/ops.py b/cs231-capsule-yolo-traffic-sign-detection_amd/ops.py
--- a/cs231-capsule-yolo-traffic-sign-detection_amd/ops.py
+++ b/cs231-capsule-yolo-traffic-sign-detection_amd/ops.py
@@ -117,6 +117,7 @@
 USE_CONV1_MOMENTS = True
 FUSE_BN_BWD_APPLY_BF16 = True
 USE_CONV1_ONEPASS = True
+CONV1_SIGNMASK = True
 CONV1_MOMENTS_MIN_PIXELS = 1 << 18
 USE_CONV1_BWD = True
 USE_CONV1 = True
@@ -145,7 +146,8 @@
     'conv1',
     'conv1_bwd',
     'conv1_moments',
-    'conv1_onepass'])
+    'conv1_onepass',
+    'conv1_signmask'])
 _WINO3_DGRAD = ('conv_wino_dgrad', 'conv_wino4_dgrad')
 
 
@@ -189,9 +191,11 @@
             wgrad, in_affine = 'conv_wino2_wgrad', not relu
     dgrad_bn_fuse = bool(FUSE_BN_BWD_REDUCE and dgrad is not None and dgrad not in _WINO3_DGRAD and Cin % 4 == 0)
     conv1_bwd = bool(conv1 and USE_CONV1_BWD)
+    conv1_moments = bool(conv1_bwd and USE_CONV1_MOMENTS and B * Hi * Wi >= CONV1_MOMENTS_MIN_PIXELS)
+    conv1_onepass = bool(conv1 and USE_CONV1_ONEPASS)
     return ConvPlan(fwd, dgrad, wgrad, in_affine, dgrad_bn_fuse, dgrad_bn_fuse and dgrad in ('conv_wino2_dgrad', 'conv_wino42_dgrad'),
-                    wgrad_bn, wgrad_bn4, conv1, conv1_bwd,
-                    bool(conv1_bwd and USE_CONV1_MOMENTS and B * Hi * Wi >= CONV1_MOMENTS_MIN_PIXELS), bool(conv1 and USE_CONV1_ONEPASS))
+                    wgrad_bn, wgrad_bn4, conv1, conv1_bwd, conv1_moments, conv1_onepass,
+                    bool(CONV1_SIGNMASK and conv1_moments and conv1_onepass))
 
 
 def _winograd(x, weight, bias, stats, transpose, f4, tag, out_slope=1.0):
@@ -213,11 +217,17 @@
     return y
 
 
-def conv1_affine_act(x, weight, bias, scale, shift, slope, tag='conv', out_bf16=False):
+def conv1_affine_act(x, weight, bias, scale, shift, slope, tag='conv', out_bf16=False, mask=None):
     B, _, Hi, Wi = x.shape
     Cout = weight.shape[0]
     with timer.range('conv1_fwd_act/' + tag):
-        if out_bf16:
+        if mask is not None:
+            if out_bf16:
+                raise _lib.HipExtensionError('conv1_affine_act: the sign mask belongs to the fp32 activation pass')
+            out = _empty((B, Hi, Wi, Cout), x)
+            call('cy_conv1_3x3_fwd_act_mask', _ptr(x), _ptr(weight.contiguous()), _ptr(bias), _ptr(out), _ptr(scale), _ptr(shift),
+                 float(slope), _ptr(mask), B, Hi, Wi, Cout, _stream())
+        elif out_bf16:
             out = torch.empty((B, Hi, Wi, Cout), dtype=torch.bfloat16, device=x.device)
             call('cy_conv1_3x3_fwd_act_bf16', _ptr(x), _ptr(weight.contiguous()), _ptr(bias), _ptr(out), _ptr(scale), _ptr(shift),
                  float(slope), B, Hi, Wi, Cout, _stream())
@@ -473,7 +483,7 @@
         scale, shift, mean, invstd = (_empty((N,), x) for _ in range(4))
         slope = 1.0 if cfg.slope is None else float(cfg.slope)
         plan = conv_plan(x.shape, N, cfg.k, cfg.stride, cfg.pad, cfg.nchw_in)
-        ctx.conv1_m2 = None
+        ctx.conv1_m2 = ctx.conv1_mask = None
         ctx.conv1_fused = bool(plan.conv1_bwd and bn.training and not cfg.defer_act and not x.requires_grad and 0.0 <= slope <= 1.0)
         if bn.training:
             stats = zero_pool.take((STATS_COPIES, N, 2), torch.float64, x.device)
@@ -518,7 +528,10 @@
             ctx.holder = cfg.out_holder = {'mean': mean, 'invstd': invstd, 'red': None} if ctx.bn_train else None
             return z, scale, shift
         if plan.conv1 and 0.0 <= slope <= 1.0:
-            return conv1_affine_act(x, weight, bias, scale, shift, slope, cfg.name, cfg.out_bf16)
+            if plan.conv1_signmask and ctx.conv1_m2 is not None and not cfg.out_bf16 and _sync_world()[0] is None:
+                Bx, _, Hx, Wx = x.shape
+                ctx.conv1_mask = torch.empty((query('cy_conv1_signmask_bytes', Bx, Hx, Wx, N),), dtype=torch.uint8, device=x.device)
+            return conv1_affine_act(x, weight, bias, scale, shift, slope, cfg.name, cfg.out_bf16, ctx.conv1_mask)
         out = torch.empty_like(z)
         call('cy_affine_act', _ptr(z), _ptr(out), _ptr(scale), _ptr(shift), slope, P, N, st)
         return _leave(out, cfg, st)
@@ -568,9 +581,14 @@
                 dbias = _const_zeros(N, z) if ctx.has_bias else None
                 if plan.conv1_onepass and ctx.conv1_m2 is not None and _sync_world()[0] is None:
                     with timer.range('conv1_bn_bwd_onepass/' + cfg.name):
-                        call('cy_conv1_bn_bwd_onepass_bf16' if da_bf16 else 'cy_conv1_bn_bwd_onepass', _ptr(x), _ptr(weight),
-                             _ptr(bias_t), _ptr(da), _ptr(scale), _ptr(shift), _ptr(mean), _ptr(invstd), slope,
-                             _ptr(ctx.conv1_m2), _ptr(redc), _ptr(dW), _ptr(dgamma), _ptr(dbeta), None, _ptr(ws), B, Hi, Wi, N, st)
+                        if ctx.conv1_mask is not None and not da_bf16 and da.data_ptr() % 16 == 0:
+                            call('cy_conv1_bn_bwd_onepass_mask', _ptr(x), _ptr(weight), _ptr(bias_t), _ptr(da), _ptr(ctx.conv1_mask),
+                                 _ptr(scale), _ptr(shift), _ptr(mean), _ptr(invstd), slope, _ptr(ctx.conv1_m2), _ptr(redc), _ptr(dW),
+                                 _ptr(dgamma), _ptr(dbeta), None, _ptr(ws), B, Hi, Wi, N, st)
+                        else:
+                            call('cy_conv1_bn_bwd_onepass_bf16' if da_bf16 else 'cy_conv1_bn_bwd_onepass', _ptr(x), _ptr(weight),
+                                 _ptr(bias_t), _ptr(da), _ptr(scale), _ptr(shift), _ptr(mean), _ptr(invstd), slope,
+                                 _ptr(ctx.conv1_m2), _ptr(redc), _ptr(dW), _ptr(dgamma), _ptr(dbeta), None, _ptr(ws), B, Hi, Wi, N, st)
                     return None, dW, dbias, dgamma, dbeta, None, None, None
                 with timer.range('conv1_bn_bwd_reduce/' + cfg.name):
                     call('cy_conv1_bn_bwd_reduce_bf16' if da_bf16 else 'cy_conv1_bn_bwd_reduce', _ptr(x), _ptr(weight), _ptr(bias_t), _ptr(da), _ptr(scale), _ptr(shift),
diff --git a/include/capsyolo_hip.h b/include/capsyolo_hip.h
--- a/include/capsyolo_hip.h
+++ b/include/capsyolo_hip.h
@@ -55,6 +55,13 @@
                                  const float* shift, const float* mean, const float* invstd, float slope, const double* M2,
                                  double* redc, float* dW, float* dgamma, float* dbeta, double* red_out, float* ws, int B, int H,
                                  int Wd, int Cout, void* stream);
+long long cy_conv1_signmask_bytes(int B, int H, int Wd, int Cout);
+int cy_conv1_3x3_fwd_act_mask(const float* X, const float* W, const float* bias, float* Y, const float* scale,
+                              const float* shift, float slope, void* mask, int B, int H, int Wd, int Cout, void* stream);
+int cy_conv1_bn_bwd_onepass_mask(const float* X, const float* W, const float* bias, const float* dA, const void* mask,
+                                 const float* scale, const float* shift, const float* mean, const float* invstd, float slope,
+                                 const double* M2, double* redc, float* dW, float* dgamma, float* dbeta, double* red_out,
+                                 float* ws, int B, int H, int Wd, int Cout, void* stream);
 
 long long cy_conv_packed_floats(int K, int N);
 int cy_conv_pack_weights(const float* W, float* Wp, int Cout, int Cin, int KH, int KW,
```
